# mad-red/VSR-guided-CIC

Measured on NVIDIA B200. Metric: captions/sec beam-search decode (COCO-Entities shape), higher is better.
Workload: dtype f32

## Files before the change

vsr-guided-cic_b200/csrc/api.cu:

```cuda
#include <stdarg.h>
#include <stdlib.h>
#include <string.h>

#include <algorithm>

#include "common.cuh"

namespace vsr {

static thread_local char g_err[1024] = "";

void set_error(const char* fmt, ...) {
  va_list ap;
  va_start(ap, fmt);
  vsnprintf(g_err, sizeof(g_err), fmt, ap);
  va_end(ap);
}

int dev_alloc(Ctx* c, void** p, size_t bytes, bool zero) {
  *p = nullptr;
  if (bytes == 0) bytes = 16;
  cudaError_t e = cudaMalloc(p, bytes);
  if (e != cudaSuccess) {
    set_error("cudaMalloc(%zu bytes) failed: %s", bytes, cudaGetErrorString(e));
    cudaGetLastError();
    return VSR_ENOMEM;
  }
  c->owned.push_back(*p);
  c->epoch++;
  if (zero) VSR_CHECK_CUDA(cudaMemset(*p, 0, bytes));
  return VSR_OK;
}

static void dev_free(Ctx* c, void* p) {
  if (p == nullptr) return;
  auto it = std::find(c->owned.begin(), c->owned.end(), p);
  if (it != c->owned.end()) c->owned.erase(it);
  c->epoch++;
  cudaFree(p);
}

PhaseScope::PhaseScope(Ctx* c_, int id_, cudaStream_t st_) : c(c_), id(id_), st(st_) {
  c->phases[id].launches++;
  if (!c->profiling) return;
  cudaEvent_t e;
  if (cudaEventCreate(&e) == cudaSuccess) { cudaEventRecord(e, st); c->phases[id].ev.push_back(e); }
}
PhaseScope::~PhaseScope() {
  if (!c->profiling) return;
  cudaEvent_t e;
  if (cudaEventCreate(&e) == cudaSuccess) { cudaEventRecord(e, st); c->phases[id].ev.push_back(e); }
}

static const char* kPhaseNames[PH_COUNT] = {
    "prologue", "gemm_a_lstm1_gates", "lstm1_pointwise", "gemm_b_sentinel_h1proj", "gate_pointwise",
    "gemm_c_att_ga", "attend_gate", "gemm_d_lstm2_gates", "lstm2_pointwise", "gemm_e_vocab",
    "softmax_topk", "beam_select", "state_reorder", "backtrack"};

static void reset_phases(Ctx* c) {
  for (int i = 0; i < PH_COUNT; ++i) {
    for (cudaEvent_t e : c->phases[i].ev) cudaEventDestroy(e);
    c->phases[i].ev.clear();
    c->phases[i].launches = 0;
  }
}

#define ALLOC_F(ptr, count) VSR_TRY(dev_alloc(c, (void**)&(ptr), sizeof(float) * (size_t)(count)))

static int pad_rows(int n_valid, int bn, int alt_bn) {
  int r = round_up(n_valid, bn);
  if (alt_bn > 0) r = std::max(r, round_up(n_valid, alt_bn));
  return round_up(r, 128);
}

enum PairKind { PAIR_F16X3 = 0, PAIR_F8 = 1, PAIR_BOTH = 2 };
static PairKind step_kind(const Ctx* c) { return c->gemm_f8 ? PAIR_F8 : PAIR_F16X3; }

int alloc_pair(Ctx* c, F16Pair* b, int rows, int ld, int box_rows, PairKind kind, bool weight = false, int n_valid = 0,
               int alt_bn = 0, int alt_kb = 64) {
  dev_free(c, b->hi); dev_free(c, b->lo); dev_free(c, b->hi8); dev_free(c, b->lo8);
  b->hi = b->lo = b->hi8 = b->lo8 = nullptr;
  if (!c->use_tc) return VSR_OK;
  VSR_TRY(dev_alloc(c, &b->hi, (size_t)rows * ld * 2));
  b->rows = rows; b->ld = ld; b->box_rows = box_rows;
  VSR_TRY(make_tmap_f16(b->map_hi, b->hi, rows, ld, ld, box_rows));
  VSR_TRY(make_tmap_f16(b->map32_hi, b->hi, rows, ld, ld, box_rows, 32));
  if (kind == PAIR_F16X3 || kind == PAIR_BOTH) {
    VSR_TRY(dev_alloc(c, &b->lo, (size_t)rows * ld * 2));
    VSR_TRY(make_tmap_f16(b->map_lo, b->lo, rows, ld, ld, box_rows));
    VSR_TRY(make_tmap_f16(b->map32_lo, b->lo, rows, ld, ld, box_rows, 32));
  }
  if (kind == PAIR_F8 || kind == PAIR_BOTH) {
    VSR_TRY(dev_alloc(c, &b->hi8, (size_t)rows * ld));
    VSR_TRY(dev_alloc(c, &b->lo8, (size_t)rows * ld));
    VSR_TRY(make_tmap_u8(b->map8_hi, b->hi8, rows, ld, ld, box_rows));
    VSR_TRY(make_tmap_u8(b->map8_lo, b->lo8, rows, ld, ld, box_rows));
    VSR_TRY(make_tmap_u8(b->map8_32_hi, b->hi8, rows, ld, ld, box_rows, 32));
    VSR_TRY(make_tmap_u8(b->map8_32_lo, b->lo8, rows, ld, ld, box_rows, 32));
  }
  b->act_scale = (!weight && kind != PAIR_F16X3) ? ACT_SCALE_F8 : 1.f;
  b->kb = c->gemm_kb;
  b->n_valid = n_valid > 0 ? n_valid : rows;
  b->alt_bn = 0;
  if (alt_bn > 0 && c->use_alt_tiles) {
    VSR_TRY(make_tmap_f16(b->alt_hi, b->hi, rows, ld, ld, alt_bn, alt_kb));
    if (kind != PAIR_F8) VSR_TRY(make_tmap_f16(b->alt_lo, b->lo, rows, ld, ld, alt_bn, alt_kb));
    if (kind != PAIR_F16X3) {
      VSR_TRY(make_tmap_u8(b->alt8_hi, b->hi8, rows, ld, ld, alt_bn, alt_kb));
      VSR_TRY(make_tmap_u8(b->alt8_lo, b->lo8, rows, ld, ld, alt_bn, alt_kb));
    }
    b->alt_bn = alt_bn; b->alt_kb = alt_kb;
  }
  if (weight && b->scale == nullptr) VSR_TRY(dev_alloc(c, (void**)&b->scale, 2 * sizeof(float)));
  return VSR_OK;
}

int ensure_rows(Ctx* c, int rows) {
  if (rows <= c->cap_rows) return VSR_OK;
  const int cap = round_up(rows, MPAD);
  float** bufs[] = {&c->h1, &c->c1, &c->h2, &c->c2, &c->h1n, &c->c1n, &c->h2n, &c->c2n, &c->pre1,
                    &c->s_t, &c->g_t, &c->gq, &c->sent, &c->hb, &c->ga, &c->att, &c->pre2, &c->logits, &c->gate_lp,
                    &c->row_max, &c->row_lsum, &c->shift, &c->vpart};
  for (float** p : bufs) { dev_free(c, *p); *p = nullptr; }
  dev_free(c, c->word_idx);
  dev_free(c, c->ptr); dev_free(c, c->ptrn); dev_free(c, c->forced); dev_free(c, c->cand); dev_free(c, c->word_in);
  c->cap_rows = 0;
  const size_t n = cap;
  ALLOC_F(c->h1, n * c->Hp); ALLOC_F(c->c1, n * c->Hp); ALLOC_F(c->h2, n * c->Hp); ALLOC_F(c->c2, n * c->Hp);
  ALLOC_F(c->h1n, n * c->Hp); ALLOC_F(c->c1n, n * c->Hp); ALLOC_F(c->h2n, n * c->Hp); ALLOC_F(c->c2n, n * c->Hp);
  VSR_TRY(dev_alloc(c, (void**)&c->word_idx, sizeof(int32_t) * n));
  ALLOC_F(c->pre1, n * c->NA);
  ALLOC_F(c->s_t, n * c->Hp); ALLOC_F(c->g_t, n * c->Hp); ALLOC_F(c->gq, n * c->Hp);
  ALLOC_F(c->sent, n * c->NB1); ALLOC_F(c->hb, n * c->NB2); ALLOC_F(c->ga, n * c->NC);
  ALLOC_F(c->att, n * c->Fp); ALLOC_F(c->pre2, n * c->ND); ALLOC_F(c->logits, n * c->NE);
  ALLOC_F(c->gate_lp, n * 2); ALLOC_F(c->row_max, n); ALLOC_F(c->row_lsum, n); ALLOC_F(c->shift, n);
  ALLOC_F(c->vpart, n * (size_t)(c->NE / 16) * 2);
  VSR_TRY(dev_alloc(c, (void**)&c->ptr, sizeof(int32_t) * n));
  VSR_TRY(dev_alloc(c, (void**)&c->ptrn, sizeof(int32_t) * n));
  VSR_TRY(dev_alloc(c, (void**)&c->forced, sizeof(int32_t) * n));
  VSR_TRY(dev_alloc(c, (void**)&c->cand, sizeof(int32_t) * n * VSR_MAX_BEAM));
  VSR_TRY(dev_alloc(c, (void**)&c->word_in, sizeof(int64_t) * n));
  const PairKind sk = step_kind(c), hk = sk == PAIR_F8 ? PAIR_BOTH : sk;
  VSR_TRY(alloc_pair(c, &c->h1_b, cap, c->Hp, MPAD, hk)); VSR_TRY(alloc_pair(c, &c->h2_b, cap, c->Hp, MPAD, hk));
  VSR_TRY(alloc_pair(c, &c->s_t_b, cap, c->Hp, MPAD, sk));
  VSR_TRY(alloc_pair(c, &c->h1n_b, cap, c->Hp, MPAD, hk)); VSR_TRY(alloc_pair(c, &c->g_t_b, cap, c->Hp, MPAD, sk));
  VSR_TRY(alloc_pair(c, &c->att_b, cap, c->Fp, MPAD, sk)); VSR_TRY(alloc_pair(c, &c->h2n_b, cap, c->Hp, MPAD, hk));
  c->cap_rows = cap;
  return VSR_OK;
}

int ensure_beam_ws(Ctx* c, int caps, int T) {
  if (caps <= c->cap_caps && T <= c->cap_T) return VSR_OK;
  caps = std::max(caps, c->cap_caps); T = std::max(T, c->cap_T);
  float** fb[] = {&c->seq_lp, &c->seq_lp_n, &c->m0, &c->m1, &c->m0n, &c->m1n, &c->hist_score, &c->hist_lpw, &c->hist_lpg};
  int32_t** ib[] = {&c->sel_beam, &c->sel_word, &c->sel_gate, &c->sel_beam_n, &c->sel_word_n, &c->sel_gate_n,
                    &c->hist_parent, &c->hist_word, &c->hist_gate};
  for (float** p : fb) { dev_free(c, *p); *p = nullptr; }
  for (int32_t** p : ib) { dev_free(c, *p); *p = nullptr; }
  c->cap_caps = 0; c->cap_T = 0;
  const size_t s = (size_t)caps * VSR_MAX_BEAM, hs = s * T;
  ALLOC_F(c->seq_lp, s); ALLOC_F(c->seq_lp_n, s); ALLOC_F(c->m0, s); ALLOC_F(c->m1, s); ALLOC_F(c->m0n, s); ALLOC_F(c->m1n, s);
  ALLOC_F(c->hist_score, hs); ALLOC_F(c->hist_lpw, hs); ALLOC_F(c->hist_lpg, hs);
  VSR_TRY(dev_alloc(c, (void**)&c->sel_beam, sizeof(int32_t) * s));
  VSR_TRY(dev_alloc(c, (void**)&c->sel_word, sizeof(int32_t) * s));
  VSR_TRY(dev_alloc(c, (void**)&c->sel_gate, sizeof(int32_t) * s));
  VSR_TRY(dev_alloc(c, (void**)&c->sel_beam_n, sizeof(int32_t) * s));
  VSR_TRY(dev_alloc(c, (void**)&c->sel_word_n, sizeof(int32_t) * s));
  VSR_TRY(dev_alloc(c, (void**)&c->sel_gate_n, sizeof(int32_t) * s));
  VSR_TRY(dev_alloc(c, (void**)&c->hist_parent, sizeof(int32_t) * hs));
  VSR_TRY(dev_alloc(c, (void**)&c->hist_word, sizeof(int32_t) * hs));
  VSR_TRY(dev_alloc(c, (void**)&c->hist_gate, sizeof(int32_t) * hs));
  c->cap_caps = caps; c->cap_T = T;
  return VSR_OK;
}

static int create_impl(const VsrDims* d, const float* const* w, Ctx** out) {
  VSR_REQUIRE(d != nullptr && w != nullptr && out != nullptr, VSR_EINVAL, "vsr_create: null argument");
  VSR_REQUIRE(d->vocab_size > 0 && d->rnn_size > 0 && d->att_size > 0 && d->input_encoding_size > 0 &&
                  d->det_feat_size > 0 && d->seq_len > 0,
              VSR_EINVAL, "vsr_create: non-positive dimension");
  VSR_REQUIRE(d->det_feat_size % 4 == 0 && d->att_size % 4 == 0, VSR_EINVAL,
              "vsr_create: det_feat_size=%d and att_size=%d must be multiples of 4 (128-bit loads)",
              d->det_feat_size, d->att_size);
  VSR_REQUIRE(d->bos_idx >= 0 && d->bos_idx < d->vocab_size, VSR_EINVAL, "vsr_create: bos_idx out of range");
  VSR_REQUIRE(d->vocab_size <= 1024 * 48, VSR_EINVAL,
              "vsr_create: vocab_size=%d > 49152 unsupported (register-resident softmax/top-k row)", d->vocab_size);
  int ndev = 0;
  cudaError_t e = cudaGetDeviceCount(&ndev);
  VSR_REQUIRE(e == cudaSuccess && ndev > 0, VSR_ECUDA,
              "vsr_create: no CUDA device available (%s); libvsrdec has no CPU fallback",
              cudaGetErrorString(e));
  Ctx* c = new Ctx();
  c->d = *d;
  VSR_CHECK_CUDA(cudaGetDevice(&c->device));
  c->V = d->vocab_size; c->E = d->input_encoding_size; c->H = d->rnn_size; c->F = d->det_feat_size; c->A = d->att_size;
  c->Hp = round_up(c->H, KPAD); c->Ep = round_up(c->E, KPAD); c->Fp = round_up(c->F, KPAD); c->Ap = round_up(c->A, KPAD);
  c->NA = 6 * c->Hp;
  c->oB1_sa = c->Fp;
  c->NB1v = c->oB1_sa + c->A;
  c->NB1 = pad_rows(c->NB1v, 128, 0);
  c->oB2_ha = c->Hp;
  c->oB2_p2 = c->oB2_ha + c->Ap;
  c->NB2v = c->oB2_p2;
  c->NB2 = pad_rows(c->NB2v, 128, 0);
  c->NC = round_up(c->A, NPAD);
  c->ND = 4 * c->Hp;
  c->NE = round_up(c->V, 1152);
  c->NVA = round_up(c->A, NPAD);
  c->KA = (d->h2_first_lstm ? c->Hp : 0) + c->Hp;
  c->KD = c->Fp + 2 * c->Hp;
  for (int i = 0; i < PH_COUNT; ++i) c->phases[i].name = kPhaseNames[i];
  *out = c;
  ALLOC_F(c->WA, (size_t)c->NA * c->KA); ALLOC_F(c->WU, (size_t)c->NA * c->Fp); ALLOC_F(c->bU, c->NA);
  ALLOC_F(c->WB1, (size_t)c->NB1 * c->Hp); ALLOC_F(c->bB1, c->NB1);
  ALLOC_F(c->WB2, (size_t)c->NB2 * c->Hp);
  ALLOC_F(c->WC, (size_t)c->NC * c->Hp);
  ALLOC_F(c->WD, (size_t)c->ND * c->KD); ALLOC_F(c->bD, c->ND);
  if (d->img_second_lstm) ALLOC_F(c->WU2, (size_t)c->ND * c->Fp);
  ALLOC_F(c->WE, (size_t)c->NE * c->Hp); ALLOC_F(c->bE, c->NE);
  ALLOC_F(c->Wva, (size_t)c->NVA * c->Fp);
  ALLOC_F(c->v_a, c->Ap); ALLOC_F(c->v_s, c->Ap); ALLOC_F(c->v_g, c->Ap);
  ALLOC_F(c->embed, (size_t)c->V * c->Ep);
  ALLOC_F(c->WAx, (size_t)c->NA * c->Ep); ALLOC_F(c->X, (size_t)c->V * c->NA);
  {
    const char* mode = getenv("VSRDEC_GEMM");
    c->use_tc = !(mode != nullptr && strcmp(mode, "simt") == 0);
    c->gemm_f8 = !(mode != nullptr && strcmp(mode, "f16x3") == 0);
  }
  int bn = 128;
  if (const char* e = getenv("VSRDEC_BN")) bn = atoi(e) == 256 ? 256 : 128;
  if (const char* e = getenv("VSRDEC_GRAPH")) c->use_graphs = atoi(e) != 0;
  if (const char* e = getenv("VSRDEC_PDL")) c->use_pdl = atoi(e) != 0;
  if (const char* e = getenv("VSRDEC_ZERO_STATE")) c->zero_state_opt = atoi(e) != 0;
  if (const char* e = getenv("VSRDEC_PDL_MODE")) c->pdl_mode = atoi(e);
  if (const char* e = getenv("VSRDEC_KB")) c->gemm_kb = atoi(e) == 32 ? 32 : 64;
  if (const char* e = getenv("VSRDEC_ALT_TILES")) c->use_alt_tiles = atoi(e) != 0;
  const PairKind sk = step_kind(c);
  VSR_TRY(alloc_pair(c, &c->WA_b, c->NA, c->KA, 192, sk == PAIR_F8 ? PAIR_BOTH : sk, true)); VSR_TRY(alloc_pair(c, &c->WB1_b, c->NB1, c->Hp, bn, sk, true, c->NB1v));
  VSR_TRY(alloc_pair(c, &c->WB2_b, c->NB2, c->Hp, bn, sk, true, c->NB2v)); VSR_TRY(alloc_pair(c, &c->WC_b, c->NC, c->Hp, 128, sk, true));
  VSR_TRY(alloc_pair(c, &c->WD_b, c->ND, c->KD, 128, sk, true)); VSR_TRY(alloc_pair(c, &c->WE_b, c->NE, c->Hp, bn, sk, true, c->V, 144, 64));
  if (const char* e = getenv("VSRDEC_PAIR")) c->use_pair = atoi(e) != 0;
  if (const char* e = getenv("VSRDEC_PAIR_MIN_ROWS")) c->pair_min_rows = atoi(e);
  if (c->use_pair && c->use_tc) {
    VSR_TRY(make_pair_maps(&c->WA_b, 96)); VSR_TRY(make_pair_maps(&c->WB1_b, 128)); VSR_TRY(make_pair_maps(&c->WB2_b, 128));
    VSR_TRY(make_pair_maps(&c->WC_b, 128)); VSR_TRY(make_pair_maps(&c->WD_b, 128)); VSR_TRY(make_pair_maps(&c->WE_b, 96));
  }
  c->WA_b.kb = 32;
  if (const char* e = getenv("VSRDEC_KB_A")) c->WA_b.kb = atoi(e) == 32 ? 32 : 64;
  VSR_TRY(alloc_pair(c, &c->WU_b, c->NA, c->Fp, 128, PAIR_F16X3, true)); VSR_TRY(alloc_pair(c, &c->Wva_b, c->NVA, c->Fp, bn, PAIR_F16X3, true));
  if (d->img_second_lstm) VSR_TRY(alloc_pair(c, &c->WU2_b, c->ND, c->Fp, 128, PAIR_F16X3, true));
  VSR_TRY(pack_weights(c, w, 0));
  VSR_CHECK_CUDA(cudaStreamSynchronize(0));
  return VSR_OK;
}

static void drop_graphs(Ctx* c) {
  for (auto& g : c->graphs) cudaGraphExecDestroy(g.exec);
  c->graphs.clear();
  c->graph_seen.clear();
}

template <typename Enqueue>
static int run_graphed(Ctx* c, const Ctx::GraphKey& key, cudaStream_t st, Enqueue enqueue) {
  if (!c->graphs.empty() && c->graphs[0].key.epoch != c->epoch) drop_graphs(c);
  ++c->graph_clock;
  for (auto& g : c->graphs)
    if (memcmp(&g.key, &key, sizeof(key)) == 0) {
      VSR_CHECK_CUDA(cudaGraphLaunch(g.exec, st));
      c->launches += g.launches; g.last_use = c->graph_clock;
      return VSR_OK;
    }
  bool seen = false;
  for (auto& s : c->graph_seen) seen = seen || memcmp(&s, &key, sizeof(key)) == 0;
  if (!seen) {
    if (c->graph_seen.size() >= 32) c->graph_seen.erase(c->graph_seen.begin());
    c->graph_seen.push_back(key);
    return enqueue(st);
  }
  if (c->cap_stream == nullptr) VSR_CHECK_CUDA(cudaStreamCreateWithFlags(&c->cap_stream, cudaStreamNonBlocking));
  const int64_t l0 = c->launches;
  VSR_CHECK_CUDA(cudaStreamBeginCapture(c->cap_stream, cudaStreamCaptureModeThreadLocal));
  const int rc = enqueue(c->cap_stream);
  cudaGraph_t graph = nullptr;
  const cudaError_t ce = cudaStreamEndCapture(c->cap_stream, &graph);
  const int64_t n_launch = c->launches - l0;
  c->launches = l0;
  if (rc != VSR_OK) { if (graph) cudaGraphDestroy(graph); return rc; }
  VSR_CHECK_CUDA(ce);
  cudaGraphExec_t exec = nullptr;
  const cudaError_t ie = cudaGraphInstantiate(&exec, graph, 0);
  cudaGraphDestroy(graph);
  VSR_CHECK_CUDA(ie);
  if (c->graphs.size() >= 16) {
    size_t lru = 0;
    for (size_t i = 1; i < c->graphs.size(); ++i) if (c->graphs[i].last_use < c->graphs[lru].last_use) lru = i;
    cudaGraphExecDestroy(c->graphs[lru].exec);
    c->graphs.erase(c->graphs.begin() + lru);
  }
  c->graphs.push_back({key, exec, n_launch, c->graph_clock});
  VSR_CHECK_CUDA(cudaGraphLaunch(exec, st));
  c->launches += n_launch;
  return VSR_OK;
}

static Ctx::GraphKey graph_key(const Ctx* c, int kind) {
  Ctx::GraphKey key;
  memset(&key, 0, sizeof(key));
  key.kind = kind;
  key.epoch = c->epoch; key.det = c->det; key.det_seqs = c->det_seqs; key.slot_index = c->slot_index; key.verbs = c->verbs;
  key.det_stride = c->det_stride;
  key.b = c->b; key.D = c->D; key.L = c->L; key.R = c->R; key.n_img = c->n_img; key.verbs_dtype = c->verbs_dtype;
  return key;
}

static bool graphs_usable(Ctx* c, cudaStream_t st) {
  cudaStreamCaptureStatus cap = cudaStreamCaptureStatusNone;
  if (cudaStreamIsCapturing(st, &cap) != cudaSuccess) { cudaGetLastError(); cap = cudaStreamCaptureStatusActive; }
  return c->use_graphs && !c->profiling && cap == cudaStreamCaptureStatusNone;
}

static int prologue_impl(Ctx* c, const float* det, int64_t det_stride, int D, const float* det_seqs,
                         const int32_t* slot_index, int b, int L, int R, const void* verbs, int verbs_dtype,
                         cudaStream_t st) {
  VSR_REQUIRE(det != nullptr && (det_seqs != nullptr || slot_index != nullptr), VSR_EINVAL, "vsr_prologue: null input");
  VSR_REQUIRE(b > 0 && D > 0 && L > 0 && R > 0, VSR_EINVAL, "vsr_prologue: bad shape b=%d D=%d L=%d R=%d", b, D, L, R);
  VSR_REQUIRE(R <= 64, VSR_EINVAL, "vsr_prologue: R=%d regions per slot > 64 unsupported", R);
  VSR_REQUIRE(det_stride == 0 || det_stride >= (int64_t)D * c->F, VSR_EINVAL, "vsr_prologue: bad det_batch_stride");
  VSR_REQUIRE(verbs == nullptr || (verbs_dtype >= 0 && verbs_dtype <= 2), VSR_EINVAL, "vsr_prologue: bad verbs dtype");
  VSR_REQUIRE(slot_index == nullptr || det_stride == 0 || det_stride == (int64_t)D * c->F, VSR_EINVAL,
              "vsr_prologue_indexed: detections must be dense (b, D, F) or one shared image");
  VSR_REQUIRE(((uintptr_t)det % 16) == 0 && ((uintptr_t)det_seqs % 16) == 0 && (det_stride % 4) == 0, VSR_EINVAL,
              "vsr_prologue: feature tensors must be 16-byte aligned");
  c->have_prologue = false;
  if (c->profiling) reset_phases(c);
  c->b = b; c->D = D; c->L = L; c->R = R;
  c->n_img = det_stride == 0 ? 1 : b;
  c->det_seqs = det_seqs; c->slot_index = slot_index; c->det = det; c->det_stride = det_stride;
  c->verbs = verbs; c->verbs_dtype = verbs_dtype;
  const size_t n_img_pad = round_up(c->n_img, MPAD);
  if (n_img_pad > c->cap_img) {
    dev_free(c, c->img); dev_free(c, c->U); dev_free(c, c->U2);
    c->img = c->U = c->U2 = nullptr; c->cap_img = 0;
    ALLOC_F(c->img, n_img_pad * c->Fp); ALLOC_F(c->U, n_img_pad * c->NA);
    if (c->d.img_second_lstm) ALLOC_F(c->U2, n_img_pad * c->ND);
    VSR_TRY(alloc_pair(c, &c->img_b, (int)n_img_pad, c->Fp, MPAD, PAIR_F16X3));
    c->cap_img = n_img_pad;
  }
  const size_t prow = slot_index == nullptr
                          ? (size_t)b * L * R
                          : (size_t)round_up(c->n_img * D, MPAD) + round_up(c->n_img, MPAD);
  if (prow > c->cap_P || (size_t)b * L + 1 > c->cap_slots) {
    const size_t need_rows = std::max(prow, c->cap_P), need_slots = std::max((size_t)b * L + 1, c->cap_slots);
    dev_free(c, c->P); dev_free(c, c->seq_valid); dev_free(c, c->slot_mask); dev_free(c, c->slot_base); dev_free(c, c->comp_valid);
    c->P = nullptr; c->seq_valid = nullptr; c->slot_mask = nullptr; c->slot_base = nullptr; c->comp_valid = nullptr;
    c->cap_P = 0; c->cap_slots = 0;
    ALLOC_F(c->P, round_up((int)need_rows, MPAD) * (size_t)c->NVA);
    VSR_TRY(dev_alloc(c, (void**)&c->seq_valid, round_up((int)need_rows, MPAD)));
    VSR_TRY(dev_alloc(c, (void**)&c->slot_mask, sizeof(unsigned long long) * need_slots));
    VSR_TRY(dev_alloc(c, (void**)&c->slot_base, sizeof(int32_t) * need_slots));
    VSR_TRY(dev_alloc(c, (void**)&c->comp_valid, round_up((int)need_rows, MPAD)));
    VSR_TRY(alloc_pair(c, &c->ds_b, round_up((int)need_rows, MPAD), c->Fp, MPAD, PAIR_F16X3));
    c->cap_P = need_rows; c->cap_slots = need_slots;
  }
  c->Pmean = slot_index != nullptr ? c->P + (size_t)round_up(c->n_img * D, MPAD) * c->NVA : nullptr;
  const size_t dvr = (size_t)c->n_img * D;
  if (dvr > c->cap_detv) {
    dev_free(c, c->det_valid); c->det_valid = nullptr; c->cap_detv = 0;
    VSR_TRY(dev_alloc(c, (void**)&c->det_valid, dvr));
    c->cap_detv = dvr;
  }
  VSR_TRY(ensure_rows(c, b));
  c->p_compact = slot_index == nullptr && c->use_tc;
  auto enqueue = [&](cudaStream_t s) {
    return slot_index == nullptr ? run_prologue(c, det, det_stride, s) : run_prologue_indexed(c, det, det_stride, s);
  };
  if (graphs_usable(c, st)) VSR_TRY(run_graphed(c, graph_key(c, 1), st, enqueue));
  else VSR_TRY(enqueue(st));
  c->have_prologue = true;
  return VSR_OK;
}

__global__ void k_copy2d(float* dst, int ld_dst, const float* src, int ld_src, int w, int rows) {
  const int i = blockIdx.x * blockDim.x + threadIdx.x;
  const int n = blockIdx.y;
  if (i < w && n < rows) dst[(size_t)n * ld_dst + i] = src[(size_t)n * ld_src + i];
}
__global__ void k_slots_from_i64(int32_t* ptr, const int64_t* slot, int rows, int L) {
  const int n = blockIdx.x * blockDim.x + threadIdx.x;
  if (n >= rows) return;
  int64_t s = slot[n];
  s = s < 0 ? 0 : (s > L - 1 ? L - 1 : s);
  ptr[n] = (int32_t)s;
}
__global__ void k_fill_i32(int32_t* p, int v, int n) {
  const int i = blockIdx.x * blockDim.x + threadIdx.x;
  if (i < n) p[i] = v;
}

static int copy2d(Ctx* c, float* dst, int ld_dst, const float* src, int ld_src, int w, int rows, cudaStream_t st) {
  dim3 grid((w + 255) / 256, rows);
  k_copy2d<<<grid, 256, 0, st>>>(dst, ld_dst, src, ld_src, w, rows);
  VSR_CHECK_CUDA(cudaGetLastError()); c->launches++;
  return VSR_OK;
}

static int step_impl(Ctx* c, const float* h1, const float* c1, const float* h2, const float* c2,
                     const int64_t* slot, const int64_t* word, int use_verbs, int gt, float* h1o, float* c1o,
                     float* h2o, float* c2o, float* out_logp, float* gate_logp, cudaStream_t st) {
  VSR_REQUIRE(c->have_prologue, VSR_ESTATE, "vsr_step: call vsr_prologue first");
  VSR_REQUIRE(h1 && c1 && h2 && c2 && slot && word, VSR_EINVAL, "vsr_step: null state input");
  VSR_REQUIRE(!use_verbs || c->verbs != nullptr, VSR_EINVAL, "vsr_step: use_verbs without a verbs tensor");
  const int b = c->b, H = c->H;
  VSR_TRY(copy2d(c, c->h1, c->Hp, h1, H, H, b, st));
  VSR_TRY(copy2d(c, c->c1, c->Hp, c1, H, H, b, st));
  VSR_TRY(copy2d(c, c->h2, c->Hp, h2, H, H, b, st));
  VSR_TRY(copy2d(c, c->c2, c->Hp, c2, H, H, b, st));
  k_slots_from_i64<<<(b + 127) / 128, 128, 0, st>>>(c->ptr, slot, b, c->L);
  VSR_CHECK_CUDA(cudaGetLastError()); c->launches++;
  VSR_TRY(launch_words(c, word, b, st));
  if (c->use_tc) {
    VSR_TRY(launch_split_pair(c->h1, c->h1_b, (size_t)b * c->Hp, st));
    VSR_TRY(launch_split_pair(c->h2, c->h2_b, (size_t)b * c->Hp, st));
    c->launches += 2;
  }
  StepIO io{};
  io.rows = b; io.cur_beam = 1; io.use_verbs = use_verbs != 0; io.gt = gt != 0;
  io.out_logp = out_logp; io.out_stride = c->V; io.gate_out = gate_logp; io.gate_stride = 2; io.topk = 0;
  io.need_h32 = true;
  VSR_TRY(run_step(c, io, st));
  if (h1o) VSR_TRY(copy2d(c, h1o, H, c->h1n, c->Hp, H, b, st));
  if (c1o) VSR_TRY(copy2d(c, c1o, H, c->c1n, c->Hp, H, b, st));
  if (h2o) VSR_TRY(copy2d(c, h2o, H, c->h2n, c->Hp, H, b, st));
  if (c2o) VSR_TRY(copy2d(c, c2o, H, c->c2n, c->Hp, H, b, st));
  return VSR_OK;
}

static int enqueue_beam_steps(Ctx* c, int k, const int64_t* eos, int use_verbs, int gt, const VsrTrace* tr,
                              cudaStream_t st) {
  const int b = c->b, T = c->d.seq_len;
  VSR_TRY(launch_state_init(c, b, st));
  const bool have_forced = tr && tr->forced_beam && tr->forced_word && tr->forced_gate;
  if (c->profiling) {
    for (cudaEvent_t e : c->step_ev) cudaEventDestroy(e);
    c->step_ev.clear();
  }
  for (int t = 0; t < T; ++t) {
    if (c->profiling) {
      cudaEvent_t e;
      if (cudaEventCreate(&e) == cudaSuccess) { cudaEventRecord(e, st); c->step_ev.push_back(e); }
    }
    const int cur = t == 0 ? 1 : k;
    const int rows = b * cur;
    StepIO io{};
    io.rows = rows; io.cur_beam = cur; io.use_verbs = use_verbs != 0; io.gt = gt != 0; io.topk = k;
    io.zero_state = t == 0 && c->zero_state_opt;
    if (tr && tr->step_out) { io.out_logp = tr->step_out + (size_t)t * b * k * c->V; io.out_stride = c->V; }
    if (tr && tr->step_gate) { io.gate_out = tr->step_gate + (size_t)t * b * k * 2; io.gate_stride = 2; }
    VSR_TRY(run_step(c, io, st));
    const size_t fo = (size_t)t * b * k;
    VSR_TRY(launch_beam_step(c, t, b, cur, k, eos[0], eos[1], have_forced ? tr->forced_beam + fo : nullptr,
                             have_forced ? tr->forced_word + fo : nullptr,
                             have_forced ? tr->forced_gate + fo : nullptr, t + 1 < T, st));
  }
  if (c->profiling) {
    cudaEvent_t e;
    if (cudaEventCreate(&e) == cudaSuccess) { cudaEventRecord(e, st); c->step_ev.push_back(e); }
  }
  return VSR_OK;
}

static int beam_steps_graphed(Ctx* c, int k, const int64_t* eos, int use_verbs, int gt, cudaStream_t st) {
  Ctx::GraphKey key = graph_key(c, 0);
  key.eos0 = eos[0]; key.eos1 = eos[1];
  key.k = k; key.use_verbs = use_verbs; key.gt = gt; key.T = c->d.seq_len;
  return run_graphed(c, key, st, [&](cudaStream_t s) { return enqueue_beam_steps(c, k, eos, use_verbs, gt, nullptr, s); });
}

static int beam_search_impl(Ctx* c, int k, int out_size, const int64_t* eos, int use_verbs, int gt,
                            int64_t* out_words, int64_t* out_gates, float* lp_words, float* lp_gates,
                            const VsrTrace* tr, cudaStream_t st) {
  VSR_REQUIRE(c->have_prologue, VSR_ESTATE, "vsr_beam_search: call vsr_prologue first");
  VSR_REQUIRE(k >= 1 && k <= VSR_MAX_BEAM, VSR_EINVAL, "vsr_beam_search: beam_size=%d not in [1,%d]", k, VSR_MAX_BEAM);
  VSR_REQUIRE(out_size >= 1 && out_size <= k, VSR_EINVAL, "vsr_beam_search: out_size=%d not in [1,beam]", out_size);
  VSR_REQUIRE(c->V >= k, VSR_EINVAL, "vsr_beam_search: vocabulary (%d) smaller than the beam (%d): a row has fewer than "
              "beam distinct word candidates", c->V, k);
  VSR_REQUIRE(c->d.seq_len <= VSR_MAX_SEQ_LEN, VSR_EINVAL, "vsr_beam_search: seq_len=%d > %d unsupported by the back-track kernel",
              c->d.seq_len, VSR_MAX_SEQ_LEN);
  VSR_REQUIRE(eos && out_words && out_gates && lp_words && lp_gates, VSR_EINVAL, "vsr_beam_search: null argument");
  VSR_REQUIRE(!use_verbs || c->verbs != nullptr, VSR_EINVAL, "vsr_beam_search: use_verbs without a verbs tensor");
  const int b = c->b, T = c->d.seq_len;
  VSR_TRY(ensure_rows(c, b * k));
  VSR_TRY(ensure_beam_ws(c, b, T));
  c->hist_T = T; c->hist_b = b; c->hist_k = k;
  if (tr == nullptr && graphs_usable(c, st))
    VSR_TRY(beam_steps_graphed(c, k, eos, use_verbs, gt, st));
  else
    VSR_TRY(enqueue_beam_steps(c, k, eos, use_verbs, gt, tr, st));
  VSR_TRY(launch_backtrack(c, b, k, T, out_size, out_words, out_gates, lp_words, lp_gates, st));
  return VSR_OK;
}

static int ensure_fwd_ws(Ctx* c, int rows) {
  if (rows <= c->cap_fwd_rows) return VSR_OK;
  const int cap = round_up(rows, MPAD);
  dev_free(c, c->logits_all); dev_free(c, c->gate_all);
  c->logits_all = c->gate_all = nullptr; c->cap_fwd_rows = 0;
  ALLOC_F(c->logits_all, (size_t)cap * c->NE); ALLOC_F(c->gate_all, (size_t)cap * 2);
  VSR_TRY(alloc_pair(c, &c->h2all_b, cap, c->Hp, MPAD, step_kind(c)));
  c->cap_fwd_rows = cap;
  return VSR_OK;
}

static int enqueue_forward_steps(Ctx* c, const int64_t* captions, int T, bool batched, float* out, float* gate, cudaStream_t st) {
  const int b = c->b;
  VSR_TRY(launch_state_init(c, b, st));
  for (int t = 0; t < T; ++t) {
    if (t == 0) {
      VSR_CHECK_CUDA(cudaMemcpy2DAsync(c->word_in, sizeof(int64_t), captions, sizeof(int64_t) * T,
                                       sizeof(int64_t), b, cudaMemcpyDeviceToDevice, st));
      VSR_TRY(launch_words(c, c->word_in, b, st));
    }
    StepIO io{};
    io.rows = b; io.cur_beam = 1; io.use_verbs = false; io.gt = false; io.topk = 0;
    io.zero_state = t == 0 && c->zero_state_opt;
    if (batched) {
      io.skip_vocab = true;
      VSR_TRY(run_step(c, io, st));
      VSR_TRY(launch_gate_head(c, b, c->gate_all + (size_t)t * 2, (int64_t)T * 2, st));
      VSR_TRY(launch_rows_to_all(c, c->h2n_b, c->h2all_b, b, T, t, st));
    } else {
      io.out_logp = out + (size_t)t * c->V; io.out_stride = (int64_t)T * c->V;
      io.gate_out = gate + (size_t)t * 2; io.gate_stride = (int64_t)T * 2;
      VSR_TRY(run_step(c, io, st));
    }
    if (t + 1 < T) VSR_TRY(launch_commit_identity(c, b, captions + (t + 1), T, t + 1, st));
  }
  if (batched) VSR_TRY(run_vocab_rows(c, c->h2all_b, c->logits_all, b * T, nullptr, st, false));
  return VSR_OK;
}

static int forward_impl(Ctx* c, const int64_t* captions, int T, float* out, float* gate, cudaStream_t st) {
  VSR_REQUIRE(c->have_prologue, VSR_ESTATE, "vsr_forward_teacher: call vsr_prologue first");
  VSR_REQUIRE(captions && out && gate, VSR_EINVAL, "vsr_forward_teacher: null argument");
  VSR_REQUIRE(T >= 1 && T <= c->L, VSR_EINVAL, "vsr_forward_teacher: T=%d exceeds the prologue's slot count L=%d", T, c->L);
  const int b = c->b;
  VSR_TRY(ensure_rows(c, b));
  const bool batched = c->use_tc;
  if (!batched) return enqueue_forward_steps(c, captions, T, false, out, gate, st);
  VSR_TRY(ensure_fwd_ws(c, b * T));
  if (graphs_usable(c, st)) {
    Ctx::GraphKey key = graph_key(c, 2);
    key.captions = captions; key.T = T;
    VSR_TRY(run_graphed(c, key, st, [&](cudaStream_t s) { return enqueue_forward_steps(c, captions, T, true, nullptr, nullptr, s); }));
  } else {
    VSR_TRY(enqueue_forward_steps(c, captions, T, true, nullptr, nullptr, st));
  }
  VSR_TRY(run_vocab_rows(c, c->h2all_b, c->logits_all, b * T, out, st, true));
  VSR_CHECK_CUDA(cudaMemcpyAsync(gate, c->gate_all, sizeof(float) * (size_t)b * T * 2, cudaMemcpyDeviceToDevice, st));
  return VSR_OK;
}

static int greedy_impl(Ctx* c, int64_t* out_words, int64_t* out_gates, cudaStream_t st) {
  VSR_REQUIRE(c->have_prologue, VSR_ESTATE, "vsr_greedy: call vsr_prologue first");
  VSR_REQUIRE(out_words && out_gates, VSR_EINVAL, "vsr_greedy: null argument");
  const int b = c->b, T = c->d.seq_len;
  VSR_TRY(ensure_rows(c, b));
  VSR_TRY(ensure_beam_ws(c, b, T));
  VSR_TRY(launch_state_init(c, b, st));
  for (int t = 0; t < T; ++t) {
    StepIO io{};
    io.rows = b; io.cur_beam = 1; io.use_verbs = false; io.gt = false; io.topk = 1;
    io.zero_state = t == 0 && c->zero_state_opt;
    VSR_TRY(run_step(c, io, st));
    VSR_TRY(launch_greedy_pick(c, b, t, T, out_words, out_gates, st));
    if (t + 1 < T) VSR_TRY(launch_commit_identity(c, b, nullptr, 0, -1, st));
  }
  return VSR_OK;
}

static int sample_impl(Ctx* c, uint64_t seed, int64_t* out_words, int64_t* out_gates, float* lp_words, float* lp_gates,
                       cudaStream_t st) {
  VSR_REQUIRE(c->have_prologue, VSR_ESTATE, "vsr_sample: call vsr_prologue first");
  VSR_REQUIRE(out_words && out_gates && lp_words && lp_gates, VSR_EINVAL, "vsr_sample: null argument");
  const int b = c->b, T = c->d.seq_len;
  VSR_TRY(ensure_rows(c, b));
  VSR_TRY(ensure_beam_ws(c, b, T));
  VSR_TRY(launch_state_init(c, b, st));
  for (int t = 0; t < T; ++t) {
    StepIO io{};
    io.rows = b; io.cur_beam = 1; io.use_verbs = false; io.gt = false; io.topk = 0;
    io.zero_state = t == 0 && c->zero_state_opt;
    VSR_TRY(run_step(c, io, st));
    VSR_TRY(launch_sample_pick(c, b, t, T, seed, out_words, out_gates, lp_words, lp_gates, st));
    if (t + 1 < T) VSR_TRY(launch_commit_identity(c, b, nullptr, 0, -1, st));
  }
  return VSR_OK;
}

}

using vsr::Ctx;

struct DeviceGuard {
  int prev = -1; bool switched = false;
  explicit DeviceGuard(const vsr::Ctx* c) {
    if (c != nullptr && cudaGetDevice(&prev) == cudaSuccess && prev != c->device) switched = cudaSetDevice(c->device) == cudaSuccess;
  }
// ... 187 lines not shown
```

vsr-guided-cic_b200/csrc/beam.cu:

```cuda
#include <cuda_fp16.h>
#include <math.h>

#include "common.cuh"

namespace vsr {

namespace {

__device__ __forceinline__ bool before(float v1, int i1, float v2, int i2) {
  return v1 > v2 || (v1 == v2 && i1 < i2);
}

__device__ __forceinline__ float row_logp(const float* logits, int ld, const float* row_max,
                                          const float* row_lsum, const int32_t* forced, int row, int word) {
  const int f = forced[row];
  if (f >= 0) return word == f ? 0.f : -1e6f;
  return (logits[(size_t)row * ld + word] - row_max[row]) - row_lsum[row];
}

struct BeamArgs {
  int t, b, cur, k, V;
  int64_t eos0, eos1;
  const float* logits; int ld;
  const float* row_max; const float* row_lsum; const int32_t* forced; const int32_t* cand;
  const float* gate_lp;
  const float* seq_lp; float* seq_lp_n;
  float *m0, *m1, *m0n, *m1n;
  const int32_t *prev_word, *prev_gate;
  int32_t *sel_beam, *sel_word, *sel_gate;
  int32_t *hist_parent, *hist_word, *hist_gate;
  float *hist_score, *hist_lpw, *hist_lpg;
  const int32_t *f_beam, *f_word, *f_gate;
};

constexpr int MAXC = 2 * VSR_MAX_BEAM * VSR_MAX_BEAM;

struct BeamSmem {
  float seq[VSR_MAX_BEAM], m0[VSR_MAX_BEAM], m1[VSR_MAX_BEAM], ps[VSR_MAX_BEAM];
  int full[VSR_MAX_BEAM], pb[VSR_MAX_BEAM], pw[VSR_MAX_BEAM], pg[VSR_MAX_BEAM];
};

__device__ __forceinline__ void beam_select_warp(const BeamArgs& a, BeamSmem& sh, int c, int lane, bool write) {
  const int k = a.k, cur = a.cur;
  float* s_seq = sh.seq; float* s_m0 = sh.m0; float* s_m1 = sh.m1; float* s_ps = sh.ps;
  int* s_full = sh.full; int* s_pb = sh.pb; int* s_pw = sh.pw; int* s_pg = sh.pg;

  if (lane < cur) {
    float m0 = 1.f, m1 = 1.f, seq = 0.f;
    if (a.t > 0) {
      seq = a.seq_lp[c * k + lane];
      m0 = a.m0[c * k + lane] * ((int64_t)a.prev_word[c * k + lane] != a.eos0 ? 1.f : 0.f);
      m1 = a.m1[c * k + lane] * ((int64_t)a.prev_gate[c * k + lane] != a.eos1 ? 1.f : 0.f);
    }
    s_seq[lane] = seq; s_m0[lane] = m0; s_m1[lane] = m1;
    s_full[lane] = (a.t == 0) ? 1 : (fminf(fmaxf(m0 + m1, 0.f), 1.f) != 0.f);
  }
  __syncwarp();

  if (a.f_beam == nullptr) {
    float cs[MAXC / 32]; int cf[MAXC / 32]; bool used[MAXC / 32];
    const int ncand = cur * k * 2;
#pragma unroll
    for (int q = 0; q < MAXC / 32; ++q) {
      const int idx = lane + 32 * q;
      cs[q] = -INFINITY; cf[q] = 0x7fffffff; used[q] = true;
      if (idx < ncand) {
        const int j = idx / (2 * k), i = (idx >> 1) % k, g = idx & 1;
        const int row = c * cur + j;
        int word; float sc;
        if (s_full[j]) {
          word = a.cand[row * VSR_MAX_BEAM + i];
          const float wl = row_logp(a.logits, a.ld, a.row_max, a.row_lsum, a.forced, row, word);
          sc = __fadd_rn(s_seq[j], __fadd_rn(wl, a.gate_lp[row * 2 + g]));
        } else {
          word = i;
          sc = (i == 0) ? s_seq[j] : -999.f;
        }
        cs[q] = sc; cf[q] = j * 2 * a.V + word * 2 + g; used[q] = false;
      }
    }
    for (int sel = 0; sel < k; ++sel) {
      float bv = -INFINITY; int bf = 0x7fffffff;
#pragma unroll
      for (int q = 0; q < MAXC / 32; ++q)
        if (!used[q] && before(cs[q], cf[q], bv, bf)) { bv = cs[q]; bf = cf[q]; }
      {
        const unsigned u = __float_as_uint(bv);
        const unsigned key = (u & 0x80000000u) ? ~u : (u | 0x80000000u);
        const unsigned kbest = __reduce_max_sync(0xffffffffu, key);
        const int fbest = (int)__reduce_min_sync(0xffffffffu, key == kbest ? (unsigned)bf : 0xffffffffu);
        const unsigned owner = __ballot_sync(0xffffffffu, key == kbest && bf == fbest);
        bv = __shfl_sync(0xffffffffu, bv, __ffs(owner) - 1);
        bf = fbest;
      }
#pragma unroll
      for (int q = 0; q < MAXC / 32; ++q) if (cf[q] == bf) used[q] = true;
      if (lane == 0) {
        const int j = bf / (2 * a.V), rem = bf - j * 2 * a.V;
        s_pb[sel] = j; s_pw[sel] = rem >> 1; s_pg[sel] = rem & 1; s_ps[sel] = bv;
      }
    }
  } else if (lane < k) {
    const int j = a.f_beam[c * k + lane], word = a.f_word[c * k + lane], g = a.f_gate[c * k + lane];
    const int row = c * cur + j;
    float sc;
    if (s_full[j]) {
      const float wl = row_logp(a.logits, a.ld, a.row_max, a.row_lsum, a.forced, row, word);
      sc = __fadd_rn(s_seq[j], __fadd_rn(wl, a.gate_lp[row * 2 + g]));
    } else {
      sc = (word == 0) ? s_seq[j] : -999.f;
    }
    s_pb[lane] = j; s_pw[lane] = word; s_pg[lane] = g; s_ps[lane] = sc;
  }
  __syncwarp();

  if (lane < k && write) {
    const int j = s_pb[lane], word = s_pw[lane], g = s_pg[lane];
    const int row = c * cur + j;
    const int o = c * k + lane;
    float lw = row_logp(a.logits, a.ld, a.row_max, a.row_lsum, a.forced, row, word);
    float lg = a.gate_lp[row * 2 + g];
    if (a.t > 0) { lw *= s_m0[j]; lg *= s_m1[j]; }
    a.sel_beam[o] = j; a.sel_word[o] = word; a.sel_gate[o] = g;
    a.seq_lp_n[o] = s_ps[lane];
    a.m0n[o] = s_m0[j]; a.m1n[o] = s_m1[j];
    a.hist_parent[o] = j; a.hist_word[o] = word; a.hist_gate[o] = g;
    a.hist_score[o] = s_ps[lane]; a.hist_lpw[o] = lw; a.hist_lpg[o] = lg;
  }
}

struct AdvanceArgs {
  int rows_new, cur, k;
  const int32_t* parent;
  const int32_t* word32;
  const int64_t* word64; int64_t word64_stride;
  const int32_t* gate32;
  int fixed_slot;
  int L, Hp, Ep, V;
  const float *h1n, *c1n, *h2n, *c2n;
  float *h1, *c1, *h2, *c2;
  const int32_t* ptr; int32_t* ptrn;
  int32_t* word_idx;
  int n_tw;
  const uint4* tw_src[8]; uint4* tw_dst[8]; int tw_vec[8];
};

__device__ __forceinline__ void advance_row(const AdvanceArgs& a, int n, int p, int64_t w, int gate_shift) {
  const size_t so = (size_t)p * a.Hp, dof = (size_t)n * a.Hp;
  for (int i = threadIdx.x * 4; i < a.Hp; i += blockDim.x * 4) {
    if (a.h1n != nullptr) {
      *reinterpret_cast<float4*>(a.h1 + dof + i) = *reinterpret_cast<const float4*>(a.h1n + so + i);
      *reinterpret_cast<float4*>(a.h2 + dof + i) = *reinterpret_cast<const float4*>(a.h2n + so + i);
    }
    *reinterpret_cast<float4*>(a.c1 + dof + i) = *reinterpret_cast<const float4*>(a.c1n + so + i);
    *reinterpret_cast<float4*>(a.c2 + dof + i) = *reinterpret_cast<const float4*>(a.c2n + so + i);
  }
  w = w < 0 ? 0 : (w >= a.V ? a.V - 1 : w);
  for (int q = 0; q < a.n_tw; ++q) {
    const int nv = a.tw_vec[q];
    const uint4* src = a.tw_src[q] + (size_t)p * nv;
    uint4* dst = a.tw_dst[q] + (size_t)n * nv;
    for (int i = threadIdx.x; i < nv; i += blockDim.x) dst[i] = src[i];
  }
  if (threadIdx.x == 0) {
    a.word_idx[n] = (int32_t)w;
    int s;
    if (a.fixed_slot >= 0) s = a.fixed_slot;
    else {
      s = a.ptr[p] + gate_shift;
      s = s < 0 ? 0 : (s > a.L - 1 ? a.L - 1 : s);
    }
    a.ptrn[n] = s;
  }
}

__global__ void __launch_bounds__(256) k_advance(const AdvanceArgs a) {
  const int n = blockIdx.x;
  const int c = n / a.k;
  const int p = a.parent != nullptr ? c * a.cur + a.parent[n] : n;
  const int64_t w = a.word32 != nullptr ? (int64_t)a.word32[n] : a.word64[(size_t)n * a.word64_stride];
  advance_row(a, n, p, w, a.gate32 != nullptr ? a.gate32[n] : 0);
}

__global__ void __launch_bounds__(256) k_beam_step(const BeamArgs b, const AdvanceArgs a, int do_advance) {
  __shared__ BeamSmem sh;
  const int c = blockIdx.x, i = blockIdx.y;
  pdl_trigger();
  pdl_wait();
  if (threadIdx.x < 32) beam_select_warp(b, sh, c, threadIdx.x, i == 0);
  __syncthreads();
  if (!do_advance) return;
  advance_row(a, c * b.k + i, c * b.cur + sh.pb[i], (int64_t)sh.pw[i], sh.pg[i]);
}

__global__ void k_state_init(float* h1, float* c1, float* h2, float* c2, int32_t* word_idx, int32_t* ptr,
                             int bos, int Hp, TwinOut h1b, TwinOut h2b) {
  const int n = blockIdx.x;
  const float4 z = make_float4(0.f, 0.f, 0.f, 0.f);
  for (int i = threadIdx.x * 4; i < Hp; i += blockDim.x * 4) {
    const size_t o = (size_t)n * Hp + i;
    *reinterpret_cast<float4*>(h1 + o) = z; *reinterpret_cast<float4*>(c1 + o) = z;
    *reinterpret_cast<float4*>(h2 + o) = z; *reinterpret_cast<float4*>(c2 + o) = z;
    store_twin4(h1b, o, z); store_twin4(h2b, o, z);
  }
  if (threadIdx.x == 0) { ptr[n] = 0; word_idx[n] = bos; }
}

__global__ void k_words_from_i64(const int64_t* words, int32_t* word_idx, int rows, int V) {
  const int n = blockIdx.x * blockDim.x + threadIdx.x;
  if (n >= rows) return;
  int64_t w = words[n];
  w = w < 0 ? 0 : (w >= V ? V - 1 : w);
  word_idx[n] = (int32_t)w;
}

__global__ void k_greedy_pick(const int32_t* cand, const float* gate_lp, int32_t* sel_word,
                              int32_t* sel_gate, int64_t* out_words, int64_t* out_gates, int rows,
                              int t, int T) {
  const int n = blockIdx.x * blockDim.x + threadIdx.x;
  if (n >= rows) return;
  const int w = cand[n * VSR_MAX_BEAM];
  const int g = gate_lp[n * 2 + 1] > gate_lp[n * 2 + 0] ? 1 : 0;
  sel_word[n] = w; sel_gate[n] = g;
  out_words[(size_t)n * T + t] = w; out_gates[(size_t)n * T + t] = g;
}

__device__ __forceinline__ uint4 philox4x32_10(uint4 ctr, uint2 key) {
#pragma unroll
  for (int r = 0; r < 10; ++r) {
    const unsigned hi0 = __umulhi(0xD2511F53u, ctr.x), lo0 = 0xD2511F53u * ctr.x;
    const unsigned hi1 = __umulhi(0xCD9E8D57u, ctr.z), lo1 = 0xCD9E8D57u * ctr.z;
    ctr = make_uint4(hi1 ^ ctr.y ^ key.x, lo1, hi0 ^ ctr.w ^ key.y, lo0);
    key.x += 0x9E3779B9u; key.y += 0xBB67AE85u;
  }
  return ctr;
}
__device__ __forceinline__ float u01(unsigned x) { return ((float)(x >> 8) + 0.5f) * (1.f / 16777216.f); }

__global__ void __launch_bounds__(256) k_sample_pick(const float* __restrict__ logits, int ld, int V, const float* __restrict__ row_max,
                                                     const float* __restrict__ row_lsum, const float* __restrict__ gate_lp,
                                                     unsigned long long seed, int t, int T, int32_t* sel_word, int32_t* sel_gate,
                                                     int64_t* out_words, int64_t* out_gates, float* lp_words, float* lp_gates) {
  __shared__ float s_v[8];
  __shared__ int s_i[8];
  const int n = blockIdx.x, tid = threadIdx.x, lane = tid & 31, warp = tid >> 5;
  const float* x = logits + (size_t)n * ld;
  const uint2 key = make_uint2((unsigned)seed, (unsigned)(seed >> 32));
  float bv = -INFINITY; int bi = 0x7fffffff;
  for (int v0 = tid * 4; v0 < V; v0 += 256 * 4) {
    const uint4 r = philox4x32_10(make_uint4((unsigned)(v0 >> 2), (unsigned)n, (unsigned)t, 0u), key);
    const float4 q = *reinterpret_cast<const float4*>(x + v0);
    const float xs[4] = {q.x, q.y, q.z, q.w};
    const unsigned rs[4] = {r.x, r.y, r.z, r.w};
#pragma unroll
    for (int e = 0; e < 4; ++e) {
      if (v0 + e >= V) break;
      const float g = -logf(-logf(u01(rs[e])));
      const float sc = xs[e] + g;
      if (sc > bv) { bv = sc; bi = v0 + e; }
    }
  }
#pragma unroll
  for (int o = 16; o > 0; o >>= 1) {
    const float ov = __shfl_xor_sync(0xffffffffu, bv, o);
    const int oi = __shfl_xor_sync(0xffffffffu, bi, o);
    if (before(ov, oi, bv, bi)) { bv = ov; bi = oi; }
  }
  if (lane == 0) { s_v[warp] = bv; s_i[warp] = bi; }
  __syncthreads();
  if (tid == 0) {
    for (int w = 1; w < 8; ++w) if (before(s_v[w], s_i[w], bv, bi)) { bv = s_v[w]; bi = s_i[w]; }
    const int word = bi < V ? bi : V - 1;
    const float lw = (x[word] - row_max[n]) - row_lsum[n];
    const uint4 r = philox4x32_10(make_uint4(0u, (unsigned)n, (unsigned)t, 1u), key);
    const float g0 = gate_lp[(size_t)n * 2], g1 = gate_lp[(size_t)n * 2 + 1];
    const int gate = u01(r.x) < expf(g0) ? 0 : 1;
    sel_word[n] = word; sel_gate[n] = gate;
    out_words[(size_t)n * T + t] = word; out_gates[(size_t)n * T + t] = gate;
    lp_words[(size_t)n * T + t] = lw; lp_gates[(size_t)n * T + t] = gate == 0 ? g0 : g1;
  }
}

__global__ void __launch_bounds__(64) k_backtrack(int b, int k, int T, int out_size, const float* seq_lp,
                                                  const int32_t* hist_parent, const int32_t* hist_word,
                                                  const int32_t* hist_gate, const float* hist_lpw, const float* hist_lpg,
                                                  int64_t* out_words, int64_t* out_gates, float* lp_words, float* lp_gates) {
  extern __shared__ __align__(16) unsigned char bt_smem[];
  int32_t* s_par = reinterpret_cast<int32_t*>(bt_smem);
  int32_t* s_wrd = s_par + T * k;
  int32_t* s_gat = s_wrd + T * k;
  float* s_lpw = reinterpret_cast<float*>(s_gat + T * k);
  float* s_lpg = s_lpw + T * k;
  __shared__ float s_seq[VSR_MAX_BEAM];
  const int c = blockIdx.x;
  for (int i = threadIdx.x; i < T * k; i += blockDim.x) {
    const int t = i / k, j = i - t * k;
    const size_t hi = ((size_t)t * b + c) * k + j;
    s_par[i] = hist_parent[hi]; s_wrd[i] = hist_word[hi]; s_gat[i] = hist_gate[hi];
    s_lpw[i] = hist_lpw[hi]; s_lpg[i] = hist_lpg[hi];
  }
  if (threadIdx.x < k) s_seq[threadIdx.x] = seq_lp[c * k + threadIdx.x];
  __syncthreads();
  const int o = threadIdx.x;
  if (o >= out_size) return;
  int order[VSR_MAX_BEAM];
  for (int i = 0; i < k; ++i) order[i] = i;
  for (int i = 1; i < k; ++i) {
    const int oi = order[i];
    const float v = s_seq[oi];
    int j = i - 1;
    while (j >= 0 && s_seq[order[j]] < v) { order[j + 1] = order[j]; --j; }
    order[j + 1] = oi;
  }
  const int final_slot = order[o];
  int slot = final_slot;
  const size_t ob = ((size_t)c * out_size + o) * T;
  for (int t = T - 1; t >= 0; --t) {
    out_words[ob + t] = s_wrd[t * k + slot];
    out_gates[ob + t] = s_gat[t * k + slot];
    lp_words[ob + t] = s_lpw[t * k + final_slot];
    lp_gates[ob + t] = s_lpg[t * k + final_slot];
    slot = s_par[t * k + slot];
  }
}

}

static TwinOut pp(const Ctx* c, const F16Pair& b) { return twin_out(&b, c->use_tc); }

int launch_state_init(Ctx* c, int rows, cudaStream_t st) {
  k_state_init<<<rows, 256, 0, st>>>(c->h1, c->c1, c->h2, c->c2, c->word_idx, c->ptr, c->d.bos_idx, c->Hp,
                                     pp(c, c->h1_b), pp(c, c->h2_b));
  VSR_CHECK_CUDA(cudaGetLastError()); c->launches++;
  return VSR_OK;
}

int launch_words(Ctx* c, const int64_t* words, int rows, cudaStream_t st) {
  k_words_from_i64<<<(rows + 127) / 128, 128, 0, st>>>(words, c->word_idx, rows, c->V);
  VSR_CHECK_CUDA(cudaGetLastError()); c->launches++;
  return VSR_OK;
}

static void fill_advance(Ctx* c, AdvanceArgs& a) {
  a.L = c->L; a.Hp = c->Hp; a.Ep = c->Ep; a.V = c->V;
  a.h1n = c->state_h32 ? c->h1n : nullptr; a.c1n = c->c1n; a.h2n = c->state_h32 ? c->h2n : nullptr; a.c2n = c->c2n;
  a.h1 = c->h1; a.c1 = c->c1; a.h2 = c->h2; a.c2 = c->c2;
  a.ptr = c->ptr; a.ptrn = c->ptrn; a.word_idx = c->word_idx;
  a.n_tw = 0;
  if (c->use_tc) {
    auto add = [&](const void* src, void* dst, int bytes_per_elem) {
      if (src == nullptr || dst == nullptr) return;
      a.tw_src[a.n_tw] = (const uint4*)src; a.tw_dst[a.n_tw] = (uint4*)dst; a.tw_vec[a.n_tw] = c->Hp * bytes_per_elem / 16;
      ++a.n_tw;
    };
    const F16Pair* src[2] = {&c->h1n_b, &c->h2n_b};
    F16Pair* dst[2] = {&c->h1_b, &c->h2_b};
    for (int q = 0; q < 2; ++q) {
      add(src[q]->hi, dst[q]->hi, 2); add(src[q]->lo, dst[q]->lo, 2);
      add(src[q]->hi8, dst[q]->hi8, 1); add(src[q]->lo8, dst[q]->lo8, 1);
    }
  }
}

int launch_beam_step(Ctx* c, int t, int b, int cur, int k, int64_t eos0, int64_t eos1, const int32_t* f_beam,
                     const int32_t* f_word, const int32_t* f_gate, bool advance, cudaStream_t st) {
  PhaseScope ps(c, PH_BEAM, st);
  BeamArgs a{};
  a.t = t; a.b = b; a.cur = cur; a.k = k; a.V = c->V; a.eos0 = eos0; a.eos1 = eos1;
  a.logits = c->logits; a.ld = c->NE; a.row_max = c->row_max; a.row_lsum = c->row_lsum;
  a.forced = c->forced; a.cand = c->cand; a.gate_lp = c->gate_lp;
  a.seq_lp = c->seq_lp; a.seq_lp_n = c->seq_lp_n;
  a.m0 = c->m0; a.m1 = c->m1; a.m0n = c->m0n; a.m1n = c->m1n;
  a.prev_word = c->sel_word; a.prev_gate = c->sel_gate;
  a.sel_beam = c->sel_beam_n; a.sel_word = c->sel_word_n; a.sel_gate = c->sel_gate_n;
  const size_t off = (size_t)t * b * k;
  a.hist_parent = c->hist_parent + off; a.hist_word = c->hist_word + off; a.hist_gate = c->hist_gate + off;
  a.hist_score = c->hist_score + off; a.hist_lpw = c->hist_lpw + off; a.hist_lpg = c->hist_lpg + off;
  a.f_beam = f_beam; a.f_word = f_word; a.f_gate = f_gate;
  AdvanceArgs ad{};
  ad.rows_new = b * k; ad.cur = cur; ad.k = k; ad.fixed_slot = -1;
  fill_advance(c, ad);
  VSR_CHECK_CUDA(launch_k(k_beam_step, dim3(b, advance ? k : 1), dim3(256), 0, st, c->use_pdl && (c->pdl_mode & 2), a, ad, advance ? 1 : 0));
  VSR_CHECK_CUDA(cudaGetLastError()); c->launches++;
  std::swap(c->sel_beam, c->sel_beam_n);
  std::swap(c->sel_word, c->sel_word_n);
  std::swap(c->sel_gate, c->sel_gate_n);
  std::swap(c->seq_lp, c->seq_lp_n);
  std::swap(c->m0, c->m0n);
  std::swap(c->m1, c->m1n);
  if (advance) std::swap(c->ptr, c->ptrn);
  return VSR_OK;
}

static int launch_advance(Ctx* c, AdvanceArgs& a, cudaStream_t st) {
  fill_advance(c, a);
  k_advance<<<a.rows_new, 256, 0, st>>>(a);
  VSR_CHECK_CUDA(cudaGetLastError()); c->launches++;
  std::swap(c->ptr, c->ptrn);
  return VSR_OK;
}

int launch_commit_identity(Ctx* c, int rows, const int64_t* next_words, int64_t word_stride,
                           int next_slot, cudaStream_t st) {
  PhaseScope ps(c, PH_REORDER, st);
  AdvanceArgs a{};
  a.rows_new = rows; a.cur = 1; a.k = 1;
  a.parent = nullptr;
  if (next_words != nullptr) { a.word64 = next_words; a.word64_stride = word_stride; a.gate32 = nullptr; }
  else { a.word32 = c->sel_word; a.gate32 = c->sel_gate; }
  a.fixed_slot = next_slot;
  return launch_advance(c, a, st);
}

int launch_greedy_pick(Ctx* c, int rows, int t, int T, int64_t* out_words, int64_t* out_gates,
                       cudaStream_t st) {
  PhaseScope ps(c, PH_BEAM, st);
  k_greedy_pick<<<(rows + 127) / 128, 128, 0, st>>>(c->cand, c->gate_lp, c->sel_word, c->sel_gate,
                                                    out_words, out_gates, rows, t, T);
  VSR_CHECK_CUDA(cudaGetLastError()); c->launches++;
  return VSR_OK;
}

int launch_sample_pick(Ctx* c, int rows, int t, int T, uint64_t seed, int64_t* out_words, int64_t* out_gates,
                       float* lp_words, float* lp_gates, cudaStream_t st) {
  PhaseScope ps(c, PH_BEAM, st);
  k_sample_pick<<<rows, 256, 0, st>>>(c->logits, c->NE, c->V, c->row_max, c->row_lsum, c->gate_lp, (unsigned long long)seed, t, T,
                                      c->sel_word, c->sel_gate, out_words, out_gates, lp_words, lp_gates);
  VSR_CHECK_CUDA(cudaGetLastError()); c->launches++;
  return VSR_OK;
}

int launch_backtrack(Ctx* c, int b, int k, int T, int out_size, int64_t* out_words,
                     int64_t* out_gates, float* lp_words, float* lp_gates, cudaStream_t st) {
  PhaseScope ps(c, PH_FINAL, st);
  VSR_REQUIRE(T <= VSR_MAX_SEQ_LEN, VSR_EINVAL, "seq_len=%d > %d unsupported by the back-track kernel", T, VSR_MAX_SEQ_LEN);
  k_backtrack<<<b, 64, (size_t)T * k * 20, st>>>(b, k, T, out_size, c->hist_score + (size_t)(T - 1) * b * k, c->hist_parent, c->hist_word,
                                            c->hist_gate, c->hist_lpw, c->hist_lpg, out_words, out_gates,
                                            lp_words, lp_gates);
  VSR_CHECK_CUDA(cudaGetLastError()); c->launches++;
  return VSR_OK;
}

}
```

vsr-guided-cic_b200/csrc/common.cuh:

```cuda
#pragma once
#include <cuda_runtime.h>
#include <stdint.h>
#include <stdio.h>
#include <string>
#include <vector>

#include "../../include/vsrdec.h"

namespace vsr {

void set_error(const char* fmt, ...);
#define VSR_CHECK_CUDA(expr)                                                                 \
  do {                                                                                       \
    cudaError_t _e = (expr);                                                                 \
    if (_e != cudaSuccess) {                                                                 \
      vsr::set_error("%s:%d CUDA error %s: %s", __FILE__, __LINE__, #expr,                   \
                     cudaGetErrorString(_e));                                                \
      return VSR_ECUDA;                                                                      \
    }                                                                                        \
  } while (0)
#define VSR_REQUIRE(cond, code, ...)                                                         \
  do {                                                                                       \
    if (!(cond)) {                                                                           \
      vsr::set_error(__VA_ARGS__);                                                           \
      return (code);                                                                         \
    }                                                                                        \
  } while (0)
#define VSR_TRY(expr)                                                                        \
  do {                                                                                       \
    int _r = (expr);                                                                         \
    if (_r != VSR_OK) return _r;                                                             \
  } while (0)

static inline int round_up(int x, int m) { return (x + m - 1) / m * m; }

#ifdef __CUDACC__
}
#include <cuda_fp16.h>
#include <cuda_fp8.h>
namespace vsr {
__device__ __forceinline__ float fast_sigmoid(float x) { return __fdividef(1.f, 1.f + __expf(-x)); }
__device__ __forceinline__ float fast_tanh(float x) { return 1.f - __fdividef(2.f, __expf(2.f * x) + 1.f); }
#endif

constexpr int KPAD = 64;
constexpr int NPAD = 256;
constexpr int MPAD = 128;

constexpr float ACT_SCALE_F8 = 256.f;

struct F16Pair {
  void* hi = nullptr;
  void* lo = nullptr;
  void* hi8 = nullptr;
  void* lo8 = nullptr;
  float act_scale = 1.f;
  int rows = 0, ld = 0, box_rows = 0;
  float* scale = nullptr;
  int kb = 64;
  alignas(64) unsigned char map_hi[128];
  alignas(64) unsigned char map_lo[128];
  alignas(64) unsigned char map32_hi[128];
  alignas(64) unsigned char map32_lo[128];
  alignas(64) unsigned char map8_hi[128];
  alignas(64) unsigned char map8_lo[128];
  alignas(64) unsigned char map8_32_hi[128];
  alignas(64) unsigned char map8_32_lo[128];
  alignas(64) unsigned char alt8_hi[128];
  alignas(64) unsigned char alt8_lo[128];
  int pair_rows = 0;
  alignas(64) unsigned char pair_hi[128];
  alignas(64) unsigned char pair_lo[128];
  alignas(64) unsigned char pair_lo16[128];
  alignas(64) unsigned char pair_h8[128];
  int n_valid = 0;
  int alt_bn = 0, alt_kb = 64;
  alignas(64) unsigned char alt_hi[128];
  alignas(64) unsigned char alt_lo[128];
};

struct TwinOut {
  void* hi; void* lo; uint8_t* hi8; uint8_t* lo8;
  float scale;
};
inline TwinOut twin_out(const F16Pair* b, bool enabled = true) {
  TwinOut o{nullptr, nullptr, nullptr, nullptr, 1.f};
  if (b != nullptr && enabled) { o.hi = b->hi; o.lo = b->lo; o.hi8 = (uint8_t*)b->hi8; o.lo8 = (uint8_t*)b->lo8; o.scale = b->act_scale; }
  return o;
}
#ifdef __CUDACC__
__device__ __forceinline__ void store_twin4(const TwinOut& o, size_t off, const float4 v) {
  if (o.hi == nullptr) return;
  const float x[4] = {fminf(fmaxf(v.x * o.scale, -65504.f), 65504.f), fminf(fmaxf(v.y * o.scale, -65504.f), 65504.f),
                      fminf(fmaxf(v.z * o.scale, -65504.f), 65504.f), fminf(fmaxf(v.w * o.scale, -65504.f), 65504.f)};
  __align__(8) __half h[4];
  float hf[4], r[4];
#pragma unroll
  for (int j = 0; j < 4; ++j) { h[j] = __float2half_rn(x[j]); hf[j] = __half2float(h[j]); r[j] = x[j] - hf[j]; }
  *reinterpret_cast<uint2*>(reinterpret_cast<__half*>(o.hi) + off) = *reinterpret_cast<const uint2*>(h);
  if (o.lo != nullptr) {
    __align__(8) __half l[4];
#pragma unroll
    for (int j = 0; j < 4; ++j) l[j] = __float2half_rn(r[j]);
    *reinterpret_cast<uint2*>(reinterpret_cast<__half*>(o.lo) + off) = *reinterpret_cast<const uint2*>(l);
  }
  if (o.hi8 != nullptr) {
    const unsigned h01 = __nv_cvt_float2_to_fp8x2(make_float2(hf[0] * 0.03125f, hf[1] * 0.03125f), __NV_SATFINITE, __NV_E4M3);
    const unsigned h23 = __nv_cvt_float2_to_fp8x2(make_float2(hf[2] * 0.03125f, hf[3] * 0.03125f), __NV_SATFINITE, __NV_E4M3);
    const unsigned l01 = __nv_cvt_float2_to_fp8x2(make_float2(r[0] * 32.f, r[1] * 32.f), __NV_SATFINITE, __NV_E4M3);
    const unsigned l23 = __nv_cvt_float2_to_fp8x2(make_float2(r[2] * 32.f, r[3] * 32.f), __NV_SATFINITE, __NV_E4M3);
    *reinterpret_cast<uint32_t*>(o.hi8 + off) = h01 | (h23 << 16);
    *reinterpret_cast<uint32_t*>(o.lo8 + off) = l01 | (l23 << 16);
  }
}
#endif

struct GemmSeg {
  const float* a;
  int lda;
  int k;
  int k_valid;
  const F16Pair* b = nullptr;
};
__host__ __device__ inline int cell_col(int g, int u, int ng) {
  return (u >> 5) * (ng * 32) + g * 32 + (u & 31);
}

#ifdef __CUDACC__
__device__ __forceinline__ void pdl_wait() { asm volatile("griddepcontrol.wait;" ::: "memory"); }
__device__ __forceinline__ void pdl_trigger() { asm volatile("griddepcontrol.launch_dependents;" ::: "memory"); }

template <typename... KArgs, typename... Args>
inline cudaError_t launch_k(void (*kernel)(KArgs...), dim3 grid, dim3 block, size_t smem, cudaStream_t st, bool pdl,
                            Args&&... args) {
  cudaLaunchConfig_t cfg = {};
  cfg.gridDim = grid; cfg.blockDim = block; cfg.dynamicSmemBytes = smem; cfg.stream = st;
  cudaLaunchAttribute attr[1];
  attr[0].id = cudaLaunchAttributeProgrammaticStreamSerialization;
  attr[0].val.programmaticStreamSerializationAllowed = 1;
  cfg.attrs = attr; cfg.numAttrs = pdl ? 1 : 0;
  return cudaLaunchKernelEx(&cfg, kernel, std::forward<Args>(args)...);
}
#endif

struct FusedCell {
  int mode = 0;
  const float* c_old = nullptr; float* c_new = nullptr; float* h_new = nullptr;
  const F16Pair *h_b = nullptr, *s_b = nullptr, *g_b = nullptr;
  float* s_new = nullptr;
  float* gq = nullptr;
  int ld_state = 0;
  int gt_cols = 0; const float* gt_gq = nullptr; const float* gt_c1n = nullptr;
  float* g_t = nullptr;
  float* vocab_part = nullptr; int* vocab_tiles_out = nullptr; int* vocab_bn_out = nullptr;
};
constexpr int VOCAB_REC = 16;

struct GemmArgs {
  GemmSeg seg[3];
  int nseg;
  const float* w;
  int ldw;
  const float* bias;
  const float* rowadd;
  int ld_rowadd, row_div, rowadd_mul;
  const float* cadd;
  int ld_cadd;
  float* c;
  int ldc;
  int M, N;
  const float* gather = nullptr;
  int ld_gather = 0;
  const int32_t* gather_idx = nullptr;
  const uint8_t* row_skip;
  const F16Pair* wb = nullptr;
  bool allow_pair = false;
  int pair_min_rows = 1024;
  bool no_alt = false;
  bool f8 = false;
  bool pdl = false;
  bool relu = false;
  bool zero_acc = false;
  int pdl_flags = 0;
  FusedCell cell;
};
struct Ctx;
int launch_gemm(Ctx* c, const GemmArgs& g, cudaStream_t st, const GemmArgs* g2 = nullptr);
int launch_gemm_simt(const GemmArgs& g, cudaStream_t st);
int launch_gemm_tc(const GemmArgs& g, const GemmArgs* g2, cudaStream_t st);
bool gemm_uses_tc(const Ctx* c, const GemmArgs& g);
int make_tmap_f16(void* out_map, const void* base, int rows, int cols, int ld, int box_rows, int kb = 64);
int make_tmap_u8(void* out_map, const void* base, int rows, int cols, int ld, int box_rows, int kb = 64);
int make_pair_maps(F16Pair* b, int pair_rows);
int launch_split_pair(const float* x, const F16Pair& p, size_t n, cudaStream_t st, bool weight_scale = false);

struct Phase {
  const char* name;
  std::vector<cudaEvent_t> ev;
  int launches = 0;
};

enum PhaseId {
  PH_PROLOGUE = 0, PH_GEMM_A, PH_LSTM1, PH_GEMM_B, PH_GT, PH_GEMM_C, PH_ATTEND, PH_GEMM_D, PH_LSTM2,
  PH_GEMM_E, PH_SOFTMAX_TOPK, PH_BEAM, PH_REORDER, PH_FINAL, PH_COUNT
};

struct Ctx {
  VsrDims d;
  int device;
  int V, E, H, F, A;
  int Hp, Ep, Fp, Ap;
  int NA, NB1, NB2, NC, ND, NE;
  int NB1v, NB2v;
  int KA;
  int KD;
  int oB1_sa;
  int oB2_ha, oB2_p2;
  float *WA, *WU, *bU;
  float *WB1, *bB1;
  float *WB2;
  float *WC;
  float *WD, *bD;
  float *WU2;
  float *WE, *bE;
  float *Wva;
  float *v_a, *v_s, *v_g;
  float *embed;
  float *WAx;
  float *X;
  int NVA;
  bool use_tc = true;
  int pair_min_rows = 640;
  bool use_pair = true;
  bool gemm_f8 = true;
  bool use_alt_tiles = true;
  int gemm_kb = 64;
  F16Pair WA_b, WB1_b, WB2_b, WC_b, WD_b, WE_b;
  F16Pair WU_b, WU2_b, Wva_b;
  F16Pair ds_b, img_b;
  F16Pair h1_b, h2_b, s_t_b, h1n_b, g_t_b, att_b, h2n_b;
  F16Pair h2all_b; float* logits_all = nullptr; float* gate_all = nullptr; int cap_fwd_rows = 0;
  int64_t* vt_keys = nullptr; int32_t* vt_off = nullptr; int32_t* vt_idx = nullptr; int vt_n = 0;
  bool have_prologue = false;
  int b = 0, D = 0, L = 0, R = 0, n_img = 0;
  const float* det_seqs = nullptr;
  const int32_t* slot_index = nullptr;
  const float* det = nullptr; int64_t det_stride = 0;
  float* Pmean = nullptr;
  const void* verbs = nullptr; int verbs_dtype = 0;
  float* img = nullptr;
  float* U = nullptr;
  float* U2 = nullptr;
  float* P = nullptr;
  uint8_t* seq_valid = nullptr;
  unsigned long long* slot_mask = nullptr;
  int32_t* slot_base = nullptr;
  uint8_t* comp_valid = nullptr;
  bool p_compact = false;
  uint8_t* det_valid = nullptr;
  size_t cap_img = 0, cap_P = 0, cap_detv = 0, cap_slots = 0;
  int cap_rows = 0;
  float *h1, *c1, *h2, *c2;
  float *h1n, *c1n, *h2n, *c2n;
  int32_t *word_idx;
  int32_t *ptr, *ptrn;
  float *pre1;
  float *s_t, *g_t;
  float *gq;
  float *sent;
  float *hb;
  float *ga;
  float *att;
  float *pre2;
  float *logits;
  float *gate_lp;
  float *shift;
  float *row_max, *row_lsum;
  int32_t *forced;
  int32_t *cand;
  float *vpart;
  int cap_caps = 0, cap_T = 0;
  float *seq_lp, *seq_lp_n;
  float *m0, *m1, *m0n, *m1n;
  int32_t *sel_beam, *sel_word, *sel_gate;
  int32_t *sel_beam_n, *sel_word_n, *sel_gate_n;
  int32_t *hist_parent, *hist_word, *hist_gate;
  float *hist_score, *hist_lpw, *hist_lpg;
  int hist_T = 0, hist_b = 0, hist_k = 0;
  int64_t* word_in = nullptr;
  int64_t launches = 0;
  bool profiling = false;
  Phase phases[PH_COUNT];
  std::vector<cudaEvent_t> step_ev;
  std::vector<void*> owned;
  struct GraphKey {
    uint64_t epoch;
    int64_t kind;
    const void* captions;
    const void *det, *det_seqs, *slot_index, *verbs;
    int64_t det_stride, eos0, eos1;
    int32_t b, D, L, R, n_img, verbs_dtype, k, use_verbs, gt, T;
  };
  struct GraphEntry { GraphKey key; cudaGraphExec_t exec; int64_t launches; uint64_t last_use; };
  std::vector<GraphEntry> graphs;
  std::vector<GraphKey> graph_seen;
  uint64_t epoch = 0, graph_clock = 0;
  cudaStream_t cap_stream = nullptr;
  bool attend_attr_set = false;
  bool state_h32 = true;
  bool use_graphs = true;
  bool zero_state_opt = true;
  bool use_pdl = true;
  int pdl_mode = 5;
};

int dev_alloc(Ctx* c, void** p, size_t bytes, bool zero = true);

struct PhaseScope {
  Ctx* c; int id; cudaStream_t st;
  PhaseScope(Ctx* c_, int id_, cudaStream_t st_);
  ~PhaseScope();
};

int pack_weights(Ctx* c, const float* const* w, cudaStream_t st);
int run_prologue(Ctx* c, const float* det, int64_t det_stride, cudaStream_t st);
int run_prologue_indexed(Ctx* c, const float* det, int64_t det_stride, cudaStream_t st);
int ensure_rows(Ctx* c, int rows);
int ensure_beam_ws(Ctx* c, int caps, int T);

struct StepIO {
  int rows;
  int cur_beam;
  bool use_verbs, gt;
  float* out_logp;
  int64_t out_stride;
  float* gate_out;
  int64_t gate_stride;
  int topk;
  bool zero_state;
  bool skip_vocab;
  bool need_h32;
};
int run_step(Ctx* c, const StepIO& io, cudaStream_t st);

int launch_state_init(Ctx* c, int rows, cudaStream_t st);
int launch_words(Ctx* c, const int64_t* words, int rows, cudaStream_t st);
int launch_beam_step(Ctx* c, int t, int b, int cur, int k, int64_t eos0, int64_t eos1,
                     const int32_t* f_beam, const int32_t* f_word, const int32_t* f_gate, bool advance,
                     cudaStream_t st);
int launch_backtrack(Ctx* c, int b, int k, int T, int out_size, int64_t* out_words,
                     int64_t* out_gates, float* lp_words, float* lp_gates, cudaStream_t st);
int launch_commit_identity(Ctx* c, int rows, const int64_t* next_words, int64_t word_stride,
                           int next_slot, cudaStream_t st);
int launch_greedy_pick(Ctx* c, int rows, int t, int T, int64_t* out_words, int64_t* out_gates,
                       cudaStream_t st);
int launch_sample_pick(Ctx* c, int rows, int t, int T, uint64_t seed, int64_t* out_words, int64_t* out_gates,
                       float* lp_words, float* lp_gates, cudaStream_t st);
int launch_gate_head(Ctx* c, int rows, float* gate_out, int64_t gate_stride, cudaStream_t st);
int launch_rows_to_all(Ctx* c, const F16Pair& src, const F16Pair& dst, int rows, int T, int t, cudaStream_t st);
int run_vocab_rows(Ctx* c, const F16Pair& a_b, float* logits, int M, float* out_logp, cudaStream_t st, bool softmax_only);

}
```

vsr-guided-cic_b200/csrc/gemm_tc.cu:

```cuda
#include <cuda.h>
#include <stdlib.h>
#include <string.h>
#include <cuda_fp16.h>

#include "common.cuh"

namespace vsr {

namespace {

constexpr int BM = 128;
constexpr int BK = 64;
constexpr int UMMA_K = 16;
constexpr int TC_EPI_WARPS = 8;
constexpr int TC_EPI_THREADS = 32 * TC_EPI_WARPS;
constexpr int TC_THREADS = 64 + TC_EPI_THREADS;

template <int BN, int KB> struct TcCfg {
  static constexpr int kStageB = 2 * BM * KB * 2 + 2 * BN * KB * 2;
  static constexpr int kStages = (220 * 1024) / kStageB > 8 ? 8 : (220 * 1024) / kStageB;
  static constexpr int kTmemCols = (BN <= 128) ? 128 : 256;
  static constexpr int kABytes = BM * KB * 2;
  static constexpr int kWBytes = BN * KB * 2;
  static constexpr int kStageBytes = 2 * kABytes + 2 * kWBytes;
  static constexpr int kRingBytes = kStages * kStageBytes;
  static constexpr bool kTileEpi = (BN == 128 || BN == 192);
  static constexpr int kEpiBytes = kTileEpi ? 32 * BN * 4 : 4096;
  static constexpr int kSmemBytes = kRingBytes + 1024 + kEpiBytes;
};

__device__ __forceinline__ uint32_t smem_u32(const void* p) { return (uint32_t)__cvta_generic_to_shared(p); }

__device__ __forceinline__ void mbar_init(uint64_t* bar, uint32_t count) {
  asm volatile("mbarrier.init.shared::cta.b64 [%0], %1;" ::"r"(smem_u32(bar)), "r"(count));
}
__device__ __forceinline__ void mbar_expect_tx(uint64_t* bar, uint32_t bytes) {
  asm volatile("mbarrier.arrive.expect_tx.shared::cta.b64 _, [%0], %1;" ::"r"(smem_u32(bar)), "r"(bytes) : "memory");
}
__device__ __forceinline__ void mbar_wait(uint64_t* bar, uint32_t parity) {
  asm volatile(
      "{\n\t"
      ".reg .pred p;\n\t"
      "WAIT_LOOP:\n\t"
      "mbarrier.try_wait.parity.shared::cta.b64 p, [%0], %1;\n\t"
      "@p bra WAIT_DONE;\n\t"
      "bra WAIT_LOOP;\n\t"
      "WAIT_DONE:\n\t"
      "}" ::"r"(smem_u32(bar)), "r"(parity) : "memory");
}
__device__ __forceinline__ void tma_load_2d(const CUtensorMap* map, uint64_t* bar, void* dst, int c0, int c1) {
  asm volatile(
      "cp.async.bulk.tensor.2d.shared::cluster.global.mbarrier::complete_tx::bytes [%0], [%1, {%3, %4}], [%2];"
      ::"r"(smem_u32(dst)), "l"(map), "r"(smem_u32(bar)), "r"(c0), "r"(c1) : "memory");
}
__device__ __forceinline__ void prefetch_tmap(const CUtensorMap* map) {
  asm volatile("prefetch.tensormap [%0];" ::"l"(map) : "memory");
}

__device__ __forceinline__ uint64_t make_sw64_desc(uint32_t smem_addr) {
  uint64_t d = 0;
  d |= (uint64_t)((smem_addr >> 4) & 0x3FFF);
  d |= (uint64_t)1 << 16;
  d |= (uint64_t)(512 >> 4) << 32;
  d |= (uint64_t)1 << 46;
  d |= (uint64_t)4 << 61;
  return d;
}
template <int KB> __device__ __forceinline__ uint64_t make_kmajor_desc(uint32_t smem_addr);

__device__ __forceinline__ uint64_t make_sw128_desc(uint32_t smem_addr) {
  uint64_t d = 0;
  d |= (uint64_t)((smem_addr >> 4) & 0x3FFF);
  d |= (uint64_t)1 << 16;
  d |= (uint64_t)(1024 >> 4) << 32;
  d |= (uint64_t)1 << 46;
  d |= (uint64_t)2 << 61;
  return d;
}

template <> __device__ __forceinline__ uint64_t make_kmajor_desc<64>(uint32_t a) { return make_sw128_desc(a); }
template <> __device__ __forceinline__ uint64_t make_kmajor_desc<32>(uint32_t a) { return make_sw64_desc(a); }

__device__ __forceinline__ uint64_t make_sw32_desc(uint32_t smem_addr) {
  uint64_t d = 0;
  d |= (uint64_t)((smem_addr >> 4) & 0x3FFF);
  d |= (uint64_t)1 << 16;
  d |= (uint64_t)(256 >> 4) << 32;
  d |= (uint64_t)1 << 46;
  d |= (uint64_t)6 << 61;
  return d;
}
template <int KB> __device__ __forceinline__ uint64_t make_kmajor_desc8(uint32_t smem_addr);
template <> __device__ __forceinline__ uint64_t make_kmajor_desc8<64>(uint32_t a) { return make_sw64_desc(a); }
template <> __device__ __forceinline__ uint64_t make_kmajor_desc8<32>(uint32_t a) { return make_sw32_desc(a); }

template <int BN> __device__ __forceinline__ constexpr uint32_t make_idesc() {
  return (1u << 4) | ((uint32_t)(BN >> 3) << 17) | ((uint32_t)(BM >> 4) << 24);
}

__device__ __forceinline__ void umma_f16(uint32_t tmem_d, uint64_t adesc, uint64_t bdesc, uint32_t idesc, uint32_t acc) {
  asm volatile(
      "{\n\t"
      ".reg .pred p;\n\t"
      "setp.ne.b32 p, %4, 0;\n\t"
      "tcgen05.mma.cta_group::1.kind::f16 [%0], %1, %2, %3, p;\n\t"
      "}" ::"r"(tmem_d), "l"(adesc), "l"(bdesc), "r"(idesc), "r"(acc) : "memory");
}
__device__ __forceinline__ void umma_f8(uint32_t tmem_d, uint64_t adesc, uint64_t bdesc, uint32_t idesc, uint32_t acc) {
  asm volatile(
      "{\n\t"
      ".reg .pred p;\n\t"
      "setp.ne.b32 p, %4, 0;\n\t"
      "tcgen05.mma.cta_group::1.kind::f8f6f4 [%0], %1, %2, %3, p;\n\t"
      "}" ::"r"(tmem_d), "l"(adesc), "l"(bdesc), "r"(idesc), "r"(acc) : "memory");
}
__device__ __forceinline__ void umma_commit(uint64_t* bar) {
  asm volatile("tcgen05.commit.cta_group::1.mbarrier::arrive::one.shared::cluster.b64 [%0];" ::"r"(smem_u32(bar)) : "memory");
}
__device__ __forceinline__ void tmem_ld16(uint32_t taddr, uint32_t (&r)[16]) {
  asm volatile(
      "tcgen05.ld.sync.aligned.32x32b.x16.b32 "
      "{%0, %1, %2, %3, %4, %5, %6, %7, %8, %9, %10, %11, %12, %13, %14, %15}, [%16];"
      : "=r"(r[0]), "=r"(r[1]), "=r"(r[2]), "=r"(r[3]), "=r"(r[4]), "=r"(r[5]), "=r"(r[6]), "=r"(r[7]),
        "=r"(r[8]), "=r"(r[9]), "=r"(r[10]), "=r"(r[11]), "=r"(r[12]), "=r"(r[13]), "=r"(r[14]), "=r"(r[15])
      : "r"(taddr));
  asm volatile("tcgen05.wait::ld.sync.aligned;" ::: "memory");
}



enum { EPI_PLAIN = 0, EPI_LSTM1 = 1, EPI_LSTM2 = 2, EPI_VOCAB = 3 };

struct TcProblem {
  CUtensorMap a_hi[3], a_lo[3], w_hi, w_lo;
  CUtensorMap a_h8[3], w_h8;
  int f8;
  int nseg;
  int kblocks[3];
  int n_tiles, m_tiles, M;
  const uint8_t* row_skip;
  const float* bias;
  const float* rowadd; int ld_rowadd, row_div, rowadd_mul;
  const float* cadd; int ld_cadd;
  const float* gather; int ld_gather; const int32_t* gather_idx;
  float* c; int ldc;
  int mode;
  const float* c_old; float* c_new; float* h_new; TwinOut h_tw;
  float* s_new; TwinOut s_tw; float* gq;
  int ld_state;
  int gt_cols; const float* gt_gq; const float* gt_c1n; float* g_t; TwinOut g_tw;
  float* vpart; int n_valid;
  int zero_acc;
  const float* acc_scale;
  float act_inv;
};
struct TcParams {
  TcProblem pr[2];
  int nprob;
  int pdl_flags;
};

__device__ __forceinline__ void epi_bar(int id) { asm volatile("bar.sync %0, %1;" ::"r"(id), "n"(TC_EPI_THREADS) : "memory"); }
__device__ __forceinline__ void add4(float4& a, const float4 b) { a.x += b.x; a.y += b.y; a.z += b.z; a.w += b.w; }

template <int BN>
__device__ __forceinline__ int tile_slot(int r, int c4) { return r * BN + ((c4 ^ (r & 7)) << 2); }

__device__ __forceinline__ void store4(float* f32, const TwinOut& tw, size_t off, const float4 v) {
  if (f32 != nullptr) *reinterpret_cast<float4*>(f32 + off) = v;
  store_twin4(tw, off, v);
}

template <int BN>
__device__ __forceinline__ void tile_dump(uint32_t tlane, float* tile, int hsel, int lane, bool zero_acc, float sc) {
  constexpr int NCH = BN / 16;
#pragma unroll
  for (int ch = 0; ch < NCH; ++ch) {
    if ((ch < NCH / 2) != (hsel == 0)) continue;
    uint32_t r[16];
    if (zero_acc) {
#pragma unroll
      for (int j = 0; j < 16; ++j) r[j] = 0u;
    } else {
      tmem_ld16(tlane + (uint32_t)(ch * 16), r);
    }
#pragma unroll
    for (int j = 0; j < 4; ++j)
      *reinterpret_cast<float4*>(tile + tile_slot<BN>(lane, ch * 4 + j)) =
          make_float4(__uint_as_float(r[4 * j]) * sc, __uint_as_float(r[4 * j + 1]) * sc, __uint_as_float(r[4 * j + 2]) * sc,
                      __uint_as_float(r[4 * j + 3]) * sc);
  }
}

template <int BN>
__device__ __forceinline__ void tile_plain(const TcProblem& p, const float* tile, const float* s_bias, int rowq, int n0, int te) {
  constexpr int P4 = BN / 4, ITEMS = 32 * P4 / TC_EPI_THREADS;
  float4 acc[ITEMS], x0[ITEMS], x1[ITEMS], x2[ITEMS];
  const float4 zero = make_float4(0.f, 0.f, 0.f, 0.f);
#pragma unroll
  for (int k = 0; k < ITEMS; ++k) {
    const int idx = te + k * TC_EPI_THREADS;
    const int r = idx / P4, c4 = idx - r * P4;
    const int row = rowq + r, n = n0 + 4 * c4;
    acc[k] = *reinterpret_cast<const float4*>(tile + tile_slot<BN>(r, c4));
    x0[k] = zero; x1[k] = zero; x2[k] = zero;
    if (row < p.M) {
      if (n < p.gt_cols) {
        x0[k] = *reinterpret_cast<const float4*>(p.gt_gq + (size_t)row * p.ld_state + n);
        x1[k] = *reinterpret_cast<const float4*>(p.gt_c1n + (size_t)row * p.ld_state + n);
      } else {
        if (p.rowadd != nullptr)
          x0[k] = __ldg(reinterpret_cast<const float4*>(p.rowadd + (size_t)((row / p.row_div) * p.rowadd_mul) * p.ld_rowadd + n));
        if (p.cadd != nullptr) x1[k] = *reinterpret_cast<const float4*>(p.cadd + (size_t)row * p.ld_cadd + n);
        if (p.gather != nullptr) x2[k] = __ldg(reinterpret_cast<const float4*>(p.gather + (size_t)p.gather_idx[row] * p.ld_gather + n));
      }
    }
  }
#pragma unroll
  for (int k = 0; k < ITEMS; ++k) {
    const int idx = te + k * TC_EPI_THREADS;
    const int r = idx / P4, c4 = idx - r * P4;
    const int row = rowq + r, n = n0 + 4 * c4;
    if (row >= p.M) continue;
    if (n < p.gt_cols) {
      const float4 o = make_float4(fast_sigmoid(x0[k].x + acc[k].x) * fast_tanh(x1[k].x), fast_sigmoid(x0[k].y + acc[k].y) * fast_tanh(x1[k].y),
                                   fast_sigmoid(x0[k].z + acc[k].z) * fast_tanh(x1[k].z), fast_sigmoid(x0[k].w + acc[k].w) * fast_tanh(x1[k].w));
      store4(p.g_t, p.g_tw, (size_t)row * p.ld_state + n, o);
    } else {
      float4 o = acc[k];
      add4(o, *reinterpret_cast<const float4*>(s_bias + 4 * c4));
      add4(o, x0[k]); add4(o, x1[k]); add4(o, x2[k]);
      *reinterpret_cast<float4*>(p.c + (size_t)row * p.ldc + n) = o;
    }
  }
}

template <int BN, int NG>
__device__ __forceinline__ void tile_cell(const TcProblem& p, const float* tile, const float* s_bias, int rowq, int n0_tile, int n_tile_,
                                          int te, int h = 0) {
  static_assert(BN % (NG * 32) == 0, "whole 32-unit chunks per tile");
  constexpr int CH = BN / (NG * 32);
  const int r = te >> 3, uq = te & 7;
  const int row = rowq + r;
  if (row >= p.M) return;
  const int n_tile = n_tile_ * CH + h;
  const int n0 = n0_tile + h * NG * 32;
  tile += 0; s_bias += h * NG * 32;
  const int cpiece = h * NG * 8;
  const int unit = n_tile * 32 + uq * 4;
  const size_t so = (size_t)row * p.ld_state + unit;
  float4 pre[NG], x0[NG], x1[NG], x2[NG];
  const float4 zero = make_float4(0.f, 0.f, 0.f, 0.f);
#ifdef VSR_DBG_CLK
  const long long k0 = clock64();
#endif
  const float4 cold = *reinterpret_cast<const float4*>(p.c_old + so);
  const float* radd = p.rowadd != nullptr ? p.rowadd + (size_t)((row / p.row_div) * p.rowadd_mul) * p.ld_rowadd + n0 + uq * 4 : nullptr;
  const float* cadd = p.cadd != nullptr ? p.cadd + (size_t)row * p.ld_cadd + n0 + uq * 4 : nullptr;
  const float* gath = p.gather != nullptr ? p.gather + (size_t)p.gather_idx[row] * p.ld_gather + n0 + uq * 4 : nullptr;
#pragma unroll
  for (int g = 0; g < NG; ++g) {
    pre[g] = *reinterpret_cast<const float4*>(tile + tile_slot<BN>(r, cpiece + g * 8 + uq));
    x0[g] = radd != nullptr ? __ldg(reinterpret_cast<const float4*>(radd + g * 32)) : zero;
    x1[g] = cadd != nullptr ? *reinterpret_cast<const float4*>(cadd + g * 32) : zero;
    x2[g] = gath != nullptr ? __ldg(reinterpret_cast<const float4*>(gath + g * 32)) : zero;
  }
#pragma unroll
  for (int g = 0; g < NG; ++g) {
    add4(pre[g], *reinterpret_cast<const float4*>(s_bias + g * 32 + uq * 4));
    add4(pre[g], x0[g]); add4(pre[g], x1[g]); add4(pre[g], x2[g]);
  }
#ifdef VSR_DBG_CLK
  const long long k1 = clock64();
#endif
  const float pi[4] = {pre[0].x, pre[0].y, pre[0].z, pre[0].w}, pf[4] = {pre[1].x, pre[1].y, pre[1].z, pre[1].w};
  const float pg[4] = {pre[2].x, pre[2].y, pre[2].z, pre[2].w}, po[4] = {pre[3].x, pre[3].y, pre[3].z, pre[3].w};
  const float co[4] = {cold.x, cold.y, cold.z, cold.w};
  float cn[4], hn[4], tc[4];
#pragma unroll
  for (int u = 0; u < 4; ++u) {
    const float ig = fast_sigmoid(pi[u]), fg = fast_sigmoid(pf[u]), gg = fast_tanh(pg[u]), og = fast_sigmoid(po[u]);
    cn[u] = fg * co[u] + ig * gg;
    tc[u] = fast_tanh(cn[u]);
    hn[u] = og * tc[u];
  }
#ifdef VSR_DBG_CLK
  const long long k2 = clock64();
#endif
  *reinterpret_cast<float4*>(p.c_new + so) = make_float4(cn[0], cn[1], cn[2], cn[3]);
  store4(p.h_new, p.h_tw, so, make_float4(hn[0], hn[1], hn[2], hn[3]));
  if constexpr (NG == 6) {
    const float ps[4] = {pre[4].x, pre[4].y, pre[4].z, pre[4].w};
    store4(p.s_new, p.s_tw, so, make_float4(fast_sigmoid(ps[0]) * tc[0], fast_sigmoid(ps[1]) * tc[1],
                                                     fast_sigmoid(ps[2]) * tc[2], fast_sigmoid(ps[3]) * tc[3]));
    *reinterpret_cast<float4*>(p.gq + so) = pre[5];
  }
#ifdef VSR_DBG_CLK
  if ((te == 0 || te == 200) && blockIdx.x == 5 && p.M > 200 && (rowq & 127) == 0)
    printf("cell NG=%d te=%d: loads+adds %lld math %lld stores %lld\n", NG, te, k1 - k0, k2 - k1, clock64() - k2);
#endif
}

template <int BN>
__device__ __forceinline__ void tile_epilogue(const TcProblem& p, uint32_t tmem_base, int m0, int n0, int n_tile, int warp, int lane,
                                              const float* s_bias, float* tile) {
  const int q = warp & 3, hsel = (warp - 2) >> 2, te = (warp - 2) * 32 + lane;
  const uint32_t tlane = tmem_base + ((uint32_t)(q * 32) << 16);
  const float sc = (p.acc_scale != nullptr ? __ldg(p.acc_scale) : 1.f) * p.act_inv;
#ifdef VSR_DBG_CLK
  long long td = 0, tb1 = 0, tp = 0, tb2 = 0;
#endif
#pragma unroll 1
  for (int qq = 0; qq < 4; ++qq) {
    if (m0 + qq * 32 >= p.M) break;
#ifdef VSR_DBG_CLK
    const long long c0 = clock64();
#endif
    if (q == qq) tile_dump<BN>(tlane, tile, hsel, lane, p.zero_acc != 0, sc);
#ifdef VSR_DBG_CLK
    const long long c1 = clock64();
#endif
    epi_bar(3);
#ifdef VSR_DBG_CLK
    const long long c2 = clock64();
#endif
    const int rowq = m0 + qq * 32;
    if (p.mode == EPI_PLAIN) tile_plain<BN>(p, tile, s_bias, rowq, n0, te);
    if constexpr (BN == 192) { if (p.mode == EPI_LSTM1) tile_cell<BN, 6>(p, tile, s_bias, rowq, n0, n_tile, te); }
    if constexpr (BN == 128) { if (p.mode == EPI_LSTM2) tile_cell<BN, 4>(p, tile, s_bias, rowq, n0, n_tile, te); }
    if constexpr (BN == 256) {
      if (p.mode == EPI_LSTM2) { tile_cell<BN, 4>(p, tile, s_bias, rowq, n0, n_tile, te, 0); tile_cell<BN, 4>(p, tile, s_bias, rowq, n0, n_tile, te, 1); }
    }
#ifdef VSR_DBG_CLK
    const long long c3 = clock64();
#endif
    epi_bar(4);
#ifdef VSR_DBG_CLK
    td += c1 - c0; tb1 += c2 - c1; tp += c3 - c2; tb2 += clock64() - c3;
#endif
  }
#ifdef VSR_DBG_CLK
  if (lane == 0 && (warp == 2 || warp == 4 || warp == 9) && blockIdx.x == 5 && p.M > 200)
    printf("epi BN=%d mode=%d warp=%d: dump %lld bar1 %lld process %lld bar2 %lld\n", BN, p.mode, warp, td, tb1, tp, tb2);
#endif
}

template <int BN>
__device__ __forceinline__ void vocab_epilogue(const TcProblem& p, uint32_t tlane, int row, bool live, int n0,
                                               const float* s_bias, int hsel) {
  constexpr int NCH = BN / 16, H0 = (NCH + 1) / 2;
  float* crow = p.c + (size_t)row * p.ldc;
  float2* rec = reinterpret_cast<float2*>(p.vpart) + (size_t)row * (p.ldc / 16) + n0 / 16;
  const float sc = (p.acc_scale != nullptr ? __ldg(p.acc_scale) : 1.f) * p.act_inv;
#pragma unroll
  for (int ch = 0; ch < NCH; ++ch) {
    if ((ch < H0) != (hsel == 0)) continue;
    uint32_t r[16];
    tmem_ld16(tlane + (uint32_t)(ch * 16), r);
    const int n = n0 + ch * 16;
    if (live) {
      float v[16];
#pragma unroll
      for (int j = 0; j < 16; j += 4) {
        const float4 b = *reinterpret_cast<const float4*>(s_bias + ch * 16 + j);
        v[j] = __uint_as_float(r[j]) * sc + b.x; v[j + 1] = __uint_as_float(r[j + 1]) * sc + b.y;
        v[j + 2] = __uint_as_float(r[j + 2]) * sc + b.z; v[j + 3] = __uint_as_float(r[j + 3]) * sc + b.w;
        *reinterpret_cast<float4*>(crow + n + j) = make_float4(v[j], v[j + 1], v[j + 2], v[j + 3]);
      }
      if (n + 16 > p.n_valid) {
#pragma unroll
        for (int j = 0; j < 16; ++j) if (n + j >= p.n_valid) v[j] = -INFINITY;
      }
      float cm = fmaxf(fmaxf(fmaxf(v[0], v[1]), fmaxf(v[2], v[3])), fmaxf(fmaxf(v[4], v[5]), fmaxf(v[6], v[7])));
      cm = fmaxf(cm, fmaxf(fmaxf(fmaxf(v[8], v[9]), fmaxf(v[10], v[11])), fmaxf(fmaxf(v[12], v[13]), fmaxf(v[14], v[15]))));
      float cs = 0.f;
      if (cm > -INFINITY) {
        float e0 = 0.f, e1 = 0.f, e2 = 0.f, e3 = 0.f;
#pragma unroll
        for (int j = 0; j < 16; j += 4) {
          e0 += __expf(v[j] - cm); e1 += __expf(v[j + 1] - cm); e2 += __expf(v[j + 2] - cm); e3 += __expf(v[j + 3] - cm);
        }
        cs = (e0 + e1) + (e2 + e3);
      }
      rec[ch] = make_float2(cm, cs);
    }
  }
}

template <int BN>
__device__ __forceinline__ void epi_bias(const TcProblem& p, int m0, int n0, int n_tile, int warp, int lane, float* s_bias,
                                         bool reuse) {
  if (reuse) epi_bar(1);
  const int te = (warp - 2) * 32 + lane;
  for (int i = te; i < BN; i += TC_EPI_THREADS) s_bias[i] = p.bias != nullptr ? __ldg(p.bias + n0 + i) : 0.f;
  if (p.mode == EPI_LSTM1 || p.mode == EPI_LSTM2) {
    const int r = te >> 3, g = te & 7;
#pragma unroll
    for (int qq = 0; qq < 4; ++qq) {
      const int row = m0 + qq * 32 + r;
      if (row >= p.M) break;
      const float* line = nullptr;
      if (g < BN / 32) {
        if (p.gather != nullptr) line = p.gather + (size_t)p.gather_idx[row] * p.ld_gather + n0 + g * 32;
      } else if (g == 6) {
        line = p.c_old + (size_t)row * p.ld_state + n_tile * 32;
      } else if (p.rowadd != nullptr) {
        line = p.rowadd + (size_t)((row / p.row_div) * p.rowadd_mul) * p.ld_rowadd + n0;
      }
      if (line != nullptr) asm volatile("prefetch.global.L2 [%0];" ::"l"(line));
    }
  }
  epi_bar(1);
}

template <int BN>
__device__ __forceinline__ void rowwise_plain(const TcProblem& p, uint32_t tmem_base, int m0, int n0, int warp, int lane,
                                              int hsel, int nsplit) {
  const int q = warp & 3;
  const int row = m0 + q * 32 + lane;
  const bool live = row < p.M;
  const uint32_t tlane = tmem_base + ((uint32_t)(q * 32) << 16);
  const float* radd = (p.rowadd != nullptr && live)
                          ? p.rowadd + (size_t)((row / p.row_div) * p.rowadd_mul) * p.ld_rowadd : nullptr;
  const float* cadd = (p.cadd != nullptr && live) ? p.cadd + (size_t)row * p.ld_cadd : nullptr;
  const float* gath = (p.gather != nullptr && live) ? p.gather + (size_t)p.gather_idx[row] * p.ld_gather : nullptr;
  float* crow = p.c + (size_t)row * p.ldc;
  constexpr int NCH = BN / 16;
  const float sc = (p.acc_scale != nullptr ? __ldg(p.acc_scale) : 1.f) * p.act_inv;
  const int c_lo = hsel * NCH / nsplit, c_hi = (hsel + 1) * NCH / nsplit;
#pragma unroll 1
  for (int ch = c_lo; ch < c_hi; ++ch) {
    uint32_t r[16];
    tmem_ld16(tlane + (uint32_t)(ch * 16), r);
    const int n = n0 + ch * 16;
    if (!live) continue;
#pragma unroll
    for (int j = 0; j < 16; j += 4) {
      float4 o = make_float4(__uint_as_float(r[j]) * sc, __uint_as_float(r[j + 1]) * sc, __uint_as_float(r[j + 2]) * sc,
                             __uint_as_float(r[j + 3]) * sc);
      if (p.bias != nullptr) add4(o, __ldg(reinterpret_cast<const float4*>(p.bias + n + j)));
      if (radd != nullptr) add4(o, __ldg(reinterpret_cast<const float4*>(radd + n + j)));
      if (cadd != nullptr) add4(o, *reinterpret_cast<const float4*>(cadd + n + j));
      if (gath != nullptr) add4(o, __ldg(reinterpret_cast<const float4*>(gath + n + j)));
      *reinterpret_cast<float4*>(crow + n + j) = o;
    }
  }
}

template <int BN, int KB>
__device__ __forceinline__ void tc_epilogue(const TcProblem& p, uint32_t tmem_base, int m0, int n0, int n_tile,
                                            int warp, int lane, const float* s_bias, float* tile) {
  using Cfg = TcCfg<BN, KB>;
  const int q = warp & 3, hsel = (warp - 2) >> 2;
  if (p.mode == EPI_VOCAB) {
    const int row = m0 + q * 32 + lane;
    vocab_epilogue<BN>(p, tmem_base + ((uint32_t)(q * 32) << 16), row, row < p.M, n0, s_bias, hsel);
  } else if constexpr (Cfg::kTileEpi) {
    tile_epilogue<BN>(p, tmem_base, m0, n0, n_tile, warp, lane, s_bias, tile);
  } else {
    rowwise_plain<BN>(p, tmem_base, m0, n0, warp, lane, hsel, 2);
  }
}

template <int BN, int KB>
__device__ __forceinline__ void load_w_stage(const TcProblem& p, uint64_t* bar, uint8_t* base, int kb, int n0) {
  using Cfg = TcCfg<BN, KB>;
  uint8_t* w = base + 2 * Cfg::kABytes;
  tma_load_2d(&p.w_hi, bar, w, kb * KB, n0);
  if (p.f8) {
    tma_load_2d(&p.w_h8, bar, w + Cfg::kWBytes, kb * KB, n0);
    tma_load_2d(&p.w_lo, bar, w + Cfg::kWBytes + Cfg::kWBytes / 2, kb * KB, n0);
  } else {
    tma_load_2d(&p.w_lo, bar, w + Cfg::kWBytes, kb * KB, n0);
  }
}
template <int BN, int KB>
__device__ __forceinline__ void load_a_stage(const TcProblem& p, uint64_t* bar, uint8_t* base, int seg, int kk, int m0) {
  using Cfg = TcCfg<BN, KB>;
  tma_load_2d(&p.a_hi[seg], bar, base, kk * KB, m0);
  if (p.f8) {
    tma_load_2d(&p.a_h8[seg], bar, base + Cfg::kABytes, kk * KB, m0);
    tma_load_2d(&p.a_lo[seg], bar, base + Cfg::kABytes + Cfg::kABytes / 2, kk * KB, m0);
  } else {
    tma_load_2d(&p.a_lo[seg], bar, base + Cfg::kABytes, kk * KB, m0);
  }
}
template <int BN, int KB>
__device__ __forceinline__ void issue_stage(const TcProblem& p, uint32_t tmem_acc, uint32_t base, bool first) {
  using Cfg = TcCfg<BN, KB>;
  constexpr uint32_t idesc = make_idesc<BN>();
  const uint64_t ah = make_kmajor_desc<KB>(base), wh = make_kmajor_desc<KB>(base + 2 * Cfg::kABytes);
  if (p.f8) {
    const uint64_t a8 = make_kmajor_desc8<KB>(base + Cfg::kABytes), al = make_kmajor_desc8<KB>(base + Cfg::kABytes + Cfg::kABytes / 2);
    const uint64_t w8 = make_kmajor_desc8<KB>(base + 2 * Cfg::kABytes + Cfg::kWBytes);
    const uint64_t wl = make_kmajor_desc8<KB>(base + 2 * Cfg::kABytes + Cfg::kWBytes + Cfg::kWBytes / 2);
#pragma unroll
    for (int k = 0; k < KB / UMMA_K; ++k) {
      const uint64_t off = (uint64_t)((k * UMMA_K * 2) >> 4);
      umma_f16(tmem_acc, ah + off, wh + off, idesc, (first && k == 0) ? 0u : 1u);
    }
#pragma unroll
    for (int k = 0; k < KB / 32; ++k) {
      const uint64_t off = (uint64_t)((k * 32) >> 4);
      umma_f8(tmem_acc, a8 + off, wl + off, idesc, 1u);
      umma_f8(tmem_acc, al + off, w8 + off, idesc, 1u);
    }
  } else {
    const uint64_t al = make_kmajor_desc<KB>(base + Cfg::kABytes), wl = make_kmajor_desc<KB>(base + 2 * Cfg::kABytes + Cfg::kWBytes);
#pragma unroll
    for (int k = 0; k < KB / UMMA_K; ++k) {
      const uint64_t off = (uint64_t)((k * UMMA_K * 2) >> 4);
      umma_f16(tmem_acc, ah + off, wh + off, idesc, (first && k == 0) ? 0u : 1u);
      umma_f16(tmem_acc, ah + off, wl + off, idesc, 1u);
      umma_f16(tmem_acc, al + off, wh + off, idesc, 1u);
    }
  }
}

template <int BN, int KB>
__global__ void __launch_bounds__(TC_THREADS, 1) k_gemm_tc(const __grid_constant__ TcParams params) {
  using Cfg = TcCfg<BN, KB>;
  extern __shared__ uint8_t smem_raw[];
  __shared__ __align__(8) uint64_t full_bar[Cfg::kStages];
  __shared__ __align__(8) uint64_t empty_bar[Cfg::kStages];
  __shared__ __align__(8) uint64_t tmem_full_bar;
  __shared__ uint32_t tmem_base_slot;
  __shared__ __align__(16) float s_bias[BN];

  const int warp = threadIdx.x >> 5, lane = threadIdx.x & 31;
  int t = blockIdx.x;
  const int tiles0 = params.pr[0].n_tiles * params.pr[0].m_tiles;
  const int pi = (params.nprob > 1 && t >= tiles0) ? 1 : 0;
  t -= pi * tiles0;
  const TcProblem& p = params.pr[pi];
  const int m_tile = t % p.m_tiles, n_tile = t / p.m_tiles;
  const int m0 = m_tile * BM, n0 = n_tile * BN;

  if (!(params.pdl_flags & 2)) pdl_trigger();
  if (p.row_skip != nullptr) {
// ... 403 lines not shown
              umma_f16_pair(tmem_acc, ah + off, wl + off, idesc, 1u);
              umma_f16_pair(tmem_acc, al + off, wh + off, idesc, 1u);
            }
          }
          umma_commit_pair(&empty_bar[st]);
        }
        umma_commit_pair(&tmem_full_bar[acc]);
      }
      __syncwarp();
    } else {
      if (ti != 0) epi_bar(1);
      for (int i = (warp - 2) * 32 + lane; i < BN; i += TC_EPI_THREADS) s_bias[i] = p.bias != nullptr ? __ldg(p.bias + n0 + i) : 0.f;
      epi_bar(1);
      mbar_wait(&tmem_full_bar[acc], aph);
      asm volatile("tcgen05.fence::after_thread_sync;" ::: "memory");
      if constexpr (VOCAB) {
        const int q = warp & 3, row = m0 + q * 32 + lane;
        vocab_epilogue<BN>(p, tmem_acc + ((uint32_t)(q * 32) << 16), row, row < p.M, n0, s_bias, (warp - 2) >> 2);
      } else {
        tile_epilogue<BN>(p, tmem_acc, m0, n0, n_tile, warp, lane, s_bias, reinterpret_cast<float*>(smem + Cfg::kRingBytes));
      }
      asm volatile("tcgen05.fence::before_thread_sync;" ::: "memory");
      __syncwarp();
      if (lane == 0) {
        if (rank == 0) mbar_arrive(&tmem_empty_bar[acc]); else mbar_arrive_cluster(&tmem_empty_bar[acc], 0);
      }
    }
    it += total_kb;
    ++ti;
  }
  asm volatile("tcgen05.fence::before_thread_sync;" ::: "memory");
  cluster_sync_all();
  if (warp == 1) {
    asm volatile("tcgen05.fence::after_thread_sync;" ::: "memory");
    asm volatile("tcgen05.dealloc.cta_group::2.sync.aligned.b32 %0, %1;" ::"r"(tmem_base), "r"(Cfg::kTmemCols) : "memory");
  }
}

typedef CUresult (*EncodeTiledFn)(CUtensorMap*, CUtensorMapDataType, cuuint32_t, void*, const cuuint64_t*,
                                  const cuuint64_t*, const cuuint32_t*, const cuuint32_t*, CUtensorMapInterleave,
                                  CUtensorMapSwizzle, CUtensorMapL2promotion, CUtensorMapFloatOOBfill);

EncodeTiledFn get_encode() {
  static EncodeTiledFn fn = nullptr;
  if (fn == nullptr) {
    void* sym = nullptr;
    cudaDriverEntryPointQueryResult q;
    if (cudaGetDriverEntryPoint("cuTensorMapEncodeTiled", &sym, cudaEnableDefault, &q) == cudaSuccess &&
        q == cudaDriverEntryPointSuccess)
      fn = (EncodeTiledFn)sym;
  }
  return fn;
}

}

int make_tmap_f16(void* out_map, const void* base, int rows, int cols, int ld, int box_rows, int kb) {
  EncodeTiledFn enc = get_encode();
  VSR_REQUIRE(enc != nullptr, VSR_ECUDA, "cuTensorMapEncodeTiled entry point not available");
  const cuuint64_t gdim[2] = {(cuuint64_t)cols, (cuuint64_t)rows};
  const cuuint64_t gstr[1] = {(cuuint64_t)ld * 2};
  const cuuint32_t box[2] = {(cuuint32_t)kb, (cuuint32_t)box_rows};
  const cuuint32_t estr[2] = {1, 1};
  CUresult r = enc((CUtensorMap*)out_map, CU_TENSOR_MAP_DATA_TYPE_FLOAT16, 2, const_cast<void*>(base), gdim, gstr,
                   box, estr, CU_TENSOR_MAP_INTERLEAVE_NONE, kb == 32 ? CU_TENSOR_MAP_SWIZZLE_64B : CU_TENSOR_MAP_SWIZZLE_128B,
                   CU_TENSOR_MAP_L2_PROMOTION_L2_256B, CU_TENSOR_MAP_FLOAT_OOB_FILL_NONE);
  VSR_REQUIRE(r == CUDA_SUCCESS, VSR_ECUDA, "cuTensorMapEncodeTiled failed (%d) rows=%d cols=%d ld=%d", (int)r, rows, cols, ld);
  return VSR_OK;
}

__global__ void k_absmax(const float* __restrict__ x, size_t n, unsigned* __restrict__ out) {
  float m = 0.f;
  for (size_t i = (size_t)blockIdx.x * blockDim.x + threadIdx.x; i < n; i += (size_t)gridDim.x * blockDim.x) {
    const float v = fabsf(x[i]);
    if (v == v && v < INFINITY) m = fmaxf(m, v);
  }
  for (int o = 16; o > 0; o >>= 1) m = fmaxf(m, __shfl_xor_sync(0xffffffffu, m, o));
  if ((threadIdx.x & 31) == 0 && m > 0.f) atomicMax(out, __float_as_uint(m));
}
__global__ void k_pick_scale(float* scale) {
  const float m = __uint_as_float(*reinterpret_cast<unsigned*>(scale));
  int e = 0;
  if (m > 0.f) { int ex; frexpf(m, &ex); e = 13 - ex; }
  e = e > 100 ? 100 : (e < -100 ? -100 : e);
  scale[0] = ldexpf(1.f, e);
  scale[1] = ldexpf(1.f, -e);
}

int make_tmap_u8(void* out_map, const void* base, int rows, int cols, int ld, int box_rows, int kb) {
  EncodeTiledFn enc = get_encode();
  VSR_REQUIRE(enc != nullptr, VSR_ECUDA, "cuTensorMapEncodeTiled entry point not available");
  const cuuint64_t gdim[2] = {(cuuint64_t)cols, (cuuint64_t)rows};
  const cuuint64_t gstr[1] = {(cuuint64_t)ld};
  const cuuint32_t box[2] = {(cuuint32_t)kb, (cuuint32_t)box_rows};
  const cuuint32_t estr[2] = {1, 1};
  CUresult r = enc((CUtensorMap*)out_map, CU_TENSOR_MAP_DATA_TYPE_UINT8, 2, const_cast<void*>(base), gdim, gstr,
                   box, estr, CU_TENSOR_MAP_INTERLEAVE_NONE, kb == 32 ? CU_TENSOR_MAP_SWIZZLE_32B : CU_TENSOR_MAP_SWIZZLE_64B,
                   CU_TENSOR_MAP_L2_PROMOTION_L2_256B, CU_TENSOR_MAP_FLOAT_OOB_FILL_NONE);
  VSR_REQUIRE(r == CUDA_SUCCESS, VSR_ECUDA, "cuTensorMapEncodeTiled (u8) failed (%d) rows=%d cols=%d ld=%d", (int)r, rows, cols, ld);
  return VSR_OK;
}

int make_pair_maps(F16Pair* b, int pair_rows) {
  b->pair_rows = 0;
  if (b->hi == nullptr || pair_rows <= 0) return VSR_OK;
  VSR_TRY(make_tmap_f16(b->pair_hi, b->hi, b->rows, b->ld, b->ld, pair_rows));
  if (b->lo != nullptr) VSR_TRY(make_tmap_f16(b->pair_lo16, b->lo, b->rows, b->ld, b->ld, pair_rows));
  if (b->hi8 != nullptr) {
    VSR_TRY(make_tmap_u8(b->pair_h8, b->hi8, b->rows, b->ld, b->ld, pair_rows));
    VSR_TRY(make_tmap_u8(b->pair_lo, b->lo8, b->rows, b->ld, b->ld, pair_rows));
  }
  b->pair_rows = pair_rows;
  return VSR_OK;
}

namespace {
__global__ void k_split_pair(const float* __restrict__ x, TwinOut o, size_t n4, const float* __restrict__ scale) {
  const size_t i = (size_t)blockIdx.x * blockDim.x + threadIdx.x;
  if (i >= n4) return;
  if (scale != nullptr) o.scale = scale[0];
  store_twin4(o, i * 4, *reinterpret_cast<const float4*>(x + i * 4));
}
}

int launch_split_pair(const float* x, const F16Pair& p, size_t n, cudaStream_t st, bool weight_scale) {
  if (n == 0 || p.hi == nullptr) return VSR_OK;
  VSR_REQUIRE(n % 4 == 0, VSR_EINVAL, "launch_split_pair: element count %zu not a multiple of 4", n);
  float* scale = weight_scale ? p.scale : nullptr;
  if (scale != nullptr) {
    VSR_CHECK_CUDA(cudaMemsetAsync(scale, 0, 2 * sizeof(float), st));
    k_absmax<<<296, 256, 0, st>>>(x, n, reinterpret_cast<unsigned*>(scale));
    k_pick_scale<<<1, 1, 0, st>>>(scale);
  }
  k_split_pair<<<(unsigned)((n / 4 + 255) / 256), 256, 0, st>>>(x, twin_out(&p), n / 4, scale);
  VSR_CHECK_CUDA(cudaGetLastError());
  return VSR_OK;
}

int tc_gemm_init() {
  static unsigned long long done_mask = 0ull;
  int dev = 0;
  VSR_CHECK_CUDA(cudaGetDevice(&dev));
  const bool done = dev < 64 && ((done_mask >> dev) & 1ull);
  if (done) return VSR_OK;
#define TC_SET_SMEM(BN_, KB_) VSR_CHECK_CUDA(cudaFuncSetAttribute(k_gemm_tc<BN_, KB_>, cudaFuncAttributeMaxDynamicSharedMemorySize, TcCfg<BN_, KB_>::kSmemBytes))
  TC_SET_SMEM(256, 64); TC_SET_SMEM(192, 64); TC_SET_SMEM(128, 64);
  TC_SET_SMEM(256, 32); TC_SET_SMEM(192, 32); TC_SET_SMEM(128, 32);
  TC_SET_SMEM(144, 64); TC_SET_SMEM(240, 32);
#define TCP_SET_SMEM(BN_, KB_) VSR_CHECK_CUDA(cudaFuncSetAttribute(k_gemm_tcp<BN_, KB_>, cudaFuncAttributeMaxDynamicSharedMemorySize, TcCfg<BN_, KB_>::kSmemBytes))
  TCP_SET_SMEM(128, 64); TCP_SET_SMEM(144, 64); TCP_SET_SMEM(192, 32); TCP_SET_SMEM(192, 64); TCP_SET_SMEM(128, 32);
#undef TCP_SET_SMEM
#undef TC_SET_SMEM
#define PAIR_SET_SMEM(BN_, KB_, V_) VSR_CHECK_CUDA(cudaFuncSetAttribute(k_gemm_pair<BN_, KB_, V_>, cudaFuncAttributeMaxDynamicSharedMemorySize, PairCfg<BN_, KB_, V_>::kSmemBytes))
  PAIR_SET_SMEM(192, 64, false); PAIR_SET_SMEM(192, 64, true); PAIR_SET_SMEM(256, 64, false);
#undef PAIR_SET_SMEM
  if (dev < 64) done_mask |= 1ull << dev;
  return VSR_OK;
}

static int fill_problem(TcProblem* p, const GemmArgs& g, int BN, int kb = 64, bool pair = false) {
  VSR_REQUIRE(g.M > 0 && g.N >= round_up(g.wb->n_valid, BN), VSR_EINVAL, "launch_gemm_tc: N=%d too small for N tile %d", g.N, BN);
  p->nseg = g.nseg;
  p->f8 = g.f8 ? 1 : 0;
  VSR_REQUIRE(g.f8 ? (g.wb->hi8 != nullptr && g.wb->lo8 != nullptr) : g.wb->lo != nullptr, VSR_EINVAL,
              "launch_gemm_tc: the weight has no %s twin", g.f8 ? "e4m3" : "fp16 residual");
  for (int s = 0; s < g.nseg; ++s) {
    const F16Pair* b = g.seg[s].b;
    VSR_REQUIRE(b != nullptr && g.seg[s].k % BK == 0, VSR_EINVAL, "launch_gemm_tc: segment %d not tensor-core ready", s);
    VSR_REQUIRE(g.f8 ? (b->hi8 != nullptr && b->lo8 != nullptr) : b->lo != nullptr, VSR_EINVAL,
                "launch_gemm_tc: segment %d has no %s twin", s, g.f8 ? "e4m3" : "fp16 residual");
    VSR_REQUIRE(b->act_scale == g.seg[0].b->act_scale, VSR_EINVAL, "launch_gemm_tc: segments with different activation scales");
    memcpy(&p->a_hi[s], kb == 32 ? b->map32_hi : b->map_hi, sizeof(CUtensorMap));
    if (g.f8) {
      memcpy(&p->a_h8[s], kb == 32 ? b->map8_32_hi : b->map8_hi, sizeof(CUtensorMap));
      memcpy(&p->a_lo[s], kb == 32 ? b->map8_32_lo : b->map8_lo, sizeof(CUtensorMap));
    } else {
      memcpy(&p->a_lo[s], kb == 32 ? b->map32_lo : b->map_lo, sizeof(CUtensorMap));
    }
    p->kblocks[s] = g.seg[s].k / kb;
  }
  const bool alt = !pair && BN == g.wb->alt_bn && BN != g.wb->box_rows;
  if (pair) {
    VSR_REQUIRE(g.wb->pair_rows * 2 == BN && kb == 64, VSR_EINVAL, "launch_gemm_tc: weight has no pair maps for N tile %d", BN);
    memcpy(&p->w_hi, g.wb->pair_hi, sizeof(CUtensorMap));
    memcpy(&p->w_lo, g.f8 ? g.wb->pair_lo : g.wb->pair_lo16, sizeof(CUtensorMap));
    if (g.f8) memcpy(&p->w_h8, g.wb->pair_h8, sizeof(CUtensorMap));
  } else {
  memcpy(&p->w_hi, alt ? g.wb->alt_hi : (kb == 32 ? g.wb->map32_hi : g.wb->map_hi), sizeof(CUtensorMap));
  if (g.f8) {
    memcpy(&p->w_h8, alt ? g.wb->alt8_hi : (kb == 32 ? g.wb->map8_32_hi : g.wb->map8_hi), sizeof(CUtensorMap));
    memcpy(&p->w_lo, alt ? g.wb->alt8_lo : (kb == 32 ? g.wb->map8_32_lo : g.wb->map8_lo), sizeof(CUtensorMap));
  } else {
    memcpy(&p->w_lo, alt ? g.wb->alt_lo : (kb == 32 ? g.wb->map32_lo : g.wb->map_lo), sizeof(CUtensorMap));
  }
  }
  p->acc_scale = g.wb->scale != nullptr ? g.wb->scale + 1 : nullptr;
  p->act_inv = 1.f / g.seg[0].b->act_scale;
  p->n_tiles = (g.wb->n_valid + BN - 1) / BN; p->m_tiles = (g.M + BM - 1) / BM; p->M = g.M; p->row_skip = g.row_skip;
  p->bias = g.bias; p->rowadd = g.rowadd; p->ld_rowadd = g.ld_rowadd; p->row_div = g.row_div > 0 ? g.row_div : 1;
  p->rowadd_mul = g.rowadd_mul; p->cadd = g.cadd; p->ld_cadd = g.ld_cadd; p->c = g.c; p->ldc = g.ldc;
  p->gather = g.gather; p->ld_gather = g.ld_gather; p->gather_idx = g.gather_idx;
  const FusedCell& f = g.cell;
  p->mode = f.mode;
  if (f.mode == EPI_VOCAB) {
    VSR_REQUIRE(f.vocab_part != nullptr && g.bias != nullptr && g.c != nullptr && g.ldc % 16 == 0 && g.N % BN == 0, VSR_EINVAL,
                "launch_gemm_tc: vocabulary epilogue needs a bias, an output padded to whole tiles and a record buffer (N tile %d)", BN);
    p->vpart = f.vocab_part; p->n_valid = g.wb->n_valid;
  } else if (f.mode != 0) {
    VSR_REQUIRE((f.mode == EPI_LSTM1 && BN == 192) || (f.mode == EPI_LSTM2 && (BN == 128 || (pair && BN == 256))), VSR_EINVAL,
                "launch_gemm_tc: fused cell mode %d does not fit N tile %d", f.mode, BN);
    p->c_old = f.c_old; p->c_new = f.c_new; p->h_new = f.h_new; p->h_tw = twin_out(f.h_b);
    p->s_new = f.s_new; p->s_tw = twin_out(f.s_b); p->gq = f.gq;
  }
  VSR_REQUIRE(f.gt_cols == 0 || BN == 128 || BN == 192 || (pair && BN == 256 && f.gt_cols % 256 == 0), VSR_EINVAL,
              "launch_gemm_tc: g_t fusion needs a 128- or 192-wide tile");
  p->zero_acc = g.zero_acc ? 1 : 0;
  p->ld_state = f.ld_state;
  p->gt_cols = f.gt_cols; p->gt_gq = f.gt_gq; p->gt_c1n = f.gt_c1n; p->g_t = f.g_t;
  p->g_tw = twin_out(f.g_b);
  return VSR_OK;
}

static bool pair_ok(const GemmArgs& g) {
  if (!g.allow_pair || g.wb == nullptr || g.wb->pair_rows <= 0 || g.M < g.pair_min_rows || g.row_skip != nullptr || g.zero_acc) return false;
  const int BN = 2 * g.wb->pair_rows;
  if (g.N % BN != 0 || (BN != 192 && BN != 256)) return false;
  const int mode = g.cell.mode;
  if (mode == EPI_VOCAB && BN != 192) return false;
  if (mode == EPI_LSTM1 && BN != 192) return false;
  if (mode == EPI_LSTM2 && BN != 256) return false;
  if (g.cell.gt_cols % BN != 0) return false;
  return true;
}

static int launch_gemm_pair(const GemmArgs& g, const GemmArgs* g2, cudaStream_t st) {
  const int BN = 2 * g.wb->pair_rows;
  const bool vocab = g.cell.mode == EPI_VOCAB;
  const int kb = 64;
  TcParams p;
  memset(&p, 0, sizeof(p));
  VSR_TRY(fill_problem(&p.pr[0], g, BN, kb, true));
  p.nprob = 1;
  int tiles = p.pr[0].n_tiles * ((p.pr[0].m_tiles + 1) / 2);
  if (g2 != nullptr) {
    VSR_TRY(fill_problem(&p.pr[1], *g2, BN, kb, true));
    p.nprob = 2;
    tiles += p.pr[1].n_tiles * ((p.pr[1].m_tiles + 1) / 2);
  }
  static int sms = 0;
  if (sms == 0) cudaDeviceGetAttribute(&sms, cudaDevAttrMultiProcessorCount, 0);
  const int clusters = tiles < sms / 2 ? tiles : sms / 2;
#define PAIR_LAUNCH(BN_, KB_, V_) VSR_CHECK_CUDA(launch_k(k_gemm_pair<BN_, KB_, V_>, dim3(2 * clusters), dim3(TC_THREADS), PairCfg<BN_, KB_, V_>::kSmemBytes, st, g.pdl, p))
  if (BN == 192 && vocab) PAIR_LAUNCH(192, 64, true);
  else if (BN == 192) PAIR_LAUNCH(192, 64, false);
  else PAIR_LAUNCH(256, 64, false);
#undef PAIR_LAUNCH
  VSR_CHECK_CUDA(cudaGetLastError());
  return VSR_OK;
}

int launch_gemm_tc(const GemmArgs& g, const GemmArgs* g2, cudaStream_t st) {
  VSR_TRY(tc_gemm_init());
  if (pair_ok(g) && (g2 == nullptr || (pair_ok(*g2) && g2->wb->pair_rows == g.wb->pair_rows))) return launch_gemm_pair(g, g2, st);
  int BN = g.wb->box_rows;
  VSR_REQUIRE(BN == 128 || BN == 192 || BN == 256, VSR_EINVAL, "launch_gemm_tc: unsupported N tile %d", BN);
  VSR_REQUIRE(g2 == nullptr || g2->wb->box_rows == BN, VSR_EINVAL, "launch_gemm_tc: grouped problems need one tile shape");
  TcParams p;
  memset(&p, 0, sizeof(p));
  int kb = g.wb->kb;
  VSR_REQUIRE(g2 == nullptr || g2->wb->kb == kb, VSR_EINVAL, "launch_gemm_tc: grouped problems need one k-block size");
  if (g.wb->alt_bn > 0 && !g.no_alt && (g.cell.mode == 0 || g.cell.mode == EPI_VOCAB) && (g2 == nullptr || (g2->wb->alt_bn == g.wb->alt_bn && g2->cell.mode == 0))) {
    int sms = 148;
    cudaDeviceGetAttribute(&sms, cudaDevAttrMultiProcessorCount, 0);
    const int mt = (g.M + BM - 1) / BM;
    auto cost = [&](int bn) {
      int tiles = mt * ((g.wb->n_valid + bn - 1) / bn);
      if (g2 != nullptr) tiles += ((g2->M + BM - 1) / BM) * ((g2->wb->n_valid + bn - 1) / bn);
      return ((tiles + sms - 1) / sms) * (BM + bn);
    };
    if (cost(g.wb->alt_bn) < cost(BN)) { BN = g.wb->alt_bn; kb = g.wb->alt_kb; }
  }
  VSR_TRY(fill_problem(&p.pr[0], g, BN, kb));
  p.nprob = 1;
  p.pdl_flags = g.pdl_flags;
  int tiles = p.pr[0].n_tiles * p.pr[0].m_tiles;
  if (g2 != nullptr) {
    VSR_TRY(fill_problem(&p.pr[1], *g2, BN, kb));
    p.nprob = 2;
    tiles += p.pr[1].n_tiles * p.pr[1].m_tiles;
  }
  static int persist = -1, sms = 148;
  if (persist < 0) {
    const char* e = getenv("VSRDEC_PERSIST");
    persist = (e == nullptr) ? 1 : atoi(e);
    cudaDeviceGetAttribute(&sms, cudaDevAttrMultiProcessorCount, 0);
  }
  if (persist && tiles > sms && g2 == nullptr && (BN == 128 || BN == 144 || BN == 192)) {
    const int grid = tiles < sms ? tiles : sms;
#define TCP_LAUNCH(BN_, KB_) VSR_CHECK_CUDA(launch_k(k_gemm_tcp<BN_, KB_>, dim3(grid), dim3(TC_THREADS), TcCfg<BN_, KB_>::kSmemBytes, st, g.pdl, p))
    if (BN == 144) TCP_LAUNCH(144, 64);
    else if (BN == 192) { if (kb == 32) TCP_LAUNCH(192, 32); else TCP_LAUNCH(192, 64); }
    else { if (kb == 32) TCP_LAUNCH(128, 32); else TCP_LAUNCH(128, 64); }
#undef TCP_LAUNCH
    VSR_CHECK_CUDA(cudaGetLastError());
    return VSR_OK;
  }
#define TC_LAUNCH(BN_, KB_) VSR_CHECK_CUDA(launch_k(k_gemm_tc<BN_, KB_>, dim3(tiles), dim3(TC_THREADS), TcCfg<BN_, KB_>::kSmemBytes, st, g.pdl, p))
  if (BN == 144) TC_LAUNCH(144, 64);
  else if (BN == 240) TC_LAUNCH(240, 32);
  else if (kb == 32) {
    if (BN == 256) TC_LAUNCH(256, 32); else if (BN == 192) TC_LAUNCH(192, 32); else TC_LAUNCH(128, 32);
  } else {
    if (BN == 256) TC_LAUNCH(256, 64); else if (BN == 192) TC_LAUNCH(192, 64); else TC_LAUNCH(128, 64);
  }
#undef TC_LAUNCH
  VSR_CHECK_CUDA(cudaGetLastError());
  return VSR_OK;
}

}
```

vsr-guided-cic_b200/csrc/step_kernels.cu:

```cuda
#include <float.h>
#include <math.h>

#include <cuda_fp16.h>

#include <cstdlib>
#include <cstring>
#include "common.cuh"
#include "vocab_head.cuh"

namespace vsr {

namespace {

__device__ __forceinline__ float sigmoidf_(float x) { return 1.f / (1.f + expf(-x)); }

using PairOut = TwinOut;
__device__ __forceinline__ void store_pair(const PairOut& o, size_t i, float v) {
  if (o.hi == nullptr) return;
  v = fminf(fmaxf(v * o.scale, -65504.f), 65504.f);
  const __half h = __float2half_rn(v);
  reinterpret_cast<__half*>(o.hi)[i] = h;
  const float r = v - __half2float(h);
  if (o.lo != nullptr) reinterpret_cast<__half*>(o.lo)[i] = __float2half_rn(r);
  if (o.hi8 != nullptr) {
// ... 343 lines not shown
#pragma unroll
    for (int u = 0; u < PRE; ++u) {
      const int j = j0 + u * THREADS;
      q[u] = j < n4 ? *reinterpret_cast<const float4*>(x + j * 4) : make_float4(-INFINITY, -INFINITY, -INFINITY, -INFINITY);
    }
    float bm = -INFINITY;
#pragma unroll
    for (int u = 0; u < PRE; ++u) {
      const int v0 = (j0 + u * THREADS) * 4;
      if (v0 + 3 >= V) {
        if (v0 + 1 >= V) q[u].y = -INFINITY;
        if (v0 + 2 >= V) q[u].z = -INFINITY;
        q[u].w = -INFINITY;
        if (v0 >= V) q[u].x = -INFINITY;
      }
      const float e4[4] = {q[u].x, q[u].y, q[u].z, q[u].w};
#pragma unroll
      for (int e = 0; e < 4; ++e) {
        const float val = e4[e];
        bm = fmaxf(bm, val);
        if (val > v2) {
          if (val > v1) { v2 = v1; i2 = i1; v1 = val; i1 = v0 + e; } else { v2 = val; i2 = v0 + e; }
        }
      }
    }
    if (bm > m) { ssum *= __expf(m - bm); m = bm; }
    if (m > -INFINITY) {
#pragma unroll
      for (int u = 0; u < PRE; ++u)
        ssum += (__expf(q[u].x - m) + __expf(q[u].y - m)) + (__expf(q[u].z - m) + __expf(q[u].w - m));
    }
  }
  {
    const float wm = warp_max(m);
    const float ws = warp_sum(m > -INFINITY ? ssum * expf(m - wm) : 0.f);
    const float wg = warp_sum(stay_part);
    if (lane == 0) { red_m[warp] = wm; red_s[warp] = ws; red_g[warp] = wg; }
  }
  {
    int head = 0;
    for (int j = 0; j < topk; ++j) {
      const float hv = head == 0 ? v1 : (head == 1 ? v2 : -INFINITY);
      const int hi = head == 0 ? i1 : (head == 1 ? i2 : 0x7fffffff);
      unsigned kb; int ib;
      warp_argbest_redux(hv, hi, kb, ib);
      const bool mine = hi == ib && ib != 0x7fffffff;
      if (mine) { wl_v[warp][j] = hv; wl_i[warp][j] = hi; wl_second[warp][j] = head; ++head; }
      if (ib == 0x7fffffff && lane == 0) { wl_v[warp][j] = -INFINITY; wl_i[warp][j] = 0x7fffffff; wl_second[warp][j] = 0; }
    }
  }
  if (tid == 0) s_slow = 0;
  __syncthreads();

  float mx = red_m[0];
#pragma unroll
  for (int w = 1; w < NW; ++w) mx = fmaxf(mx, red_m[w]);
  float se = 0.f;
#pragma unroll
  for (int w = 0; w < NW; ++w) se += red_s[w] * expf(red_m[w] - mx);
  const float lsum = logf(se);

  if (warp == 0) {
    float cvv[2] = {-INFINITY, -INFINITY}; int cii[2] = {0x7fffffff, 0x7fffffff}; int csec[2] = {0, 0};
#pragma unroll
    for (int q = 0; q < 2; ++q) {
      const int e = lane + 32 * q;
      if (e < NW * topk) { cvv[q] = wl_v[e / topk][e % topk]; cii[q] = wl_i[e / topk][e % topk]; csec[q] = wl_second[e / topk][e % topk]; }
    }
    int slow = 0;
    for (int j = 0; j < topk; ++j) {
      const bool first = before(cvv[0], cii[0], cvv[1], cii[1]);
      const float hv = first ? cvv[0] : cvv[1];
      const int hi = first ? cii[0] : cii[1];
      unsigned kb; int ib;
      warp_argbest_redux(hv, hi, kb, ib);
      if (hi == ib && ib != 0x7fffffff) {
        slow |= first ? csec[0] : csec[1];
        if (first) { cvv[0] = -INFINITY; cii[0] = 0x7fffffff; } else { cvv[1] = -INFINITY; cii[1] = 0x7fffffff; }
      }
      if (lane == 0) s_pick[j] = ib;
    }
    slow = __any_sync(0xffffffffu, slow != 0);
    if (lane == 0) s_slow = slow;
  }

  if (tid == 0) {
    int forced = -1;
    if (verb != -1) {
      if (a.gt) {
        forced = (int)verb;
      } else {
        forced = 0;
        int lo = 0, hi = a.vt_n - 1, pos = -1;
        while (lo <= hi) {
          const int mid = (lo + hi) >> 1;
          const int64_t k = a.vt_keys[mid];
          if (k == verb) { pos = mid; break; }
          if (k < verb) lo = mid + 1; else hi = mid - 1;
        }
        if (pos >= 0 && a.vt_off[pos + 1] > a.vt_off[pos]) {
          float best = -1e6f; int best_i = -1;
          for (int qq = a.vt_off[pos]; qq < a.vt_off[pos + 1]; ++qq) {
            const int idx = a.vt_idx[qq];
            const float lp = (x[idx] - mx) - lsum;
            if (lp > best) { best = lp; best_i = idx; }
          }
          forced = best_i < 0 ? V - 1 : best_i;
        }
      }
      forced = min(max(forced, 0), V - 1);
    }
    s_forced = forced;
    if (gate_head) {
    a.row_max[n] = mx;
    a.row_lsum[n] = lsum;
    a.forced[n] = forced;
    float g0, g1;
    if (forced >= 0) { g0 = -1e3f; g1 = 0.f; }
    else {
      float stay = 0.f;
#pragma unroll
      for (int w = 0; w < NW; ++w) stay += red_g[w];
      const float gm = fmaxf(stay, shift_logit);
      const float ls = logf(expf(stay - gm) + expf(shift_logit - gm));
      g0 = (stay - gm) - ls; g1 = (shift_logit - gm) - ls;
    }
    a.gate_lp[(size_t)n * 2] = g0; a.gate_lp[(size_t)n * 2 + 1] = g1;
    if (a.gate_out != nullptr) {
      a.gate_out[(size_t)n * a.gate_stride + 0] = g0;
      a.gate_out[(size_t)n * a.gate_stride + 1] = g1;
    }
    }
  }
  if (a.out_logp == nullptr && topk <= 0) return;
  __syncthreads();
  const int forced = s_forced;

  if (a.out_logp != nullptr) {
    float* o = a.out_logp + (size_t)n * a.out_stride;
    for (int v = tid; v < V; v += THREADS)
      o[v] = forced >= 0 ? (v == forced ? 0.f : -1e6f) : (x[v] - mx) - lsum;
  }
  if (topk <= 0) return;

  int32_t* cd = a.cand + (size_t)n * VSR_MAX_BEAM;
  if (forced >= 0) {
    if (tid == 0) {
      cd[0] = forced;
      int v = 0;
      for (int j = 1; j < topk; ++j) { if (v == forced) ++v; cd[j] = min(v, V - 1); ++v; }
    }
    return;
  }
  if (!s_slow) {
    if (tid < topk) cd[tid] = s_pick[tid];
    return;
  }
  float cv = v1; int ci = i1;
  for (int j = 0; j < topk; ++j) {
    float bv = cv; int bi = ci;
    warp_argbest(bv, bi);
    if (lane == 0) { red_v[j & 1][warp] = bv; red_i[j & 1][warp] = bi; }
    __syncthreads();
    bv = red_v[j & 1][0]; bi = red_i[j & 1][0];
#pragma unroll
    for (int w = 1; w < NW; ++w)
      if (before(red_v[j & 1][w], red_i[j & 1][w], bv, bi)) { bv = red_v[j & 1][w]; bi = red_i[j & 1][w]; }
    if (tid == 0) cd[j] = bi;
    if (ci == bi) {
      cv = -INFINITY; ci = 0x7fffffff;
      for (int jj = tid; jj < n4; jj += THREADS) {
        const float4 qq = *reinterpret_cast<const float4*>(x + jj * 4);
        const int v0 = jj * 4;
        const float e4[4] = {qq.x, qq.y, qq.z, qq.w};
#pragma unroll
        for (int u = 0; u < 4; ++u)
          if (v0 + u < V && before(bv, bi, e4[u], v0 + u) && before(e4[u], v0 + u, cv, ci)) { cv = e4[u]; ci = v0 + u; }
      }
    }
  }
}

constexpr int VM_WARPS = 4;
__global__ void __launch_bounds__(VM_WARPS * 32) k_vocab_merge(const SoftmaxArgs a, const float* __restrict__ vpart, int n_chunks) {
  const int lane = threadIdx.x & 31;
  const int n = blockIdx.x * VM_WARPS + (threadIdx.x >> 5);
  pdl_trigger();
  pdl_wait();
  if (n >= a.rows) return;
  RowHead h;
  merge_row(a, vpart, n_chunks, n, lane, h);
  if (lane == 0) {
    a.row_max[n] = h.mx; a.row_lsum[n] = h.lsum; a.forced[n] = h.forced;
    a.gate_lp[(size_t)n * 2] = h.g0; a.gate_lp[(size_t)n * 2 + 1] = h.g1;
    if (a.gate_out != nullptr) {
      a.gate_out[(size_t)n * a.gate_stride + 0] = h.g0;
      a.gate_out[(size_t)n * a.gate_stride + 1] = h.g1;
    }
  }
  if (lane < a.topk) a.cand[(size_t)n * VSR_MAX_BEAM + lane] = h.pick;
}

__global__ void __launch_bounds__(128) k_gate_head(const float* __restrict__ ha, int ld_ha, const float* __restrict__ ga, int ld_ga,
                                                   const float* __restrict__ v_g, int A, const float* __restrict__ shift,
                                                   float* __restrict__ gate_out, int64_t gate_stride, int rows) {
  const int lane = threadIdx.x & 31;
  const int n = blockIdx.x * 4 + (threadIdx.x >> 5);
  if (n >= rows) return;
  const float4* h4 = reinterpret_cast<const float4*>(ha + (size_t)n * ld_ha);
  const float4* g4 = reinterpret_cast<const float4*>(ga + (size_t)n * ld_ga);
  const float4* v4 = reinterpret_cast<const float4*>(v_g);
  float stay = 0.f;
  for (int i = lane; i < A / 4; i += 32) {
    const float4 h = h4[i], g = g4[i], w = __ldg(v4 + i);
    stay += (w.x * fast_tanh(g.x + h.x) + w.y * fast_tanh(g.y + h.y)) + (w.z * fast_tanh(g.z + h.z) + w.w * fast_tanh(g.w + h.w));
  }
  stay = warp_sum(stay);
  if (lane == 0) {
    const float sh = shift[n];
    const float gm = fmaxf(stay, sh);
    const float ls = logf(expf(stay - gm) + expf(sh - gm));
    gate_out[(size_t)n * gate_stride] = (stay - gm) - ls;
    gate_out[(size_t)n * gate_stride + 1] = (sh - gm) - ls;
  }
}

struct RowScatter { int n; const uint4* src[3]; uint4* dst[3]; int vec[3]; };
__global__ void __launch_bounds__(128) k_rows_to_all(const RowScatter r, int T, int t) {
  const int i = blockIdx.x;
  for (int q = 0; q < r.n; ++q) {
    const uint4* s = r.src[q] + (size_t)i * r.vec[q];
    uint4* d = r.dst[q] + ((size_t)i * T + t) * r.vec[q];
    for (int e = threadIdx.x; e < r.vec[q]; e += blockDim.x) d[e] = s[e];
  }
}

}

int launch_gate_head(Ctx* c, int rows, float* gate_out, int64_t gate_stride, cudaStream_t st) {
  k_gate_head<<<(rows + 3) / 4, 128, 0, st>>>(c->hb + c->oB2_ha, c->NB2, c->ga, c->NC, c->v_g, c->A, c->shift, gate_out, gate_stride, rows);
  VSR_CHECK_CUDA(cudaGetLastError()); c->launches++;
  return VSR_OK;
}

int launch_rows_to_all(Ctx* c, const F16Pair& src, const F16Pair& dst, int rows, int T, int t, cudaStream_t st) {
  RowScatter r{};
  auto add = [&](const void* s, void* d, int bytes) {
    if (s == nullptr || d == nullptr) return;
    r.src[r.n] = (const uint4*)s; r.dst[r.n] = (uint4*)d; r.vec[r.n] = c->Hp * bytes / 16; ++r.n;
  };
  add(src.hi, dst.hi, 2); add(src.lo, dst.lo, 2); add(src.hi8, dst.hi8, 1); add(src.lo8, dst.lo8, 1);
  k_rows_to_all<<<rows, 128, 0, st>>>(r, T, t);
  VSR_CHECK_CUDA(cudaGetLastError()); c->launches++;
  return VSR_OK;
}

int run_vocab_rows(Ctx* c, const F16Pair& a_b, float* logits, int M, float* out_logp, cudaStream_t st, bool softmax_only) {
  if (!softmax_only) {
    PhaseScope ps(c, PH_GEMM_E, st);
    GemmArgs g{};
    g.nseg = 1; g.seg[0] = {nullptr, c->Hp, c->Hp, c->Hp, &a_b};
    g.w = c->WE; g.ldw = c->Hp; g.bias = c->bE; g.wb = &c->WE_b;
    g.c = logits; g.ldc = c->NE; g.M = M; g.N = c->NE;
    g.f8 = c->gemm_f8; g.allow_pair = true; g.no_alt = true;
    VSR_TRY(launch_gemm(c, g, st)); c->launches++;
    return VSR_OK;
  }
  PhaseScope ps(c, PH_SOFTMAX_TOPK, st);
  SoftmaxArgs a{};
  a.logits = logits; a.ld = c->NE; a.rows = M; a.V = c->V; a.cur_beam = 1; a.L = c->L; a.topk = 0;
  a.out_logp = out_logp; a.out_stride = c->V;
  k_softmax_topk<<<M, SM_THREADS, 0, st>>>(a);
  VSR_CHECK_CUDA(cudaGetLastError()); c->launches++;
  return VSR_OK;
}

static PairOut pair_out(const Ctx* c, const F16Pair& b) { return twin_out(&b, c->use_tc); }

int run_step(Ctx* c, const StepIO& io, cudaStream_t st) {
  const int rows = io.rows, H = c->H;
  VSR_REQUIRE(rows > 0 && rows <= c->cap_rows, VSR_ESTATE, "run_step: rows=%d cap=%d", rows, c->cap_rows);
  VSR_REQUIRE(c->R <= ATT_MAX_R, VSR_EINVAL, "max_detections per slot R=%d > %d", c->R, ATT_MAX_R);
  const bool h2f = c->d.h2_first_lstm != 0;
  const dim3 pw_grid((H + 127) / 128, rows);
  bool fused = false;

  {
    PhaseScope ps(c, PH_GEMM_A, st);
    GemmArgs g{};
    int s = 0;
    if (h2f) g.seg[s++] = {c->h2, c->Hp, c->Hp, c->Hp, &c->h2_b};
    g.seg[s++] = {c->h1, c->Hp, c->Hp, c->Hp, &c->h1_b};
    g.nseg = s;
    g.w = c->WA; g.ldw = c->KA; g.wb = &c->WA_b;
    g.gather = c->X; g.ld_gather = c->NA; g.gather_idx = c->word_idx;
    g.rowadd = c->U; g.ld_rowadd = c->NA; g.row_div = io.cur_beam; g.rowadd_mul = (c->n_img == 1 ? 0 : 1);
    g.c = c->pre1; g.ldc = c->NA; g.M = rows; g.N = c->NA;
    g.zero_acc = io.zero_state;
    g.pdl = c->use_pdl && (c->pdl_mode & 1); g.pdl_flags = ((c->pdl_mode & 4) ? 1 : 0) | ((c->pdl_mode & 8) ? 2 : 0);
    g.allow_pair = true;
    g.f8 = c->gemm_f8 && c->use_pair; g.pair_min_rows = 1;
    fused = gemm_uses_tc(c, g);
    c->state_h32 = !fused || io.need_h32;
    if (fused) {
      g.cell.mode = 1; g.cell.c_old = c->c1; g.cell.c_new = c->c1n; g.cell.h_new = io.need_h32 ? c->h1n : nullptr;
      g.cell.h_b = &c->h1n_b;
      g.cell.s_new = nullptr; g.cell.s_b = &c->s_t_b;
      g.cell.gq = c->gq; g.cell.ld_state = c->Hp;
    }
    VSR_TRY(launch_gemm(c, g, st)); c->launches++;
  }
  if (!fused) {
    PhaseScope ps(c, PH_LSTM1, st);
    k_lstm1<<<pw_grid, 128, 0, st>>>(c->pre1, c->NA, c->c1, c->h1n, c->c1n, c->s_t, c->gq, pair_out(c, c->h1n_b),
                                     pair_out(c, c->s_t_b), c->Hp, H, rows);
    VSR_CHECK_CUDA(cudaGetLastError()); c->launches++;
  }
  {
    PhaseScope ps(c, PH_GEMM_B, st);
    GemmArgs g{};
    g.nseg = 1; g.seg[0] = {c->s_t, c->Hp, c->Hp, c->Hp, &c->s_t_b};
    g.w = c->WB1; g.ldw = c->Hp; g.bias = c->bB1; g.wb = &c->WB1_b;
    g.c = c->sent; g.ldc = c->NB1; g.M = rows; g.N = c->NB1;
    GemmArgs g2{};
    g2.nseg = 1; g2.seg[0] = {c->h1n, c->Hp, c->Hp, c->Hp, &c->h1n_b};
    g2.w = c->WB2; g2.ldw = c->Hp; g2.wb = &c->WB2_b; g2.f8 = c->gemm_f8; g2.allow_pair = true; g2.pair_min_rows = c->pair_min_rows;
    g2.c = c->hb; g2.ldc = c->NB2; g2.M = rows; g2.N = c->NB2;
    if (fused) {
      g2.cell.gt_cols = c->oB2_ha; g2.cell.gt_gq = c->gq; g2.cell.gt_c1n = c->c1n; g2.cell.g_t = nullptr;
      g2.cell.g_b = &c->g_t_b; g2.cell.ld_state = c->Hp;
    }
    g.pdl = c->use_pdl && (c->pdl_mode & 1); g.pdl_flags = ((c->pdl_mode & 4) ? 1 : 0) | ((c->pdl_mode & 8) ? 2 : 0);
    g.f8 = c->gemm_f8; g.allow_pair = true; g.pair_min_rows = c->pair_min_rows;
    VSR_TRY(launch_gemm(c, g, st, &g2)); c->launches += fused ? 1 : 2;
  }
  if (!fused) {
    PhaseScope ps(c, PH_GT, st);
    k_gt<<<pw_grid, 128, 0, st>>>(c->gq, c->hb, c->NB2, c->c1n, c->g_t, pair_out(c, c->g_t_b), c->Hp, H, rows);
    VSR_CHECK_CUDA(cudaGetLastError()); c->launches++;
  }
  {
    PhaseScope ps(c, PH_ATTEND, st);
    AttendArgs a{};
    a.det_seqs = c->det_seqs; a.P = c->P; a.slot_mask = c->slot_mask; a.ptr = c->ptr;
    a.slot_base = c->p_compact ? c->slot_base : nullptr;
    a.slot_index = c->slot_index; a.det = c->det; a.det_stride = c->det_stride; a.D = c->D;
    a.img = c->img; a.ld_img = c->Fp; a.Pmean = c->Pmean; a.img_mul = (c->n_img == 1 ? 0 : 1);
    a.sent = c->sent; a.ld_sent = c->NB1; a.o_sa = c->oB1_sa;
    a.hb = c->hb; a.ld_hb = c->NB2; a.o_ha = c->oB2_ha;
    a.v_a = c->v_a; a.v_s = c->v_s;
    a.att = fused ? nullptr : c->att; a.ld_att = c->Fp; a.att_b = pair_out(c, c->att_b); a.shift = c->shift;
    a.rows = rows; a.cur_beam = io.cur_beam; a.L = c->L; a.R = c->R; a.F = c->F; a.A = c->A; a.H = H;
    a.ldP = c->NVA;
    const size_t smem = sizeof(float) * ((size_t)c->A + (size_t)c->R * c->A + c->R + 1);
    if (!c->attend_attr_set) {
      VSR_CHECK_CUDA(cudaFuncSetAttribute(k_attend, cudaFuncAttributeMaxDynamicSharedMemorySize, 200 * 1024));
      c->attend_attr_set = true;
    }
    VSR_REQUIRE(smem <= 200 * 1024, VSR_EINVAL, "attention tile (R=%d x A=%d) does not fit shared memory", c->R, c->A);
    VSR_CHECK_CUDA(launch_k(k_attend, dim3(rows), dim3(ATT_THREADS), smem, st, c->use_pdl && (c->pdl_mode & 2), a));
    VSR_CHECK_CUDA(cudaGetLastError()); c->launches++;
  }
  {
    PhaseScope ps(c, PH_GEMM_D, st);
    GemmArgs gc{};
    gc.nseg = 1; gc.seg[0] = {c->g_t, c->Hp, c->Hp, c->Hp, &c->g_t_b};
    gc.w = c->WC; gc.ldw = c->Hp; gc.wb = &c->WC_b; gc.f8 = c->gemm_f8; gc.allow_pair = true; gc.pair_min_rows = c->pair_min_rows;
    gc.c = c->ga; gc.ldc = c->NC; gc.M = rows; gc.N = c->NC;
    GemmArgs g{};
    g.nseg = io.zero_state ? 2 : 3;
    g.seg[0] = {c->att, c->Fp, c->Fp, c->Fp, &c->att_b};
    g.seg[1] = {c->h1n, c->Hp, c->Hp, c->Hp, &c->h1n_b};
    g.seg[2] = {c->h2, c->Hp, c->Hp, c->Hp, &c->h2_b};
    g.w = c->WD; g.ldw = c->KD; g.bias = c->bD; g.wb = &c->WD_b;
    if (c->d.img_second_lstm) {
      g.rowadd = c->U2; g.ld_rowadd = c->ND; g.row_div = io.cur_beam; g.rowadd_mul = (c->n_img == 1 ? 0 : 1);
    }
    g.c = c->pre2; g.ldc = c->ND; g.M = rows; g.N = c->ND;
    if (fused) {
      g.cell.mode = 2; g.cell.c_old = c->c2; g.cell.c_new = c->c2n; g.cell.h_new = io.need_h32 ? c->h2n : nullptr;
      g.cell.h_b = &c->h2n_b; g.cell.ld_state = c->Hp;
    }
    g.pdl = c->use_pdl && (c->pdl_mode & 1); g.pdl_flags = ((c->pdl_mode & 4) ? 1 : 0) | ((c->pdl_mode & 8) ? 2 : 0);
    g.f8 = c->gemm_f8; g.allow_pair = true; g.pair_min_rows = c->pair_min_rows;
    VSR_TRY(launch_gemm(c, g, st, &gc)); c->launches += fused ? 1 : 2;
  }
  if (!fused) {
    PhaseScope ps(c, PH_LSTM2, st);
    k_lstm2<<<pw_grid, 128, 0, st>>>(c->pre2, c->ND, c->c2, c->h2n, c->c2n, pair_out(c, c->h2n_b), c->Hp, H, rows);
    VSR_CHECK_CUDA(cudaGetLastError()); c->launches++;
  }
  if (io.skip_vocab) return VSR_OK;
  static const bool fuse_enabled = [] { const char* e = getenv("VSRDEC_FUSE_VOCAB"); return e == nullptr || atoi(e) != 0; }();
  const bool fuse_vocab = fuse_enabled && fused && io.out_logp == nullptr && io.topk > 0;
  {
    PhaseScope ps(c, PH_GEMM_E, st);
    GemmArgs g{};
    g.nseg = 1; g.seg[0] = {c->h2n, c->Hp, c->Hp, c->Hp, &c->h2n_b};
    g.w = c->WE; g.ldw = c->Hp; g.bias = c->bE; g.wb = &c->WE_b;
    g.c = c->logits; g.ldc = c->NE; g.M = rows; g.N = c->NE;
    g.pdl = c->use_pdl && (c->pdl_mode & 1); g.pdl_flags = ((c->pdl_mode & 4) ? 1 : 0) | ((c->pdl_mode & 8) ? 2 : 0);
    g.f8 = c->gemm_f8; g.allow_pair = true; g.pair_min_rows = c->pair_min_rows;
    if (fuse_vocab) {
      g.cell.mode = 3; g.cell.vocab_part = c->vpart;
    }
    VSR_TRY(launch_gemm(c, g, st)); c->launches++;
  }
  {
    PhaseScope ps(c, PH_SOFTMAX_TOPK, st);
    SoftmaxArgs a = make_softmax_args(c, rows, io.cur_beam, io.topk, io.use_verbs, io.gt);
    a.out_logp = io.out_logp; a.out_stride = io.out_stride;
    a.gate_out = io.gate_out; a.gate_stride = io.gate_stride;
    if (fuse_vocab) {
      VSR_CHECK_CUDA(launch_k(k_vocab_merge, dim3((rows + VM_WARPS - 1) / VM_WARPS), dim3(VM_WARPS * 32), 0, st, c->use_pdl && (c->pdl_mode & 2),
                              a, (const float*)c->vpart, c->NE / 16));
    } else {
      VSR_CHECK_CUDA(launch_k(k_softmax_topk, dim3(rows), dim3(SM_THREADS), 0, st, c->use_pdl && (c->pdl_mode & 2), a));
    }
    VSR_CHECK_CUDA(cudaGetLastError()); c->launches++;
  }
  return VSR_OK;
}

}
```

vsr-guided-cic_b200/csrc/vocab_head.cuh:

```cuda
#pragma once
#include <math.h>

#include "common.cuh"

namespace vsr {
namespace {

__device__ __forceinline__ float warp_sum(float v) {
#pragma unroll
  for (int o = 16; o > 0; o >>= 1) v += __shfl_xor_sync(0xffffffffu, v, o);
  return v;
}
__device__ __forceinline__ float warp_max(float v) {
#pragma unroll
  for (int o = 16; o > 0; o >>= 1) v = fmaxf(v, __shfl_xor_sync(0xffffffffu, v, o));
  return v;
}

__device__ __forceinline__ int64_t load_verb(const void* verbs, int dtype, size_t i) {
  if (dtype == VSR_DT_F64) return (int64_t) reinterpret_cast<const double*>(verbs)[i];
  if (dtype == VSR_DT_F32) return (int64_t) reinterpret_cast<const float*>(verbs)[i];
  return reinterpret_cast<const int64_t*>(verbs)[i];
}

__device__ __forceinline__ bool before(float v1, int i1, float v2, int i2) {
  return v1 > v2 || (v1 == v2 && i1 < i2);
}
__device__ __forceinline__ void warp_argbest(float& bv, int& bi) {
#pragma unroll
  for (int o = 16; o > 0; o >>= 1) {
    const float ov = __shfl_xor_sync(0xffffffffu, bv, o);
    const int oi = __shfl_xor_sync(0xffffffffu, bi, o);
    if (before(ov, oi, bv, bi)) { bv = ov; bi = oi; }
  }
}
__device__ __forceinline__ unsigned orderable(float v) {
  const unsigned u = __float_as_uint(v);
  return (u & 0x80000000u) ? ~u : (u | 0x80000000u);
}
__device__ __forceinline__ void warp_argbest_redux(float v, int i, unsigned& kbest, int& ibest) {
  const unsigned key = orderable(v);
  kbest = __reduce_max_sync(0xffffffffu, key);
  ibest = (int)__reduce_min_sync(0xffffffffu, key == kbest ? (unsigned)i : 0xffffffffu);
}

struct SoftmaxArgs {
  const float* logits; int ld;
  int rows, V, cur_beam, L, topk;
  const int32_t* ptr;
  const void* verbs; int verbs_dtype; int use_verbs, gt;
  const int64_t* vt_keys; const int32_t* vt_off; const int32_t* vt_idx; int vt_n;
  const float* ha; int ld_ha;
  const float* ga; int ld_ga;
  const float* v_g; int A;
  const float* shift;
  float* row_max; float* row_lsum; int32_t* forced; int32_t* cand;
  float* gate_lp;
  float* out_logp; int64_t out_stride;
  float* gate_out; int64_t gate_stride;
};

inline SoftmaxArgs make_softmax_args(const Ctx* c, int rows, int cur_beam, int topk, bool use_verbs, bool gt) {
  SoftmaxArgs a{};
  a.logits = c->logits; a.ld = c->NE; a.rows = rows; a.V = c->V; a.cur_beam = cur_beam; a.L = c->L;
  a.topk = topk; a.ptr = c->ptr;
  a.verbs = c->verbs; a.verbs_dtype = c->verbs_dtype; a.use_verbs = use_verbs; a.gt = gt;
  a.vt_keys = c->vt_keys; a.vt_off = c->vt_off; a.vt_idx = c->vt_idx; a.vt_n = c->vt_n;
  a.ha = c->hb + c->oB2_ha; a.ld_ha = c->NB2; a.ga = c->ga; a.ld_ga = c->NC; a.v_g = c->v_g; a.A = c->A;
  a.shift = c->shift;
  a.row_max = c->row_max; a.row_lsum = c->row_lsum; a.forced = c->forced; a.cand = c->cand;
  a.gate_lp = c->gate_lp;
  return a;
}

__device__ __forceinline__ int forced_word(const SoftmaxArgs& a, int64_t verb, const float* x, float mx, float lsum) {
  if (verb == -1) return -1;
  const int V = a.V;
  int forced;
  if (a.gt) {
    forced = (int)verb;
  } else {
    forced = 0;
    int lo = 0, hi = a.vt_n - 1, pos = -1;
    while (lo <= hi) {
      const int mid = (lo + hi) >> 1;
      const int64_t k = a.vt_keys[mid];
      if (k == verb) { pos = mid; break; }
      if (k < verb) lo = mid + 1; else hi = mid - 1;
    }
    if (pos >= 0 && a.vt_off[pos + 1] > a.vt_off[pos]) {
      float best = -1e6f; int best_i = -1;
      for (int qq = a.vt_off[pos]; qq < a.vt_off[pos + 1]; ++qq) {
        const int idx = a.vt_idx[qq];
        const float lp = (x[idx] - mx) - lsum;
        if (lp > best) { best = lp; best_i = idx; }
      }
      forced = best_i < 0 ? V - 1 : best_i;
    }
  }
  return min(max(forced, 0), V - 1);
}

struct RowHead {
  float mx, lsum;
  int forced;
  float g0, g1;
  int pick;
  float pick_logit;
};

constexpr int VM_CPL = 24;

__device__ __forceinline__ void merge_row(const SoftmaxArgs& a, const float* __restrict__ vpart, int n_chunks,
                                          int n, int lane, RowHead& out) {
  const int V = a.V, topk = a.topk;
  const float2* rec = reinterpret_cast<const float2*>(vpart) + (size_t)n * n_chunks;
  const float* x = a.logits + (size_t)n * a.ld;
  const int used = (V + 15) >> 4;

  int64_t verb = -1; float shift_logit = 0.f;
  if (lane == 0) {
    shift_logit = a.shift[n];
    if (a.use_verbs && a.verbs != nullptr)
      verb = load_verb(a.verbs, a.verbs_dtype, (size_t)(n / a.cur_beam) * a.L + a.ptr[n]);
  }
  const bool in_regs = used <= 32 * VM_CPL;
  float cmx[VM_CPL];
  float m = -INFINITY, ssum = 0.f;
  if (in_regs) {
    float2 ms[VM_CPL];
#pragma unroll
    for (int q = 0; q < VM_CPL; ++q) {
      const int t = lane + 32 * q;
      ms[q] = t < used ? rec[t] : make_float2(-INFINITY, 0.f);
    }
#pragma unroll
    for (int q = 0; q < VM_CPL; ++q) {
      cmx[q] = ms[q].x;
      if (ms[q].x > m) { ssum *= __expf(m - ms[q].x); m = ms[q].x; }
      if (ms[q].x > -INFINITY) ssum += ms[q].y * __expf(ms[q].x - m);
    }
  } else {
    for (int t = lane; t < used; t += 32) {
      const float2 r2 = rec[t];
      if (r2.x > m) { ssum *= __expf(m - r2.x); m = r2.x; }
      if (r2.x > -INFINITY) ssum += r2.y * __expf(r2.x - m);
    }
  }
  float stay = 0.f;
  {
    const float4* ha = reinterpret_cast<const float4*>(a.ha + (size_t)n * a.ld_ha);
    const float4* ga = reinterpret_cast<const float4*>(a.ga + (size_t)n * a.ld_ga);
    const float4* vg = reinterpret_cast<const float4*>(a.v_g);
    for (int i = lane; i < a.A / 4; i += 32) {
      const float4 h = ha[i], g = ga[i], w = __ldg(vg + i);
      stay += (w.x * fast_tanh(g.x + h.x) + w.y * fast_tanh(g.y + h.y)) + (w.z * fast_tanh(g.z + h.z) + w.w * fast_tanh(g.w + h.w));
    }
  }
  const float mx = warp_max(m);
  const float se = warp_sum(m > -INFINITY ? ssum * expf(m - mx) : 0.f);
  const float lsum = logf(se);
  stay = warp_sum(stay);

  unsigned long long prev = ~0ull;
  int my_chunk = -1;
  for (int j = 0; j < topk; ++j) {
    unsigned long long best = 0ull;
    if (in_regs) {
#pragma unroll
      for (int q = 0; q < VM_CPL; ++q) {
        const int t = lane + 32 * q;
        const unsigned long long key = ((unsigned long long)orderable(cmx[q]) << 32) | (unsigned)(~(unsigned)t);
        if (cmx[q] > -INFINITY && key < prev && key > best) best = key;
      }
    } else {
      for (int t = lane; t < used; t += 32) {
        const float cm = rec[t].x;
        const unsigned long long key = ((unsigned long long)orderable(cm) << 32) | (unsigned)(~(unsigned)t);
        if (cm > -INFINITY && key < prev && key > best) best = key;
      }
    }
    const unsigned hi = __reduce_max_sync(0xffffffffu, (unsigned)(best >> 32));
    const unsigned lo = __reduce_max_sync(0xffffffffu, (unsigned)(best >> 32) == hi ? (unsigned)best : 0u);
    prev = ((unsigned long long)hi << 32) | lo;
    if (hi == 0u && lo == 0u) break;
    if (lane == j) my_chunk = (int)(~lo);
  }
  constexpr int EQ = VSR_MAX_BEAM * 16 / 32;
  float cv[EQ]; int ci[EQ];
#pragma unroll
  for (int q = 0; q < EQ; ++q) {
    const int e = lane + 32 * q;
    const int chunk = __shfl_sync(0xffffffffu, my_chunk, (e >> 4) & 31);
    cv[q] = -INFINITY; ci[q] = 0x7fffffff;
    if (e < topk * 16 && chunk >= 0) {
      const int col = chunk * 16 + (e & 15);
      if (col < V) { cv[q] = x[col]; ci[q] = col; }
    }
  }
  int my_pick = 0x7fffffff; float my_logit = -INFINITY;
  for (int j = 0; j < topk; ++j) {
    float bv = -INFINITY; int bi = 0x7fffffff;
#pragma unroll
    for (int q = 0; q < EQ; ++q) if (before(cv[q], ci[q], bv, bi)) { bv = cv[q]; bi = ci[q]; }
    unsigned kb; int ib;
    warp_argbest_redux(bv, bi, kb, ib);
    const float wv = __shfl_sync(0xffffffffu, bv, __ffs(__ballot_sync(0xffffffffu, bi == ib)) - 1);
#pragma unroll
    for (int q = 0; q < EQ; ++q) if (ci[q] == ib) { cv[q] = -INFINITY; ci[q] = 0x7fffffff; }
    if (lane == j) { my_pick = ib; my_logit = wv; }
  }

  int forced = -1;
  float g0 = 0.f, g1 = 0.f;
  if (lane == 0) {
    forced = forced_word(a, verb, x, mx, lsum);
    if (forced >= 0) { g0 = -1e3f; g1 = 0.f; }
    else {
      const float gm = fmaxf(stay, shift_logit);
      const float ls = logf(expf(stay - gm) + expf(shift_logit - gm));
      g0 = (stay - gm) - ls; g1 = (shift_logit - gm) - ls;
    }
  }
  forced = __shfl_sync(0xffffffffu, forced, 0);
  g0 = __shfl_sync(0xffffffffu, g0, 0);
  g1 = __shfl_sync(0xffffffffu, g1, 0);
  if (forced >= 0 && lane < topk) {
    int w = forced;
    if (lane > 0) { w = lane - 1; if (w >= forced) ++w; w = min(w, V - 1); }
    my_pick = w;
  }
  out.mx = mx; out.lsum = lsum; out.forced = forced; out.g0 = g0; out.g1 = g1; out.pick = my_pick; out.pick_logit = my_logit;
}

}
}
```

Baseline: 42920.

## Extract per-tile top-k vocabulary candidates in GEMM epilogue and skip full logits store

The vocabulary GEMM epilogue now keeps a running per-thread top-k with a sorting network and emits per-tile candidate keys. The merge kernel reduces over these keys instead of rescanning chunk maxima and rereading logits. Full logits are written only when forced words or verbs need them, which cuts global stores. The vocab pair tile moves from 192 to 256 and the padding from 1152 to 2304. Beam select reuses the cached candidate logits. The cost is a second TMEM pass and a larger register footprint in the epilogue.

```diff
diff --git a/vsr-guided-cic_b200/csrc/api.cu b/vsr-guided-cic_b200/csrc/api.cu
--- a/vsr-guided-cic_b200/csrc/api.cu
+++ b/vsr-guided-cic_b200/csrc/api.cu
@@ -120,10 +120,11 @@
   const int cap = round_up(rows, MPAD);
   float** bufs[] = {&c->h1, &c->c1, &c->h2, &c->c2, &c->h1n, &c->c1n, &c->h2n, &c->c2n, &c->pre1,
                     &c->s_t, &c->g_t, &c->gq, &c->sent, &c->hb, &c->ga, &c->att, &c->pre2, &c->logits, &c->gate_lp,
-                    &c->row_max, &c->row_lsum, &c->shift, &c->vpart};
+                    &c->row_max, &c->row_lsum, &c->shift, &c->vpart, &c->cand_logit};
   for (float** p : bufs) { dev_free(c, *p); *p = nullptr; }
   dev_free(c, c->word_idx);
   dev_free(c, c->ptr); dev_free(c, c->ptrn); dev_free(c, c->forced); dev_free(c, c->cand); dev_free(c, c->word_in);
+  dev_free(c, c->vcand);
   c->cap_rows = 0;
   const size_t n = cap;
   ALLOC_F(c->h1, n * c->Hp); ALLOC_F(c->c1, n * c->Hp); ALLOC_F(c->h2, n * c->Hp); ALLOC_F(c->c2, n * c->Hp);
@@ -135,10 +136,12 @@
   ALLOC_F(c->att, n * c->Fp); ALLOC_F(c->pre2, n * c->ND); ALLOC_F(c->logits, n * c->NE);
   ALLOC_F(c->gate_lp, n * 2); ALLOC_F(c->row_max, n); ALLOC_F(c->row_lsum, n); ALLOC_F(c->shift, n);
   ALLOC_F(c->vpart, n * (size_t)(c->NE / 16) * 2);
+  ALLOC_F(c->cand_logit, n * VSR_MAX_BEAM);
   VSR_TRY(dev_alloc(c, (void**)&c->ptr, sizeof(int32_t) * n));
   VSR_TRY(dev_alloc(c, (void**)&c->ptrn, sizeof(int32_t) * n));
   VSR_TRY(dev_alloc(c, (void**)&c->forced, sizeof(int32_t) * n));
   VSR_TRY(dev_alloc(c, (void**)&c->cand, sizeof(int32_t) * n * VSR_MAX_BEAM));
+  VSR_TRY(dev_alloc(c, (void**)&c->vcand, sizeof(unsigned long long) * n * (size_t)(c->NE / 64) * VSR_MAX_BEAM));
   VSR_TRY(dev_alloc(c, (void**)&c->word_in, sizeof(int64_t) * n));
   const PairKind sk = step_kind(c), hk = sk == PAIR_F8 ? PAIR_BOTH : sk;
   VSR_TRY(alloc_pair(c, &c->h1_b, cap, c->Hp, MPAD, hk)); VSR_TRY(alloc_pair(c, &c->h2_b, cap, c->Hp, MPAD, hk));
@@ -205,7 +208,7 @@
   c->NB2 = pad_rows(c->NB2v, 128, 0);
   c->NC = round_up(c->A, NPAD);
   c->ND = 4 * c->Hp;
-  c->NE = round_up(c->V, 1152);
+  c->NE = round_up(c->V, 2304);
   c->NVA = round_up(c->A, NPAD);
   c->KA = (d->h2_first_lstm ? c->Hp : 0) + c->Hp;
   c->KD = c->Fp + 2 * c->Hp;
@@ -243,7 +246,7 @@
   if (const char* e = getenv("VSRDEC_PAIR_MIN_ROWS")) c->pair_min_rows = atoi(e);
   if (c->use_pair && c->use_tc) {
     VSR_TRY(make_pair_maps(&c->WA_b, 96)); VSR_TRY(make_pair_maps(&c->WB1_b, 128)); VSR_TRY(make_pair_maps(&c->WB2_b, 128));
-    VSR_TRY(make_pair_maps(&c->WC_b, 128)); VSR_TRY(make_pair_maps(&c->WD_b, 128)); VSR_TRY(make_pair_maps(&c->WE_b, 96));
+    VSR_TRY(make_pair_maps(&c->WC_b, 128)); VSR_TRY(make_pair_maps(&c->WD_b, 128)); VSR_TRY(make_pair_maps(&c->WE_b, 128));
   }
   c->WA_b.kb = 32;
   if (const char* e = getenv("VSRDEC_KB_A")) c->WA_b.kb = atoi(e) == 32 ? 32 : 64;
@@ -453,6 +456,7 @@
     const int rows = b * cur;
     StepIO io{};
     io.rows = rows; io.cur_beam = cur; io.use_verbs = use_verbs != 0; io.gt = gt != 0; io.topk = k;
+    io.keep_logits = have_forced || (use_verbs && !gt);
     io.zero_state = t == 0 && c->zero_state_opt;
     if (tr && tr->step_out) { io.out_logp = tr->step_out + (size_t)t * b * k * c->V; io.out_stride = c->V; }
     if (tr && tr->step_gate) { io.gate_out = tr->step_gate + (size_t)t * b * k * 2; io.gate_stride = 2; }
diff --git a/vsr-guided-cic_b200/csrc/beam.cu b/vsr-guided-cic_b200/csrc/beam.cu
--- a/vsr-guided-cic_b200/csrc/beam.cu
+++ b/vsr-guided-cic_b200/csrc/beam.cu
@@ -22,7 +22,7 @@
   int t, b, cur, k, V;
   int64_t eos0, eos1;
   const float* logits; int ld;
-  const float* row_max; const float* row_lsum; const int32_t* forced; const int32_t* cand;
+  const float* row_max; const float* row_lsum; const int32_t* forced; const int32_t* cand; const float* cand_logit;
   const float* gate_lp;
   const float* seq_lp; float* seq_lp_n;
   float *m0, *m1, *m0n, *m1n;
@@ -36,13 +36,13 @@
 constexpr int MAXC = 2 * VSR_MAX_BEAM * VSR_MAX_BEAM;
 
 struct BeamSmem {
-  float seq[VSR_MAX_BEAM], m0[VSR_MAX_BEAM], m1[VSR_MAX_BEAM], ps[VSR_MAX_BEAM];
+  float seq[VSR_MAX_BEAM], m0[VSR_MAX_BEAM], m1[VSR_MAX_BEAM], ps[VSR_MAX_BEAM], pl[VSR_MAX_BEAM];
   int full[VSR_MAX_BEAM], pb[VSR_MAX_BEAM], pw[VSR_MAX_BEAM], pg[VSR_MAX_BEAM];
 };
 
 __device__ __forceinline__ void beam_select_warp(const BeamArgs& a, BeamSmem& sh, int c, int lane, bool write) {
   const int k = a.k, cur = a.cur;
-  float* s_seq = sh.seq; float* s_m0 = sh.m0; float* s_m1 = sh.m1; float* s_ps = sh.ps;
+  float* s_seq = sh.seq; float* s_m0 = sh.m0; float* s_m1 = sh.m1; float* s_ps = sh.ps; float* s_pl = sh.pl;
   int* s_full = sh.full; int* s_pb = sh.pb; int* s_pw = sh.pw; int* s_pg = sh.pg;
 
   if (lane < cur) {
@@ -58,32 +58,35 @@
   __syncwarp();
 
   if (a.f_beam == nullptr) {
-    float cs[MAXC / 32]; int cf[MAXC / 32]; bool used[MAXC / 32];
+    float cs[MAXC / 32], cl[MAXC / 32]; int cf[MAXC / 32]; bool used[MAXC / 32];
     const int ncand = cur * k * 2;
 #pragma unroll
     for (int q = 0; q < MAXC / 32; ++q) {
       const int idx = lane + 32 * q;
-      cs[q] = -INFINITY; cf[q] = 0x7fffffff; used[q] = true;
+      cs[q] = -INFINITY; cl[q] = 0.f; cf[q] = 0x7fffffff; used[q] = true;
       if (idx < ncand) {
         const int j = idx / (2 * k), i = (idx >> 1) % k, g = idx & 1;
         const int row = c * cur + j;
-        int word; float sc;
+        int word; float sc, wl;
         if (s_full[j]) {
           word = a.cand[row * VSR_MAX_BEAM + i];
-          const float wl = row_logp(a.logits, a.ld, a.row_max, a.row_lsum, a.forced, row, word);
+          const int f = a.forced[row];
+          wl = f >= 0 ? (word == f ? 0.f : -1e6f)
+                      : (a.cand_logit[row * VSR_MAX_BEAM + i] - a.row_max[row]) - a.row_lsum[row];
           sc = __fadd_rn(s_seq[j], __fadd_rn(wl, a.gate_lp[row * 2 + g]));
         } else {
           word = i;
+          wl = row_logp(a.logits, a.ld, a.row_max, a.row_lsum, a.forced, row, word);
           sc = (i == 0) ? s_seq[j] : -999.f;
         }
-        cs[q] = sc; cf[q] = j * 2 * a.V + word * 2 + g; used[q] = false;
+        cs[q] = sc; cl[q] = wl; cf[q] = j * 2 * a.V + word * 2 + g; used[q] = false;
       }
     }
     for (int sel = 0; sel < k; ++sel) {
-      float bv = -INFINITY; int bf = 0x7fffffff;
+      float bv = -INFINITY, bl = 0.f; int bf = 0x7fffffff;
 #pragma unroll
       for (int q = 0; q < MAXC / 32; ++q)
-        if (!used[q] && before(cs[q], cf[q], bv, bf)) { bv = cs[q]; bf = cf[q]; }
+        if (!used[q] && before(cs[q], cf[q], bv, bf)) { bv = cs[q]; bl = cl[q]; bf = cf[q]; }
       {
         const unsigned u = __float_as_uint(bv);
         const unsigned key = (u & 0x80000000u) ? ~u : (u | 0x80000000u);
@@ -91,26 +94,27 @@
         const int fbest = (int)__reduce_min_sync(0xffffffffu, key == kbest ? (unsigned)bf : 0xffffffffu);
         const unsigned owner = __ballot_sync(0xffffffffu, key == kbest && bf == fbest);
         bv = __shfl_sync(0xffffffffu, bv, __ffs(owner) - 1);
+        bl = __shfl_sync(0xffffffffu, bl, __ffs(owner) - 1);
         bf = fbest;
       }
 #pragma unroll
       for (int q = 0; q < MAXC / 32; ++q) if (cf[q] == bf) used[q] = true;
       if (lane == 0) {
         const int j = bf / (2 * a.V), rem = bf - j * 2 * a.V;
-        s_pb[sel] = j; s_pw[sel] = rem >> 1; s_pg[sel] = rem & 1; s_ps[sel] = bv;
+        s_pb[sel] = j; s_pw[sel] = rem >> 1; s_pg[sel] = rem & 1; s_ps[sel] = bv; s_pl[sel] = bl;
       }
     }
   } else if (lane < k) {
     const int j = a.f_beam[c * k + lane], word = a.f_word[c * k + lane], g = a.f_gate[c * k + lane];
     const int row = c * cur + j;
+    const float wl = row_logp(a.logits, a.ld, a.row_max, a.row_lsum, a.forced, row, word);
     float sc;
     if (s_full[j]) {
-      const float wl = row_logp(a.logits, a.ld, a.row_max, a.row_lsum, a.forced, row, word);
       sc = __fadd_rn(s_seq[j], __fadd_rn(wl, a.gate_lp[row * 2 + g]));
     } else {
       sc = (word == 0) ? s_seq[j] : -999.f;
     }
-    s_pb[lane] = j; s_pw[lane] = word; s_pg[lane] = g; s_ps[lane] = sc;
+    s_pb[lane] = j; s_pw[lane] = word; s_pg[lane] = g; s_ps[lane] = sc; s_pl[lane] = wl;
   }
   __syncwarp();
 
@@ -118,7 +122,7 @@
     const int j = s_pb[lane], word = s_pw[lane], g = s_pg[lane];
     const int row = c * cur + j;
     const int o = c * k + lane;
-    float lw = row_logp(a.logits, a.ld, a.row_max, a.row_lsum, a.forced, row, word);
+    float lw = s_pl[lane];
     float lg = a.gate_lp[row * 2 + g];
     if (a.t > 0) { lw *= s_m0[j]; lg *= s_m1[j]; }
     a.sel_beam[o] = j; a.sel_word[o] = word; a.sel_gate[o] = g;
@@ -368,7 +372,7 @@
   BeamArgs a{};
   a.t = t; a.b = b; a.cur = cur; a.k = k; a.V = c->V; a.eos0 = eos0; a.eos1 = eos1;
   a.logits = c->logits; a.ld = c->NE; a.row_max = c->row_max; a.row_lsum = c->row_lsum;
-  a.forced = c->forced; a.cand = c->cand; a.gate_lp = c->gate_lp;
+  a.forced = c->forced; a.cand = c->cand; a.cand_logit = c->cand_logit; a.gate_lp = c->gate_lp;
   a.seq_lp = c->seq_lp; a.seq_lp_n = c->seq_lp_n;
   a.m0 = c->m0; a.m1 = c->m1; a.m0n = c->m0n; a.m1n = c->m1n;
   a.prev_word = c->sel_word; a.prev_gate = c->sel_gate;
diff --git a/vsr-guided-cic_b200/csrc/common.cuh b/vsr-guided-cic_b200/csrc/common.cuh
--- a/vsr-guided-cic_b200/csrc/common.cuh
+++ b/vsr-guided-cic_b200/csrc/common.cuh
@@ -152,9 +152,9 @@
   int ld_state = 0;
   int gt_cols = 0; const float* gt_gq = nullptr; const float* gt_c1n = nullptr;
   float* g_t = nullptr;
-  float* vocab_part = nullptr; int* vocab_tiles_out = nullptr; int* vocab_bn_out = nullptr;
-};
-constexpr int VOCAB_REC = 16;
+  float* vocab_part = nullptr; unsigned long long* vocab_cand = nullptr; int vocab_topk = 0;
+  bool vocab_logits = false; int* vocab_lists_out = nullptr;
+};
 
 struct GemmArgs {
   GemmSeg seg[3];
@@ -278,7 +278,9 @@
   float *row_max, *row_lsum;
   int32_t *forced;
   int32_t *cand;
+  float *cand_logit;
   float *vpart;
+  unsigned long long *vcand;
   int cap_caps = 0, cap_T = 0;
   float *seq_lp, *seq_lp_n;
   float *m0, *m1, *m0n, *m1n;
@@ -340,6 +342,7 @@
   bool zero_state;
   bool skip_vocab;
   bool need_h32;
+  bool keep_logits;
 };
 int run_step(Ctx* c, const StepIO& io, cudaStream_t st);
 
diff --git a/vsr-guided-cic_b200/csrc/gemm_tc.cu b/vsr-guided-cic_b200/csrc/gemm_tc.cu
--- a/vsr-guided-cic_b200/csrc/gemm_tc.cu
+++ b/vsr-guided-cic_b200/csrc/gemm_tc.cu
@@ -149,7 +149,7 @@
   float* s_new; TwinOut s_tw; float* gq;
   int ld_state;
   int gt_cols; const float* gt_gq; const float* gt_c1n; float* g_t; TwinOut g_tw;
-  float* vpart; int n_valid;
+  float* vpart; unsigned long long* vcand; int n_valid, cand_k, c_full;
   int zero_acc;
   const float* acc_scale;
   float act_inv;
@@ -345,6 +345,10 @@
 #endif
 }
 
+__device__ __forceinline__ unsigned vocab_orderable(float v) {
+  const unsigned u = __float_as_uint(v);
+  return (u & 0x80000000u) ? ~u : (u | 0x80000000u);
+}
 template <int BN>
 __device__ __forceinline__ void vocab_epilogue(const TcProblem& p, uint32_t tlane, int row, bool live, int n0,
                                                const float* s_bias, int hsel) {
@@ -352,9 +356,12 @@
   float* crow = p.c + (size_t)row * p.ldc;
   float2* rec = reinterpret_cast<float2*>(p.vpart) + (size_t)row * (p.ldc / 16) + n0 / 16;
   const float sc = (p.acc_scale != nullptr ? __ldg(p.acc_scale) : 1.f) * p.act_inv;
-#pragma unroll
-  for (int ch = 0; ch < NCH; ++ch) {
-    if ((ch < H0) != (hsel == 0)) continue;
+  unsigned t[VSR_MAX_BEAM];
+#pragma unroll
+  for (int s = 0; s < VSR_MAX_BEAM; ++s) t[s] = 0u;
+  const int c_lo = hsel == 0 ? 0 : H0, c_hi = hsel == 0 ? H0 : NCH;
+#pragma unroll 1
+  for (int ch = c_lo; ch < c_hi; ++ch) {
     uint32_t r[16];
     tmem_ld16(tlane + (uint32_t)(ch * 16), r);
     const int n = n0 + ch * 16;
@@ -365,11 +372,18 @@
         const float4 b = *reinterpret_cast<const float4*>(s_bias + ch * 16 + j);
         v[j] = __uint_as_float(r[j]) * sc + b.x; v[j + 1] = __uint_as_float(r[j + 1]) * sc + b.y;
         v[j + 2] = __uint_as_float(r[j + 2]) * sc + b.z; v[j + 3] = __uint_as_float(r[j + 3]) * sc + b.w;
-        *reinterpret_cast<float4*>(crow + n + j) = make_float4(v[j], v[j + 1], v[j + 2], v[j + 3]);
+        if (p.c_full || n + j < VSR_MAX_BEAM)
+          *reinterpret_cast<float4*>(crow + n + j) = make_float4(v[j], v[j + 1], v[j + 2], v[j + 3]);
       }
       if (n + 16 > p.n_valid) {
 #pragma unroll
         for (int j = 0; j < 16; ++j) if (n + j >= p.n_valid) v[j] = -INFINITY;
+      }
+#pragma unroll
+      for (int j = 0; j < 16; ++j) {
+        unsigned x = n + j < p.n_valid ? vocab_orderable(v[j]) : 0u;
+#pragma unroll
+        for (int s = 0; s < VSR_MAX_BEAM; ++s) { const unsigned h = max(t[s], x); x = min(t[s], x); t[s] = h; }
       }
       float cm = fmaxf(fmaxf(fmaxf(v[0], v[1]), fmaxf(v[2], v[3])), fmaxf(fmaxf(v[4], v[5]), fmaxf(v[6], v[7])));
       cm = fmaxf(cm, fmaxf(fmaxf(fmaxf(v[8], v[9]), fmaxf(v[10], v[11])), fmaxf(fmaxf(v[12], v[13]), fmaxf(v[14], v[15]))));
@@ -385,6 +399,41 @@
       rec[ch] = make_float2(cm, cs);
     }
   }
+  unsigned thr = ~0u;
+  int ties = p.cand_k;
+#pragma unroll
+  for (int s = 0; s < VSR_MAX_BEAM; ++s) if (s < p.cand_k) thr = min(thr, t[s]);
+#pragma unroll
+  for (int s = 0; s < VSR_MAX_BEAM; ++s) if (s < p.cand_k && t[s] > thr) --ties;
+  if (thr == 0u) ties = 0;
+  unsigned long long* out = p.vcand + ((size_t)row * (2 * p.n_tiles) + 2 * (n0 / BN) + hsel) * p.cand_k;
+  int cnt = 0;
+#pragma unroll 1
+  for (int ch = c_lo; ch < c_hi; ++ch) {
+    uint32_t r[16];
+    tmem_ld16(tlane + (uint32_t)(ch * 16), r);
+    const int n = n0 + ch * 16;
+    if (live) {
+#pragma unroll
+      for (int j = 0; j < 16; j += 4) {
+        const float4 b = *reinterpret_cast<const float4*>(s_bias + ch * 16 + j);
+        const float v[4] = {__uint_as_float(r[j]) * sc + b.x, __uint_as_float(r[j + 1]) * sc + b.y,
+                            __uint_as_float(r[j + 2]) * sc + b.z, __uint_as_float(r[j + 3]) * sc + b.w};
+#pragma unroll
+        for (int u = 0; u < 4; ++u) {
+          const int col = n + j + u;
+          const unsigned x = col < p.n_valid ? vocab_orderable(v[u]) : 0u;
+          const bool tie = x == thr && ties > 0;
+          if (x > thr || tie) {
+            out[cnt++] = ((unsigned long long)x << 32) | (unsigned)(~(unsigned)col);
+            ties -= tie ? 1 : 0;
+          }
+        }
+      }
+    }
+  }
+  if (live)
+    for (; cnt < p.cand_k; ++cnt) out[cnt] = 0ull;
 }
 
 template <int BN>
@@ -1094,7 +1143,7 @@
 #undef TCP_SET_SMEM
 #undef TC_SET_SMEM
 #define PAIR_SET_SMEM(BN_, KB_, V_) VSR_CHECK_CUDA(cudaFuncSetAttribute(k_gemm_pair<BN_, KB_, V_>, cudaFuncAttributeMaxDynamicSharedMemorySize, PairCfg<BN_, KB_, V_>::kSmemBytes))
-  PAIR_SET_SMEM(192, 64, false); PAIR_SET_SMEM(192, 64, true); PAIR_SET_SMEM(256, 64, false);
+  PAIR_SET_SMEM(192, 64, false); PAIR_SET_SMEM(256, 64, false); PAIR_SET_SMEM(256, 64, true);
 #undef PAIR_SET_SMEM
   if (dev < 64) done_mask |= 1ull << dev;
   return VSR_OK;
@@ -1145,9 +1194,13 @@
   const FusedCell& f = g.cell;
   p->mode = f.mode;
   if (f.mode == EPI_VOCAB) {
-    VSR_REQUIRE(f.vocab_part != nullptr && g.bias != nullptr && g.c != nullptr && g.ldc % 16 == 0 && g.N % BN == 0, VSR_EINVAL,
-                "launch_gemm_tc: vocabulary epilogue needs a bias, an output padded to whole tiles and a record buffer (N tile %d)", BN);
-    p->vpart = f.vocab_part; p->n_valid = g.wb->n_valid;
+    VSR_REQUIRE(f.vocab_part != nullptr && f.vocab_cand != nullptr && f.vocab_lists_out != nullptr && g.bias != nullptr &&
+                    g.c != nullptr && g.ldc % 16 == 0 && g.N % BN == 0 && f.vocab_topk >= 1 && f.vocab_topk <= VSR_MAX_BEAM,
+                VSR_EINVAL, "launch_gemm_tc: vocabulary epilogue needs a bias, an output padded to whole tiles, record and "
+                "candidate buffers and 1 <= topk <= %d (N tile %d, topk %d)", VSR_MAX_BEAM, BN, f.vocab_topk);
+    p->vpart = f.vocab_part; p->vcand = f.vocab_cand; p->n_valid = g.wb->n_valid;
+    p->cand_k = f.vocab_topk; p->c_full = f.vocab_logits ? 1 : 0;
+    *f.vocab_lists_out = 2 * ((g.wb->n_valid + BN - 1) / BN);
   } else if (f.mode != 0) {
     VSR_REQUIRE((f.mode == EPI_LSTM1 && BN == 192) || (f.mode == EPI_LSTM2 && (BN == 128 || (pair && BN == 256))), VSR_EINVAL,
                 "launch_gemm_tc: fused cell mode %d does not fit N tile %d", f.mode, BN);
@@ -1168,7 +1221,7 @@
   const int BN = 2 * g.wb->pair_rows;
   if (g.N % BN != 0 || (BN != 192 && BN != 256)) return false;
   const int mode = g.cell.mode;
-  if (mode == EPI_VOCAB && BN != 192) return false;
+  if (mode == EPI_VOCAB && BN != 256) return false;
   if (mode == EPI_LSTM1 && BN != 192) return false;
   if (mode == EPI_LSTM2 && BN != 256) return false;
   if (g.cell.gt_cols % BN != 0) return false;
@@ -1193,7 +1246,7 @@
   if (sms == 0) cudaDeviceGetAttribute(&sms, cudaDevAttrMultiProcessorCount, 0);
   const int clusters = tiles < sms / 2 ? tiles : sms / 2;
 #define PAIR_LAUNCH(BN_, KB_, V_) VSR_CHECK_CUDA(launch_k(k_gemm_pair<BN_, KB_, V_>, dim3(2 * clusters), dim3(TC_THREADS), PairCfg<BN_, KB_, V_>::kSmemBytes, st, g.pdl, p))
-  if (BN == 192 && vocab) PAIR_LAUNCH(192, 64, true);
+  if (vocab) PAIR_LAUNCH(256, 64, true);
   else if (BN == 192) PAIR_LAUNCH(192, 64, false);
   else PAIR_LAUNCH(256, 64, false);
 #undef PAIR_LAUNCH
diff --git a/vsr-guided-cic_b200/csrc/step_kernels.cu b/vsr-guided-cic_b200/csrc/step_kernels.cu
--- a/vsr-guided-cic_b200/csrc/step_kernels.cu
+++ b/vsr-guided-cic_b200/csrc/step_kernels.cu
@@ -519,8 +519,9 @@
     }
     return;
   }
+  float* cl = a.cand_logit + (size_t)n * VSR_MAX_BEAM;
   if (!s_slow) {
-    if (tid < topk) cd[tid] = s_pick[tid];
+    if (tid < topk) { cd[tid] = s_pick[tid]; cl[tid] = x[s_pick[tid]]; }
     return;
   }
   float cv = v1; int ci = i1;
@@ -533,7 +534,7 @@
 #pragma unroll
     for (int w = 1; w < NW; ++w)
       if (before(red_v[j & 1][w], red_i[j & 1][w], bv, bi)) { bv = red_v[j & 1][w]; bi = red_i[j & 1][w]; }
-    if (tid == 0) cd[j] = bi;
+    if (tid == 0) { cd[j] = bi; cl[j] = bv; }
     if (ci == bi) {
       cv = -INFINITY; ci = 0x7fffffff;
       for (int jj = tid; jj < n4; jj += THREADS) {
@@ -549,14 +550,15 @@
 }
 
 constexpr int VM_WARPS = 4;
-__global__ void __launch_bounds__(VM_WARPS * 32) k_vocab_merge(const SoftmaxArgs a, const float* __restrict__ vpart, int n_chunks) {
+__global__ void __launch_bounds__(VM_WARPS * 32) k_vocab_merge(const SoftmaxArgs a, const float* __restrict__ vpart, int n_chunks,
+                                                               const unsigned long long* __restrict__ vcand, int n_keys) {
   const int lane = threadIdx.x & 31;
   const int n = blockIdx.x * VM_WARPS + (threadIdx.x >> 5);
   pdl_trigger();
   pdl_wait();
   if (n >= a.rows) return;
   RowHead h;
-  merge_row(a, vpart, n_chunks, n, lane, h);
+  merge_row(a, vpart, n_chunks, vcand, n_keys, n, lane, h);
   if (lane == 0) {
     a.row_max[n] = h.mx; a.row_lsum[n] = h.lsum; a.forced[n] = h.forced;
     a.gate_lp[(size_t)n * 2] = h.g0; a.gate_lp[(size_t)n * 2 + 1] = h.g1;
@@ -565,7 +567,10 @@
       a.gate_out[(size_t)n * a.gate_stride + 1] = h.g1;
     }
   }
-  if (lane < a.topk) a.cand[(size_t)n * VSR_MAX_BEAM + lane] = h.pick;
+  if (lane < a.topk) {
+    a.cand[(size_t)n * VSR_MAX_BEAM + lane] = h.pick;
+    a.cand_logit[(size_t)n * VSR_MAX_BEAM + lane] = h.pick_logit;
+  }
 }
 
 __global__ void __launch_bounds__(128) k_gate_head(const float* __restrict__ ha, int ld_ha, const float* __restrict__ ga, int ld_ga,
@@ -760,6 +765,7 @@
   if (io.skip_vocab) return VSR_OK;
   static const bool fuse_enabled = [] { const char* e = getenv("VSRDEC_FUSE_VOCAB"); return e == nullptr || atoi(e) != 0; }();
   const bool fuse_vocab = fuse_enabled && fused && io.out_logp == nullptr && io.topk > 0;
+  int vocab_lists = 0;
   {
     PhaseScope ps(c, PH_GEMM_E, st);
     GemmArgs g{};
@@ -769,7 +775,8 @@
     g.pdl = c->use_pdl && (c->pdl_mode & 1); g.pdl_flags = ((c->pdl_mode & 4) ? 1 : 0) | ((c->pdl_mode & 8) ? 2 : 0);
     g.f8 = c->gemm_f8; g.allow_pair = true; g.pair_min_rows = c->pair_min_rows;
     if (fuse_vocab) {
-      g.cell.mode = 3; g.cell.vocab_part = c->vpart;
+      g.cell.mode = 3; g.cell.vocab_part = c->vpart; g.cell.vocab_cand = c->vcand; g.cell.vocab_topk = io.topk;
+      g.cell.vocab_logits = io.keep_logits; g.cell.vocab_lists_out = &vocab_lists;
     }
     VSR_TRY(launch_gemm(c, g, st)); c->launches++;
   }
@@ -780,7 +787,7 @@
     a.gate_out = io.gate_out; a.gate_stride = io.gate_stride;
     if (fuse_vocab) {
       VSR_CHECK_CUDA(launch_k(k_vocab_merge, dim3((rows + VM_WARPS - 1) / VM_WARPS), dim3(VM_WARPS * 32), 0, st, c->use_pdl && (c->pdl_mode & 2),
-                              a, (const float*)c->vpart, c->NE / 16));
+                              a, (const float*)c->vpart, c->NE / 16, (const unsigned long long*)c->vcand, vocab_lists * io.topk));
     } else {
       VSR_CHECK_CUDA(launch_k(k_softmax_topk, dim3(rows), dim3(SM_THREADS), 0, st, c->use_pdl && (c->pdl_mode & 2), a));
     }
diff --git a/vsr-guided-cic_b200/csrc/vocab_head.cuh b/vsr-guided-cic_b200/csrc/vocab_head.cuh
--- a/vsr-guided-cic_b200/csrc/vocab_head.cuh
+++ b/vsr-guided-cic_b200/csrc/vocab_head.cuh
@@ -55,6 +55,7 @@
   const float* v_g; int A;
   const float* shift;
   float* row_max; float* row_lsum; int32_t* forced; int32_t* cand;
+  float* cand_logit;
   float* gate_lp;
   float* out_logp; int64_t out_stride;
   float* gate_out; int64_t gate_stride;
@@ -68,7 +69,7 @@
   a.vt_keys = c->vt_keys; a.vt_off = c->vt_off; a.vt_idx = c->vt_idx; a.vt_n = c->vt_n;
   a.ha = c->hb + c->oB2_ha; a.ld_ha = c->NB2; a.ga = c->ga; a.ld_ga = c->NC; a.v_g = c->v_g; a.A = c->A;
   a.shift = c->shift;
-  a.row_max = c->row_max; a.row_lsum = c->row_lsum; a.forced = c->forced; a.cand = c->cand;
+  a.row_max = c->row_max; a.row_lsum = c->row_lsum; a.forced = c->forced; a.cand = c->cand; a.cand_logit = c->cand_logit;
   a.gate_lp = c->gate_lp;
   return a;
 }
@@ -109,13 +110,17 @@
   float pick_logit;
 };
 
+__device__ __forceinline__ float from_orderable(unsigned k) {
+  return __uint_as_float((k & 0x80000000u) ? (k & 0x7fffffffu) : ~k);
+}
+
 constexpr int VM_CPL = 24;
 
 __device__ __forceinline__ void merge_row(const SoftmaxArgs& a, const float* __restrict__ vpart, int n_chunks,
-                                          int n, int lane, RowHead& out) {
+                                          const unsigned long long* __restrict__ vcand, int n_keys, int n, int lane,
+                                          RowHead& out) {
   const int V = a.V, topk = a.topk;
   const float2* rec = reinterpret_cast<const float2*>(vpart) + (size_t)n * n_chunks;
-  const float* x = a.logits + (size_t)n * a.ld;
   const int used = (V + 15) >> 4;
 
   int64_t verb = -1; float shift_logit = 0.f;
@@ -124,10 +129,8 @@
     if (a.use_verbs && a.verbs != nullptr)
       verb = load_verb(a.verbs, a.verbs_dtype, (size_t)(n / a.cur_beam) * a.L + a.ptr[n]);
   }
-  const bool in_regs = used <= 32 * VM_CPL;
-  float cmx[VM_CPL];
   float m = -INFINITY, ssum = 0.f;
-  if (in_regs) {
+  if (used <= 32 * VM_CPL) {
     float2 ms[VM_CPL];
 #pragma unroll
     for (int q = 0; q < VM_CPL; ++q) {
@@ -136,7 +139,6 @@
     }
 #pragma unroll
     for (int q = 0; q < VM_CPL; ++q) {
-      cmx[q] = ms[q].x;
       if (ms[q].x > m) { ssum *= __expf(m - ms[q].x); m = ms[q].x; }
       if (ms[q].x > -INFINITY) ssum += ms[q].y * __expf(ms[q].x - m);
     }
@@ -162,59 +164,36 @@
   const float lsum = logf(se);
   stay = warp_sum(stay);
 
-  unsigned long long prev = ~0ull;
-  int my_chunk = -1;
-  for (int j = 0; j < topk; ++j) {
-    unsigned long long best = 0ull;
-    if (in_regs) {
-#pragma unroll
-      for (int q = 0; q < VM_CPL; ++q) {
-        const int t = lane + 32 * q;
-        const unsigned long long key = ((unsigned long long)orderable(cmx[q]) << 32) | (unsigned)(~(unsigned)t);
-        if (cmx[q] > -INFINITY && key < prev && key > best) best = key;
-      }
-    } else {
-      for (int t = lane; t < used; t += 32) {
-        const float cm = rec[t].x;
-        const unsigned long long key = ((unsigned long long)orderable(cm) << 32) | (unsigned)(~(unsigned)t);
-        if (cm > -INFINITY && key < prev && key > best) best = key;
-      }
-    }
-    const unsigned hi = __reduce_max_sync(0xffffffffu, (unsigned)(best >> 32));
-    const unsigned lo = __reduce_max_sync(0xffffffffu, (unsigned)(best >> 32) == hi ? (unsigned)best : 0u);
-    prev = ((unsigned long long)hi << 32) | lo;
-    if (hi == 0u && lo == 0u) break;
-    if (lane == j) my_chunk = (int)(~lo);
-  }
-  constexpr int EQ = VSR_MAX_BEAM * 16 / 32;
-  float cv[EQ]; int ci[EQ];
-#pragma unroll
-  for (int q = 0; q < EQ; ++q) {
-    const int e = lane + 32 * q;
-    const int chunk = __shfl_sync(0xffffffffu, my_chunk, (e >> 4) & 31);
-    cv[q] = -INFINITY; ci[q] = 0x7fffffff;
-    if (e < topk * 16 && chunk >= 0) {
-      const int col = chunk * 16 + (e & 15);
-      if (col < V) { cv[q] = x[col]; ci[q] = col; }
+  const unsigned long long* keys = vcand + (size_t)n * n_keys;
+  unsigned long long best[VSR_MAX_BEAM];
+#pragma unroll
+  for (int s = 0; s < VSR_MAX_BEAM; ++s) best[s] = 0ull;
+#pragma unroll 4
+  for (int t = lane; t < n_keys; t += 32) {
+    unsigned long long x = keys[t];
+    if (x > best[VSR_MAX_BEAM - 1]) {
+#pragma unroll
+      for (int s = 0; s < VSR_MAX_BEAM; ++s)
+        if (x > best[s]) { const unsigned long long y = best[s]; best[s] = x; x = y; }
     }
   }
   int my_pick = 0x7fffffff; float my_logit = -INFINITY;
   for (int j = 0; j < topk; ++j) {
-    float bv = -INFINITY; int bi = 0x7fffffff;
-#pragma unroll
-    for (int q = 0; q < EQ; ++q) if (before(cv[q], ci[q], bv, bi)) { bv = cv[q]; bi = ci[q]; }
-    unsigned kb; int ib;
-    warp_argbest_redux(bv, bi, kb, ib);
-    const float wv = __shfl_sync(0xffffffffu, bv, __ffs(__ballot_sync(0xffffffffu, bi == ib)) - 1);
-#pragma unroll
-    for (int q = 0; q < EQ; ++q) if (ci[q] == ib) { cv[q] = -INFINITY; ci[q] = 0x7fffffff; }
-    if (lane == j) { my_pick = ib; my_logit = wv; }
+    const unsigned hi = __reduce_max_sync(0xffffffffu, (unsigned)(best[0] >> 32));
+    const unsigned lo = __reduce_max_sync(0xffffffffu, (unsigned)(best[0] >> 32) == hi ? (unsigned)best[0] : 0u);
+    if (hi == 0u && lo == 0u) break;
+    if (best[0] == (((unsigned long long)hi << 32) | lo)) {
+#pragma unroll
+      for (int s = 0; s + 1 < VSR_MAX_BEAM; ++s) best[s] = best[s + 1];
+      best[VSR_MAX_BEAM - 1] = 0ull;
+    }
+    if (lane == j) { my_pick = (int)(~lo); my_logit = from_orderable(hi); }
   }
 
   int forced = -1;
   float g0 = 0.f, g1 = 0.f;
   if (lane == 0) {
-    forced = forced_word(a, verb, x, mx, lsum);
+    forced = forced_word(a, verb, a.logits + (size_t)n * a.ld, mx, lsum);
     if (forced >= 0) { g0 = -1e3f; g1 = 0.f; }
     else {
       const float gm = fmaxf(stay, shift_logit);
```

After: 43890, median of 6. +2.3%, better.
